# AliaksandrSiarohin/wc-gan

Hardware: AMD Instinct MI355X
Metric: images/sec G+D step, CIFAR-10 ResNet-SN+WC, batch 64 (higher is better)
Workload: dtype f32; 1 GPU; CIFAR-10 ResNet SN uncond + WC (scripts/cifar10_resnet_sn_uncond.sh), batch 64/GPU, training_ratio 5, generator_batch_multiple 2; parallelism=dp1, wc_statistics=per-replica, launch=hipgraph

## Files before the change

include/wc_hip.h:

```cpp
#ifndef WC_HIP_H
#define WC_HIP_H

#include <stddef.h>
#include <stdint.h>

#ifdef __cplusplus
extern "C" {
#endif

#define WC_ABI_VERSION 8

#define WC_OK                 0
#define WC_ERR_NULL          -1
#define WC_ERR_SHAPE         -2
#define WC_ERR_CHANNELS      -3
#define WC_ERR_WORKSPACE     -4
#define WC_ERR_ARG           -5

typedef void* wc_stream_t;

int         wc_abi_version(void);
const char* wc_error_string(int code);

#define WC_CORE_API "wc_stats_f32 wc_factor_f64 wc_color_f32 wc_group_bias_f32 wc_apply_f32 wc_apply_act_f32 " \
                    "wc_bwd_reduce_f32 wc_bwd_factor_f64 wc_bwd_apply_f32 " \
                    "wc_stats_workspace_bytes wc_factor_workspace_bytes wc_color_workspace_bytes wc_apply_workspace_bytes " \
                    "wc_bwd_reduce_workspace_bytes wc_bwd_factor_workspace_bytes wc_bwd_apply_workspace_bytes"

size_t wc_whiten_workspace_bytes(int64_t M, int C, int groups);
size_t wc_factor_error_offset(int C, int groups);
int    wc_factor_route(int C, int groups);
size_t wc_whiten_error_offset(int64_t M, int C, int groups);
int    wc_whiten_f32(const float* x, int64_t M, int C, int groups, double eps, double momentum, int ddof,
                     float* moving_mean , float* moving_cov ,
                     float* mu , float* chan_scale , double* L , double* W ,
                     void* ws, size_t ws_bytes, wc_stream_t stream);

size_t wc_stats_workspace_bytes(int64_t M, int C, int groups);
size_t wc_factor_workspace_bytes(int C, int groups);
size_t wc_color_workspace_bytes(int C, int Kc);
size_t wc_bwd_reduce_workspace_bytes(int64_t N, int64_t HW, int C, int Kc, int has_slot);
size_t wc_bwd_factor_workspace_bytes(int C, int Kc);
size_t wc_apply_workspace_bytes(int64_t N, int64_t HW, int C, int Kc);
size_t wc_apply_plan_bytes(int C, int Kc);
size_t wc_bwd_apply_workspace_bytes(int64_t N, int64_t HW, int C, int Kc);

int wc_stats_f32(const float* x, int64_t M, int C, int groups,
                 double* sum , double* xtx ,
                 void* ws, size_t ws_bytes, wc_stream_t stream);

int wc_factor_f64(const double* sum, const double* xtx, int64_t M , int C, int groups,
                  double eps, double momentum, int ddof, int training,
                  float* moving_mean , float* moving_cov ,
                  float* mu , float* chan_scale ,
                  double* L , double* W ,
                  void* ws, size_t ws_bytes, wc_stream_t stream);

int wc_color_f32(const double* W , const float* gamma ,
                 int Kc, int C, int groups, int per_group,
                 float* A , float* At ,
                 const float* chan_scale , void* plan ,
                 void* ws, size_t ws_bytes, wc_stream_t stream);

int wc_group_bias_f32(const float* mu , const float* A ,
                      const float* beta ,
                      int groups, int Kc, int C, int per_group, float* center , float* bias ,
                      wc_stream_t stream);

int wc_apply_f32(const float* x, const float* mu, const float* A, const float* bias,
                 const int32_t* slot, int64_t N, int64_t HW, int C, int Kc,
                 float* y, const void* plan ,
                 void* ws, size_t ws_bytes, wc_stream_t stream);

int wc_apply_act_f32(const float* x, const float* mu, const float* A, const float* bias,
                     const int32_t* slot, int64_t N, int64_t HW, int C, int Kc, int relu,
                     float* y, const void* plan ,
                     void* ws, size_t ws_bytes, wc_stream_t stream);

size_t wc_split_bytes(int64_t M, int C);
#define WC_SPLIT_FLAG_WORDS (64 + 2 * 1024)
int wc_split_scales_f32(const float* x, int64_t M, int C, float* center , float* scale ,
                        int* flag , wc_stream_t stream);
int wc_split_f32(const float* x, const float* center , const float* scale, int64_t M, int C, int relu,
                 void* xs , int* flag , wc_stream_t stream);
int wc_unsplit_f32(const void* xs, const float* center , const float* scale, int64_t M, int C, float* x ,
                   wc_stream_t stream);

int    wc_stats_split_supported(int64_t M, int C, int groups);
size_t wc_stats_split_workspace_bytes(int64_t M, int C, int groups);
int wc_stats_split_f16x2(const void* xs, const float* xs_center, const float* xs_scale, int64_t M, int C, int groups,
                         double* sum , double* xtx , void* ws, size_t ws_bytes, wc_stream_t stream);

int    wc_split_bias_f32(const float* A , const float* bias, const float* xs_center, const float* mu, int Kc, int C,
                         float* bias_eff , wc_stream_t stream);
int    wc_apply_split_supported(int64_t N, int64_t HW, int C);
size_t wc_apply_split_workspace_bytes(int C, int Kc);
int wc_apply_split_f16x2(const void* xs, const float* xs_center , const float* xs_scale,
                         const float* mu , const float* A, const float* bias ,
                         const int32_t* slot, int64_t N, int64_t HW, int C, int Kc, int relu,
                         float* y, const void* plan , void* ws, size_t ws_bytes, wc_stream_t stream);

int wc_resadd_split_supported(int64_t N, int64_t H, int64_t W, int C);
int wc_resadd_f32(const float* h, const float* s , int64_t N, int64_t H, int64_t W, int C, int up, float* out,
                  wc_stream_t stream);
int wc_resadd_split_f32(const float* h, const float* s , int64_t N, int64_t H, int64_t W, int C, int up,
                        void* xs , float* center , float* scale ,
                        int* flag , float* x32 ,
                        wc_stream_t stream);
int wc_patch_sum_f32(const float* g , int64_t N, int64_t Hs, int64_t Ws, int C, float* out ,
                     wc_stream_t stream);
int    wc_resadd_stats_supported(int64_t N, int64_t H, int64_t W, int C, int up, int groups);
size_t wc_resadd_stats_workspace_bytes(int64_t N, int64_t H, int64_t W, int C, int groups);
int    wc_resadd_stats_split_f32(const float* h, const float* s , int64_t N, int64_t H, int64_t W, int C, int up, int groups,
                                 void* xs , float* center , float* scale , int* flag ,
                                 float* x32 , void* ws , size_t ws_bytes, wc_stream_t stream);
size_t wc_whiten_presummed_error_offset(int64_t M, int C, int groups);
int    wc_whiten_presummed_f16x2(const float* xs_center, int64_t M, int C, int groups, double eps, double momentum, int ddof,
                                 float* moving_mean , float* moving_cov , float* mu ,
                                 double* L , double* W , void* ws ,
                                 size_t ws_bytes, wc_stream_t stream);
int    wc_stats_presummed_f16x2(const float* xs_center, int64_t M, int C, int groups, double* sum ,
                                double* xtx , void* ws , size_t ws_bytes, wc_stream_t stream);
int wc_fold_channel_scale_f32(const float* w, int64_t stride_o, int64_t stride_c, int Cout, int Cin, const float* bias ,
                              const float* scale, const float* center, float* wf , float* bf , wc_stream_t stream);
int wc_unfold_channel_scale_f32(const float* D, const float* db, int64_t stride_o, int64_t stride_c, int Cout, int Cin,
                                const float* scale, const float* center, float* dW , wc_stream_t stream);

size_t wc_whiten_split_workspace_bytes(int64_t M, int C, int groups);
size_t wc_whiten_split_error_offset(int64_t M, int C, int groups);
int    wc_whiten_split_f16x2(const void* xs, const float* xs_center, const float* xs_scale, int64_t M, int C, int groups,
                             double eps, double momentum, int ddof, float* moving_mean , float* moving_cov ,
                             float* mu , double* L , double* W ,
                             void* ws, size_t ws_bytes, wc_stream_t stream);

int wc_color_split_f32(const double* W , const float* gamma , int Kc, int C, float* A ,
                       float* At , const float* xs_scale, const float* xs_center, const float* mu ,
                       const float* beta , void* plan , float* bias_eff ,
                       void* ws, size_t ws_bytes, wc_stream_t stream);
int wc_group_bias_centered_f32(const float* mu , const float* A , const float* beta ,
                               const float* center , int groups, int Kc, int C, int per_group, float* bias ,
                               wc_stream_t stream);

int    wc_factor_mix_supported(int E, int C);
int    wc_factor_mix_f32(const float* dict, const float* alpha, const int32_t* idx , const float* base ,
                         int E, int C, int K, int Kc, float* out , wc_stream_t stream);
size_t wc_factor_mix_bwd_workspace_bytes(int E, int Kc);
int    wc_factor_mix_bwd_f32(const float* dict, const float* alpha, const int32_t* idx , const float* dout ,
                             int E, int C, int K, int Kc, float* ddict , float* dalpha , float* dbase ,
                             void* ws, size_t ws_bytes, wc_stream_t stream);

int wc_apply_split_ex_f16x2(const void* xs, const float* xs_center , const float* xs_scale,
                            const float* mu , const float* A, const float* bias ,
                            const int32_t* slot, int64_t N, int64_t HW, int C, int Kc, int relu,
                            float* y , void* relu_mask , void* planes , float* oscale,
                            const void* plan , void* ws, size_t ws_bytes, wc_stream_t stream);

size_t wc_relu_mask_bytes(int64_t M, int C);
int wc_relu_mask_apply_f32(const float* gy, const void* relu_mask, int64_t M, int C, float* out, wc_stream_t stream);
int wc_apply_mask_f32(const float* x, const float* mu, const float* A, const float* bias,
                      const int32_t* slot, int64_t N, int64_t HW, int C, int Kc,
                      float* y, void* relu_mask , const void* plan ,
                      void* ws, size_t ws_bytes, wc_stream_t stream);

int    wc_apply_planes_supported(int64_t N, int64_t HW, int C);
size_t wc_apply_planes_scale_floats(void);
int    wc_out_scale_f32(const float* gamma , const float* beta , int K, int C,
                        float* oscale, wc_stream_t stream);
int    wc_apply_planes_f32(const float* x, const float* mu, const float* A, const float* bias, const int32_t* slot,
                           int64_t N, int64_t HW, int C, int Kc, int relu, void* planes , float* oscale,
                           void* relu_mask , const void* plan, wc_stream_t stream);

int wc_bwd_reduce_f32(const float* x, const float* mu, const float* gy, const int32_t* slot,
                      int64_t N, int64_t HW, int C, int Kc,
                      double* R , double* gsum ,
                      void* ws, size_t ws_bytes, wc_stream_t stream);

int wc_bwd_reduce_scaled_f32(const float* x, const float* mu, const float* gy, const int32_t* slot,
                             int64_t N, int64_t HW, int C, int Kc,
                             double* R , double* gsum , float* scales_out ,
                             void* ws, size_t ws_bytes, wc_stream_t stream);
int wc_bwd_reduce_relu_f32(const float* x, const float* mu, const float* gy, const float* relu_y , const int32_t* slot,
                           int64_t N, int64_t HW, int C, int Kc,
                           double* R , double* gsum , float* gy_masked ,
                           float* scales_out , void* ws, size_t ws_bytes, wc_stream_t stream);
int wc_bwd_reduce_mask_f32(const float* x, const float* mu, const float* gy, const void* relu_mask, const int32_t* slot,
                           int64_t N, int64_t HW, int C, int Kc,
                           double* R , double* gsum , float* gy_masked ,
                           float* scales_out , void* ws, size_t ws_bytes, wc_stream_t stream);

int wc_bwd_bits_supported(int64_t N, int64_t HW, int C, int has_slot);
int wc_bwd_reduce_bits_f32(const float* x, const float* mu, const float* gy, const void* relu_mask, const int32_t* slot,
                           int64_t N, int64_t HW, int C, int Kc, double* R , double* gsum ,
                           float* scales_out , void* ws, size_t ws_bytes, wc_stream_t stream);
int wc_bwd_apply_bits_f32(const float* gy, const void* relu_mask, const float* x, const float* mu, const float* At, const float* S,
                          const float* gmean, const int32_t* slot, int64_t N, int64_t HW, int C, int Kc,
                          const float* scales , float* dx, void* ws, size_t ws_bytes, wc_stream_t stream);
int wc_bwd_apply_scaled_f32(const float* gy, const float* x, const float* mu, const float* At,
                            const float* S, const float* gmean, const int32_t* slot,
                            int64_t N, int64_t HW, int C, int Kc, const float* scales , float* dx,
                            void* ws, size_t ws_bytes, wc_stream_t stream);

int    wc_bwd_xsplit_supported(int64_t N, int64_t HW, int C, int has_slot);
int    wc_bwd_reduce_xsplit_f32(const void* xs, const float* xs_center, const float* xs_scale, const float* mu, const float* gy,
                                const void* relu_mask , const int32_t* slot, int64_t N, int64_t HW, int C, int Kc,
                                double* R , double* gsum , float* scales_out ,
                                void* ws , size_t ws_bytes, wc_stream_t stream);
size_t wc_bwd_apply_xsplit_workspace_bytes(int C, int Kc);
int    wc_bwd_apply_xsplit_f32(const float* gy, const void* relu_mask , const void* xs, const float* xs_center,
                               const float* xs_scale, const float* mu, const float* At, const float* S, const float* gmean,
                               const int32_t* slot, int64_t N, int64_t HW, int C, int Kc, const float* scales ,
                               float* dx, void* ws, size_t ws_bytes, wc_stream_t stream);

int wc_bwd_factor_f64(const double* R, const double* gsum, const double* W, const double* L,
                      const float* gamma, const float* A, int Kc, int C, int64_t M,
                      double eps, int ddof, int training,
                      float* dgamma , float* dbeta ,
                      float* S , float* gmean ,
                      void* ws, size_t ws_bytes, wc_stream_t stream);

int wc_bwd_apply_f32(const float* gy, const float* x, const float* mu, const float* At,
                     const float* S, const float* gmean, const int32_t* slot,
                     int64_t N, int64_t HW, int C, int Kc, float* dx,
                     void* ws, size_t ws_bytes, wc_stream_t stream);

size_t wc_spectral_norm_workspace_bytes(int rows, int cols);
size_t wc_spectral_norm_amax_offset(int rows, int cols);
size_t wc_spectral_norm_error_offset(int rows, int cols);
int wc_spectral_norm_f32(const float* W, int rows, int cols, float* u, float* v, int iterations, float eps,
                         float* w_sn , float* sigma ,
                         float* u_used , float* v_used ,
                         void* ws, size_t ws_bytes, wc_stream_t stream);

int wc_spectral_norm_bwd_f32(const float* g, const float* w_sn, const float* u, const float* v, const float* sigma,
                             int rows, int cols, int fully_diff, float* dW,
                             void* ws, size_t ws_bytes, wc_stream_t stream);

typedef struct {
    const float* W; float* u; float* v; float* w_sn; float* sigma; float* u_used; float* v_used; void* ws;
    int rows, cols;
} wc_sn_item;
typedef struct {
    const float* g; const float* w_sn; const float* u; const float* v; const float* sigma; float* dW; void* ws;
    int rows, cols;
} wc_sn_bwd_item;
int wc_spectral_norm_batched_f32(const wc_sn_item* items, int count, int iterations, float eps, wc_stream_t stream);
int wc_spectral_norm_bwd_batched_f32(const wc_sn_bwd_item* items, int count, int fully_diff, wc_stream_t stream);

typedef struct {
    int N, H, W;
    int Hin, Win, Cin;
    int Hout, Wout, Cout;
    int in_stride, out_stride;
    int ntaps, nphase;
    signed char dy[4][16], dx[4][16];
    signed char off_y[4], off_x[4];
    signed char nsrc[4][16];
    signed char wr[4][16][4], ws[4][16][4];
    float wcoef;
} wc_conv_geom;

#define WC_CONV_SCRATCH_BYTES 2048

int wc_conv_supported(const wc_conv_geom* g);

int wc_conv_split_f32(const float* x, int64_t n, int relu, void* hi, void* lo, float* scale, void* amax_scratch,
                      wc_stream_t stream);

#define WC_CONV_COLSUM_ROWS 512
int wc_conv_split_colsum_f32(const float* x, int64_t n, int relu, void* hi, void* lo, float* scale, void* amax_scratch,
                             float* colsum_partials, int C, wc_stream_t stream);

#define WC_CONV_HIST_FLOATS (4 * 512 + 16)
#define WC_CONV_HIST_REDO (4 * 512)
int wc_conv_split_hist_f32(const float* x, int64_t n, int relu, void* hi, void* lo, float* scale, float* colsum_partials , int C,
                           float* hist, int bootstrap, wc_stream_t stream);

int wc_conv_split_leaky_f32(const float* x, int64_t n, float negative_slope, void* hi, void* lo, float* scale, void* amax_scratch,
                            float* colsum_partials , int C, wc_stream_t stream);
int wc_conv_split_hist_leaky_f32(const float* x, int64_t n, float negative_slope, void* hi, void* lo, float* scale,
                                 float* colsum_partials , int C, float* hist, int bootstrap, wc_stream_t stream);
int wc_conv_leaky_bwd_f32(float* dx, const float* x, int64_t n, float negative_slope, wc_stream_t stream);

size_t wc_conv_weights_bytes(const wc_conv_geom* g);
int wc_conv_weights_f32(const float* w, int64_t stride_k, int64_t stride_n, int64_t stride_r, int64_t stride_s,
                        int64_t n_elems, const wc_conv_geom* g, void* image, float* scale, void* amax_scratch,
                        const float* known_amax, int known_count, wc_stream_t stream);

int wc_conv_weights_pair_f32(const float* w, int64_t stride_r, int64_t stride_s, int64_t n_elems,
                             int64_t a_stride_k, int64_t a_stride_n, const wc_conv_geom* ga, void* image_a,
                             int64_t b_stride_k, int64_t b_stride_n, const wc_conv_geom* gb, void* image_b,
                             float* scale, void* amax_scratch, const float* known_amax, int known_count,
                             wc_stream_t stream);

size_t wc_conv_workspace_bytes(const wc_conv_geom* g);
int wc_conv_f16x3(const void* xhi, const void* xlo, const float* xscale, const void* wimage, const float* wscale,
                  const float* bias, const void* zero_line, const wc_conv_geom* g, int relu, float* y,
                  void* ws, size_t ws_bytes, wc_stream_t stream);

size_t wc_conv_wrw_workspace_bytes(const wc_conv_geom* g);
int wc_conv_wrw_f16x3(const void* xhi, const void* xlo, const float* xscale, const void* ghi, const void* glo,
                      const float* gscale, const void* zero_line, const wc_conv_geom* g, float* dw, int64_t stride_k,
                      int64_t stride_n, int64_t stride_r, int64_t stride_s, void* ws, size_t ws_bytes,
                      wc_stream_t stream);

int    wc_conv_wrw_narrow_supported(int64_t N, int64_t H, int64_t W, int Cin, int Cout, int ksize);
size_t wc_conv_wrw_narrow_workspace_bytes(int64_t N, int64_t H, int64_t W, int Cin, int Cout, int ksize);
int    wc_conv_wrw_narrow_f32(const float* x, const float* gy, int64_t N, int64_t H, int64_t W, int Cin, int Cout, int ksize,
                              float* dw, int64_t stride_k, int64_t stride_n, int64_t stride_r, int64_t stride_s, float* db ,
                              void* ws, size_t ws_bytes, wc_stream_t stream);

int    wc_conv_narrow64_supported(int64_t N, int64_t H, int64_t W, int Cin, int Cout, int ksize);
size_t wc_conv_wrw_narrow64_workspace_bytes(int64_t N, int64_t H, int64_t W, int Cin, int Cout, int ksize);
int    wc_conv_wrw_narrow64_f32(const float* x, const float* gy, int64_t N, int64_t H, int64_t W, int Cin, int Cout, int ksize,
                                float* dw, int64_t stride_k, int64_t stride_n, int64_t stride_r, int64_t stride_s, float* db ,
                                void* ws, size_t ws_bytes, wc_stream_t stream);

int    wc_conv_fwd_narrow_f32(const float* x, const float* w, int64_t stride_k, int64_t stride_n, int64_t stride_r, int64_t stride_s,
                              const float* bias , int64_t N, int64_t H, int64_t W, int Cin, int Cout, int ksize, int relu,
                              float* y, wc_stream_t stream);

int wc_conv_wrw_bias_f16x3(const void* xhi, const void* xlo, const float* xscale, const void* ghi, const void* glo,
                           const float* gscale, const void* zero_line, const wc_conv_geom* g, float* dw, int64_t stride_k,
                           int64_t stride_n, int64_t stride_r, int64_t stride_s, const float* colsum_partials, float* db,
                           void* ws, size_t ws_bytes, wc_stream_t stream);

int wc_stream_copy_f32(const float* src, float* dst, int64_t n, wc_stream_t stream);


size_t wc_std_stats_workspace_bytes(int64_t M, int C, int groups);
int    wc_std_stats_f32(const float* x, int64_t M, int C, int groups, double* sum , double* sqsum ,
                        void* ws, size_t ws_bytes, wc_stream_t stream);

int    wc_std_factor_f64(const double* sum, const double* sqsum, int64_t M, int C, int groups, double eps, double momentum, int ddof,
                         int training, float* moving_mean , float* moving_variance ,
                         const float* gamma , const float* beta , int Kc,
                         float* mu , float* w , float* a , float* b ,
                         wc_stream_t stream);

int    wc_std_apply_f32(const float* x, const float* a, const float* b, const int32_t* slot , int64_t N, int64_t HW,
                        int C, int Kt, int relu, float* y, wc_stream_t stream);

size_t wc_std_bwd_reduce_workspace_bytes(int64_t N, int64_t HW, int C, int Kc);
int    wc_std_bwd_reduce_f32(const float* x, const float* gy, const float* a, const float* b, const int32_t* slot, int64_t N, int64_t HW,
                             int C, int Kc, int relu, double* gsum , double* gxsum ,
                             void* ws, size_t ws_bytes, wc_stream_t stream);

int    wc_std_bwd_factor_f64(const double* gsum, const double* gxsum, const float* mu , const float* w ,
                             const float* gamma , int64_t M, int C, int Kc, int training,
                             float* dgamma , float* dbeta , float* q , float* r , wc_stream_t stream);

int    wc_std_bwd_apply_f32(const float* x, const float* gy, const float* a, const float* b, const float* q, const float* r,
                            const int32_t* slot, int64_t N, int64_t HW, int C, int Kc, int relu, float* dx, wc_stream_t stream);


int    wc_zca_supported(int C);
size_t wc_zca_workspace_bytes(int C, int groups);
size_t wc_zca_status_offset(int C, int groups);
int    wc_zca_f64(const double* L , int C, int groups, double eps,
                  double* U , double* lam , double* W ,
                  void* ws, size_t ws_bytes, wc_stream_t stream);

size_t wc_bwd_factor_zca_workspace_bytes(int C, int Kc);
int    wc_bwd_factor_zca_f64(const double* R, const double* gsum, const double* W, const double* U, const double* lam,
                             const float* gamma, const float* A, int Kc, int C, int64_t M,
                             double eps, int ddof, int training,
                             float* dgamma , float* dbeta ,
                             float* S , float* gmean ,
                             void* ws, size_t ws_bytes, wc_stream_t stream);


int    wc_renorm_supported(int C);
size_t wc_renorm_workspace_bytes(int C);
int    wc_renorm_f64(const float* moving_cov , const double* L , int C, double eps,
                     double* Wm , double* C0 ,
                     void* ws, size_t ws_bytes, wc_stream_t stream);

size_t wc_bwd_factor_renorm_workspace_bytes(int C, int Kc);
int    wc_bwd_factor_renorm_f64(const double* R, const double* gsum, const double* W, const double* Wm, const double* C0,
                                const float* gamma, const float* A, int Kc, int C, int64_t M,
                                double eps, int ddof, int training,
                                float* dgamma , float* dbeta ,
                                float* S , float* gmean ,
                                void* ws, size_t ws_bytes, wc_stream_t stream);


int wc_conv_split_masked_f32(const float* t, const float* a, int64_t n, float slope, void* hi, void* lo, float* scale, void* amax_scratch,
                             wc_stream_t stream);
int wc_conv_split_hist_masked_f32(const float* t, const float* a, int64_t n, float slope, void* hi, void* lo, float* scale, float* hist,
                                  int bootstrap, wc_stream_t stream);

int wc_gp_interp_f32(const float* real, const float* fake, const float* eps, int64_t N, int64_t L, float* x_hat, wc_stream_t stream);

size_t wc_gp_rows_workspace_bytes(int64_t N);
int wc_gp_rows_f32(const float* g, int64_t N, int64_t L, double lambda, double inv_n, float* norms , float* v ,
                   float* penalty , void* ws, size_t ws_bytes, wc_stream_t stream);

#ifdef __cplusplus
}
#endif
#endif
```

wc_gan_amd/_lib.py:

```python
from __future__ import annotations

import ctypes
import os
from ctypes import c_float, c_char_p, c_double, c_int, c_int64, c_size_t, c_void_p

_HERE = os.path.dirname(os.path.abspath(__file__))
LIB_PATH = os.path.join(_HERE, "libwc_hip.so")

WC_OK = 0
ABI_VERSION = 8
ERRORS = {-1: "WC_ERR_NULL", -2: "WC_ERR_SHAPE", -3: "WC_ERR_CHANNELS", -4: "WC_ERR_WORKSPACE", -5: "WC_ERR_ARG"}

SIGNATURES = {
    "wc_abi_version": (c_int, []),
    "wc_error_string": (c_char_p, [c_int]),
    "wc_stats_workspace_bytes": (c_size_t, [c_int64, c_int, c_int]),
    "wc_factor_workspace_bytes": (c_size_t, [c_int, c_int]),
    "wc_color_workspace_bytes": (c_size_t, [c_int, c_int]),
    "wc_bwd_reduce_workspace_bytes": (c_size_t, [c_int64, c_int64, c_int, c_int, c_int]),
    "wc_bwd_factor_workspace_bytes": (c_size_t, [c_int, c_int]),
    "wc_apply_workspace_bytes": (c_size_t, [c_int64, c_int64, c_int, c_int]),
    "wc_apply_plan_bytes": (c_size_t, [c_int, c_int]),
    "wc_bwd_apply_workspace_bytes": (c_size_t, [c_int64, c_int64, c_int, c_int]),
    "wc_stats_f32": (c_int, [c_void_p, c_int64, c_int, c_int, c_void_p, c_void_p, c_void_p, c_size_t, c_void_p]),
    "wc_group_bias_f32": (c_int, [c_void_p, c_void_p, c_void_p, c_int, c_int, c_int, c_int, c_void_p, c_void_p, c_void_p]),
    "wc_factor_f64": (c_int, [c_void_p, c_void_p, c_int64, c_int, c_int, c_double, c_double, c_int, c_int,
                              c_void_p, c_void_p, c_void_p, c_void_p, c_void_p, c_void_p, c_void_p, c_size_t, c_void_p]),
    "wc_color_f32": (c_int, [c_void_p, c_void_p, c_int, c_int, c_int, c_int, c_void_p, c_void_p, c_void_p, c_void_p,
                             c_void_p, c_size_t, c_void_p]),
    "wc_apply_f32": (c_int, [c_void_p, c_void_p, c_void_p, c_void_p, c_void_p, c_int64, c_int64, c_int, c_int,
                             c_void_p, c_void_p, c_void_p, c_size_t, c_void_p]),
    "wc_apply_act_f32": (c_int, [c_void_p, c_void_p, c_void_p, c_void_p, c_void_p, c_int64, c_int64, c_int, c_int, c_int,
                                 c_void_p, c_void_p, c_void_p, c_size_t, c_void_p]),
    "wc_bwd_reduce_f32": (c_int, [c_void_p, c_void_p, c_void_p, c_void_p, c_int64, c_int64, c_int, c_int,
                                  c_void_p, c_void_p, c_void_p, c_size_t, c_void_p]),
    "wc_bwd_reduce_scaled_f32": (c_int, [c_void_p, c_void_p, c_void_p, c_void_p, c_int64, c_int64, c_int, c_int,
                                         c_void_p, c_void_p, c_void_p, c_void_p, c_size_t, c_void_p]),
    "wc_bwd_reduce_relu_f32": (c_int, [c_void_p, c_void_p, c_void_p, c_void_p, c_void_p, c_int64, c_int64, c_int, c_int,
                                       c_void_p, c_void_p, c_void_p, c_void_p, c_void_p, c_size_t, c_void_p]),
    "wc_relu_mask_bytes": (c_size_t, [c_int64, c_int]),
    "wc_relu_mask_apply_f32": (c_int, [c_void_p, c_void_p, c_int64, c_int, c_void_p, c_void_p]),
    "wc_apply_mask_f32": (c_int, [c_void_p, c_void_p, c_void_p, c_void_p, c_void_p, c_int64, c_int64, c_int, c_int,
                                  c_void_p, c_void_p, c_void_p, c_void_p, c_size_t, c_void_p]),
    "wc_whiten_workspace_bytes": (c_size_t, [c_int64, c_int, c_int]),
    "wc_factor_error_offset": (c_size_t, [c_int, c_int]),
    "wc_factor_route": (c_int, [c_int, c_int]),
    "wc_whiten_error_offset": (c_size_t, [c_int64, c_int, c_int]),
    "wc_whiten_f32": (c_int, [c_void_p, c_int64, c_int, c_int, c_double, c_double, c_int, c_void_p, c_void_p, c_void_p, c_void_p,
                              c_void_p, c_void_p, c_void_p, c_size_t, c_void_p]),
    "wc_apply_planes_supported": (c_int, [c_int64, c_int64, c_int]),
    "wc_apply_planes_scale_floats": (c_size_t, []),
    "wc_out_scale_f32": (c_int, [c_void_p, c_void_p, c_int, c_int, c_void_p, c_void_p]),
    "wc_apply_planes_f32": (c_int, [c_void_p, c_void_p, c_void_p, c_void_p, c_void_p, c_int64, c_int64, c_int, c_int, c_int,
                                    c_void_p, c_void_p, c_void_p, c_void_p, c_void_p]),
    "wc_bwd_reduce_mask_f32": (c_int, [c_void_p, c_void_p, c_void_p, c_void_p, c_void_p, c_int64, c_int64, c_int, c_int,
                                       c_void_p, c_void_p, c_void_p, c_void_p, c_void_p, c_size_t, c_void_p]),
    "wc_bwd_bits_supported": (c_int, [c_int64, c_int64, c_int, c_int]),
    "wc_bwd_reduce_bits_f32": (c_int, [c_void_p, c_void_p, c_void_p, c_void_p, c_void_p, c_int64, c_int64, c_int, c_int,
                                       c_void_p, c_void_p, c_void_p, c_void_p, c_size_t, c_void_p]),
    "wc_bwd_apply_bits_f32": (c_int, [c_void_p, c_void_p, c_void_p, c_void_p, c_void_p, c_void_p, c_void_p, c_void_p,
                                      c_int64, c_int64, c_int, c_int, c_void_p, c_void_p, c_void_p, c_size_t, c_void_p]),
    "wc_bwd_apply_scaled_f32": (c_int, [c_void_p, c_void_p, c_void_p, c_void_p, c_void_p, c_void_p, c_void_p,
                                        c_int64, c_int64, c_int, c_int, c_void_p, c_void_p, c_void_p, c_size_t, c_void_p]),
    "wc_bwd_factor_f64": (c_int, [c_void_p, c_void_p, c_void_p, c_void_p, c_void_p, c_void_p, c_int, c_int, c_int64,
                                  c_double, c_int, c_int, c_void_p, c_void_p, c_void_p, c_void_p,
                                  c_void_p, c_size_t, c_void_p]),
    "wc_bwd_apply_f32": (c_int, [c_void_p, c_void_p, c_void_p, c_void_p, c_void_p, c_void_p, c_void_p,
                                 c_int64, c_int64, c_int, c_int, c_void_p, c_void_p, c_size_t, c_void_p]),
    "wc_split_bytes": (c_size_t, [c_int64, c_int]),
    "wc_split_scales_f32": (c_int, [c_void_p, c_int64, c_int, c_void_p, c_void_p, c_void_p, c_void_p]),
    "wc_split_f32": (c_int, [c_void_p, c_void_p, c_void_p, c_int64, c_int, c_int, c_void_p, c_void_p, c_void_p]),
    "wc_unsplit_f32": (c_int, [c_void_p, c_void_p, c_void_p, c_int64, c_int, c_void_p, c_void_p]),
    "wc_stats_split_supported": (c_int, [c_int64, c_int, c_int]),
    "wc_stats_split_workspace_bytes": (c_size_t, [c_int64, c_int, c_int]),
    "wc_stats_split_f16x2": (c_int, [c_void_p, c_void_p, c_void_p, c_int64, c_int, c_int, c_void_p, c_void_p, c_void_p, c_size_t, c_void_p]),
    "wc_split_bias_f32": (c_int, [c_void_p, c_void_p, c_void_p, c_void_p, c_int, c_int, c_void_p, c_void_p]),
    "wc_apply_split_supported": (c_int, [c_int64, c_int64, c_int]),
    "wc_apply_split_workspace_bytes": (c_size_t, [c_int, c_int]),
    "wc_apply_split_f16x2": (c_int, [c_void_p, c_void_p, c_void_p, c_void_p, c_void_p, c_void_p, c_void_p, c_int64, c_int64,
                                     c_int, c_int, c_int, c_void_p, c_void_p, c_void_p, c_size_t, c_void_p]),
    "wc_apply_split_ex_f16x2": (c_int, [c_void_p, c_void_p, c_void_p, c_void_p, c_void_p, c_void_p, c_void_p, c_int64, c_int64,
                                        c_int, c_int, c_int, c_void_p, c_void_p, c_void_p, c_void_p, c_void_p, c_void_p, c_size_t, c_void_p]),
    "wc_whiten_split_workspace_bytes": (c_size_t, [c_int64, c_int, c_int]),
    "wc_whiten_split_error_offset": (c_size_t, [c_int64, c_int, c_int]),
    "wc_whiten_split_f16x2": (c_int, [c_void_p, c_void_p, c_void_p, c_int64, c_int, c_int, c_double, c_double, c_int, c_void_p, c_void_p,
                                      c_void_p, c_void_p, c_void_p, c_void_p, c_size_t, c_void_p]),
    "wc_resadd_split_supported": (c_int, [c_int64, c_int64, c_int64, c_int]),
    "wc_resadd_f32": (c_int, [c_void_p, c_void_p, c_int64, c_int64, c_int64, c_int, c_int, c_void_p, c_void_p]),
    "wc_resadd_stats_supported": (c_int, [c_int64, c_int64, c_int64, c_int, c_int, c_int]),
    "wc_resadd_stats_workspace_bytes": (c_size_t, [c_int64, c_int64, c_int64, c_int, c_int]),
    "wc_resadd_stats_split_f32": (c_int, [c_void_p, c_void_p, c_int64, c_int64, c_int64, c_int, c_int, c_int, c_void_p, c_void_p, c_void_p, c_void_p,
                                          c_void_p, c_void_p, c_size_t, c_void_p]),
    "wc_whiten_presummed_error_offset": (c_size_t, [c_int64, c_int, c_int]),
    "wc_whiten_presummed_f16x2": (c_int, [c_void_p, c_int64, c_int, c_int, c_double, c_double, c_int, c_void_p, c_void_p, c_void_p, c_void_p,
                                          c_void_p, c_void_p, c_size_t, c_void_p]),
    "wc_stats_presummed_f16x2": (c_int, [c_void_p, c_int64, c_int, c_int, c_void_p, c_void_p, c_void_p, c_size_t, c_void_p]),
    "wc_resadd_split_f32": (c_int, [c_void_p, c_void_p, c_int64, c_int64, c_int64, c_int, c_int, c_void_p, c_void_p, c_void_p, c_void_p,
                                    c_void_p, c_void_p]),
    "wc_patch_sum_f32": (c_int, [c_void_p, c_int64, c_int64, c_int64, c_int, c_void_p, c_void_p]),
    "wc_fold_channel_scale_f32": (c_int, [c_void_p, c_int64, c_int64, c_int, c_int, c_void_p, c_void_p, c_void_p, c_void_p, c_void_p, c_void_p]),
    "wc_unfold_channel_scale_f32": (c_int, [c_void_p, c_void_p, c_int64, c_int64, c_int, c_int, c_void_p, c_void_p, c_void_p, c_void_p]),
    "wc_color_split_f32": (c_int, [c_void_p, c_void_p, c_int, c_int, c_void_p, c_void_p, c_void_p, c_void_p, c_void_p, c_void_p, c_void_p,
                                   c_void_p, c_void_p, c_size_t, c_void_p]),
    "wc_factor_mix_supported": (c_int, [c_int, c_int]),
    "wc_factor_mix_f32": (c_int, [c_void_p, c_void_p, c_void_p, c_void_p, c_int, c_int, c_int, c_int, c_void_p, c_void_p]),
    "wc_factor_mix_bwd_workspace_bytes": (c_size_t, [c_int, c_int]),
    "wc_factor_mix_bwd_f32": (c_int, [c_void_p, c_void_p, c_void_p, c_void_p, c_int, c_int, c_int, c_int, c_void_p, c_void_p, c_void_p,
                                      c_void_p, c_size_t, c_void_p]),
    "wc_group_bias_centered_f32": (c_int, [c_void_p, c_void_p, c_void_p, c_void_p, c_int, c_int, c_int, c_int, c_void_p, c_void_p]),
    "wc_bwd_xsplit_supported": (c_int, [c_int64, c_int64, c_int, c_int]),
    "wc_bwd_reduce_xsplit_f32": (c_int, [c_void_p, c_void_p, c_void_p, c_void_p, c_void_p, c_void_p, c_void_p, c_int64, c_int64, c_int, c_int,
                                         c_void_p, c_void_p, c_void_p, c_void_p, c_size_t, c_void_p]),
    "wc_bwd_apply_xsplit_workspace_bytes": (c_size_t, [c_int, c_int]),
    "wc_bwd_apply_xsplit_f32": (c_int, [c_void_p, c_void_p, c_void_p, c_void_p, c_void_p, c_void_p, c_void_p, c_void_p, c_void_p, c_void_p,
                                        c_int64, c_int64, c_int, c_int, c_void_p, c_void_p, c_void_p, c_size_t, c_void_p]),
    "wc_stream_copy_f32": (c_int, [c_void_p, c_void_p, c_int64, c_void_p]),
    "wc_spectral_norm_workspace_bytes": (c_size_t, [c_int, c_int]),
    "wc_spectral_norm_batched_f32": (c_int, [c_void_p, c_int, c_int, c_float, c_void_p]),
    "wc_spectral_norm_bwd_batched_f32": (c_int, [c_void_p, c_int, c_int, c_void_p]),
    "wc_spectral_norm_f32": (c_int, [c_void_p, c_int, c_int, c_void_p, c_void_p, c_int, c_float, c_void_p, c_void_p,
                                     c_void_p, c_void_p, c_void_p, c_size_t, c_void_p]),
    "wc_spectral_norm_bwd_f32": (c_int, [c_void_p, c_void_p, c_void_p, c_void_p, c_void_p, c_int, c_int, c_int, c_void_p,
                                         c_void_p, c_size_t, c_void_p]),
    "wc_conv_supported": (c_int, [c_void_p]),
    "wc_conv_split_f32": (c_int, [c_void_p, c_int64, c_int, c_void_p, c_void_p, c_void_p, c_void_p, c_void_p]),
    "wc_conv_weights_bytes": (c_size_t, [c_void_p]),
    "wc_conv_weights_f32": (c_int, [c_void_p, c_int64, c_int64, c_int64, c_int64, c_int64, c_void_p, c_void_p, c_void_p,
                                    c_void_p, c_void_p, c_int, c_void_p]),
    "wc_spectral_norm_amax_offset": (c_size_t, [c_int, c_int]),
    "wc_spectral_norm_error_offset": (c_size_t, [c_int, c_int]),
    "wc_conv_split_hist_f32": (c_int, [c_void_p, c_int64, c_int, c_void_p, c_void_p, c_void_p, c_void_p, c_int, c_void_p, c_int, c_void_p]),
    "wc_conv_split_leaky_f32": (c_int, [c_void_p, c_int64, c_float, c_void_p, c_void_p, c_void_p, c_void_p, c_void_p, c_int, c_void_p]),
    "wc_conv_split_hist_leaky_f32": (c_int, [c_void_p, c_int64, c_float, c_void_p, c_void_p, c_void_p, c_void_p, c_int, c_void_p, c_int, c_void_p]),
    "wc_conv_leaky_bwd_f32": (c_int, [c_void_p, c_void_p, c_int64, c_float, c_void_p]),
    "wc_conv_narrow64_supported": (c_int, [c_int64, c_int64, c_int64, c_int, c_int, c_int]),
    "wc_conv_wrw_narrow64_workspace_bytes": (c_size_t, [c_int64, c_int64, c_int64, c_int, c_int, c_int]),
    "wc_conv_wrw_narrow64_f32": (c_int, [c_void_p, c_void_p, c_int64, c_int64, c_int64, c_int, c_int, c_int, c_void_p, c_int64, c_int64, c_int64,
                                         c_int64, c_void_p, c_void_p, c_size_t, c_void_p]),
    "wc_conv_fwd_narrow_f32": (c_int, [c_void_p, c_void_p, c_int64, c_int64, c_int64, c_int64, c_void_p, c_int64, c_int64, c_int64, c_int, c_int, c_int,
                                       c_int, c_void_p, c_void_p]),
    "wc_conv_wrw_narrow_supported": (c_int, [c_int64, c_int64, c_int64, c_int, c_int, c_int]),
    "wc_conv_wrw_narrow_workspace_bytes": (c_size_t, [c_int64, c_int64, c_int64, c_int, c_int, c_int]),
    "wc_conv_wrw_narrow_f32": (c_int, [c_void_p, c_void_p, c_int64, c_int64, c_int64, c_int, c_int, c_int, c_void_p, c_int64, c_int64, c_int64,
                                       c_int64, c_void_p, c_void_p, c_size_t, c_void_p]),
    "wc_conv_split_colsum_f32": (c_int, [c_void_p, c_int64, c_int, c_void_p, c_void_p, c_void_p, c_void_p, c_void_p, c_int, c_void_p]),
    "wc_conv_wrw_bias_f16x3": (c_int, [c_void_p, c_void_p, c_void_p, c_void_p, c_void_p, c_void_p, c_void_p, c_void_p, c_void_p,
                                       c_int64, c_int64, c_int64, c_int64, c_void_p, c_void_p, c_void_p, c_size_t, c_void_p]),
    "wc_conv_weights_pair_f32": (c_int, [c_void_p, c_int64, c_int64, c_int64, c_int64, c_int64, c_void_p, c_void_p,
                                         c_int64, c_int64, c_void_p, c_void_p, c_void_p, c_void_p, c_void_p, c_int, c_void_p]),
    "wc_conv_wrw_workspace_bytes": (c_size_t, [c_void_p]),
    "wc_conv_wrw_f16x3": (c_int, [c_void_p, c_void_p, c_void_p, c_void_p, c_void_p, c_void_p, c_void_p, c_void_p, c_void_p,
                                  c_int64, c_int64, c_int64, c_int64, c_void_p, c_size_t, c_void_p]),
    "wc_conv_workspace_bytes": (c_size_t, [c_void_p]),
    "wc_conv_f16x3": (c_int, [c_void_p, c_void_p, c_void_p, c_void_p, c_void_p, c_void_p, c_void_p, c_void_p, c_int,
                              c_void_p, c_void_p, c_size_t, c_void_p]),
    "wc_std_stats_workspace_bytes": (c_size_t, [c_int64, c_int, c_int]),
    "wc_std_stats_f32": (c_int, [c_void_p, c_int64, c_int, c_int, c_void_p, c_void_p, c_void_p, c_size_t, c_void_p]),
    "wc_std_factor_f64": (c_int, [c_void_p, c_void_p, c_int64, c_int, c_int, c_double, c_double, c_int, c_int, c_void_p, c_void_p,
                                  c_void_p, c_void_p, c_int, c_void_p, c_void_p, c_void_p, c_void_p, c_void_p]),
    "wc_std_apply_f32": (c_int, [c_void_p, c_void_p, c_void_p, c_void_p, c_int64, c_int64, c_int, c_int, c_int, c_void_p, c_void_p]),
    "wc_std_bwd_reduce_workspace_bytes": (c_size_t, [c_int64, c_int64, c_int, c_int]),
    "wc_std_bwd_reduce_f32": (c_int, [c_void_p, c_void_p, c_void_p, c_void_p, c_void_p, c_int64, c_int64, c_int, c_int, c_int,
                                      c_void_p, c_void_p, c_void_p, c_size_t, c_void_p]),
    "wc_std_bwd_factor_f64": (c_int, [c_void_p, c_void_p, c_void_p, c_void_p, c_void_p, c_int64, c_int, c_int, c_int,
                                      c_void_p, c_void_p, c_void_p, c_void_p, c_void_p]),
    "wc_std_bwd_apply_f32": (c_int, [c_void_p, c_void_p, c_void_p, c_void_p, c_void_p, c_void_p, c_void_p, c_int64, c_int64, c_int, c_int,
                                     c_int, c_void_p, c_void_p]),
    "wc_zca_supported": (c_int, [c_int]),
    "wc_zca_workspace_bytes": (c_size_t, [c_int, c_int]),
    "wc_zca_status_offset": (c_size_t, [c_int, c_int]),
    "wc_zca_f64": (c_int, [c_void_p, c_int, c_int, c_double, c_void_p, c_void_p, c_void_p, c_void_p, c_size_t, c_void_p]),
    "wc_bwd_factor_zca_workspace_bytes": (c_size_t, [c_int, c_int]),
    "wc_bwd_factor_zca_f64": (c_int, [c_void_p, c_void_p, c_void_p, c_void_p, c_void_p, c_void_p, c_void_p, c_int, c_int, c_int64,
                                      c_double, c_int, c_int, c_void_p, c_void_p, c_void_p, c_void_p,
                                      c_void_p, c_size_t, c_void_p]),
    "wc_renorm_supported": (c_int, [c_int]),
    "wc_renorm_workspace_bytes": (c_size_t, [c_int]),
    "wc_renorm_f64": (c_int, [c_void_p, c_void_p, c_int, c_double, c_void_p, c_void_p, c_void_p, c_size_t, c_void_p]),
    "wc_bwd_factor_renorm_workspace_bytes": (c_size_t, [c_int, c_int]),
    "wc_bwd_factor_renorm_f64": (c_int, [c_void_p, c_void_p, c_void_p, c_void_p, c_void_p, c_void_p, c_void_p, c_int, c_int, c_int64,
                                         c_double, c_int, c_int, c_void_p, c_void_p, c_void_p, c_void_p,
                                         c_void_p, c_size_t, c_void_p]),
    "wc_conv_split_masked_f32": (c_int, [c_void_p, c_void_p, c_int64, c_float, c_void_p, c_void_p, c_void_p, c_void_p, c_void_p]),
    "wc_conv_split_hist_masked_f32": (c_int, [c_void_p, c_void_p, c_int64, c_float, c_void_p, c_void_p, c_void_p, c_void_p, c_int, c_void_p]),
    "wc_gp_interp_f32": (c_int, [c_void_p, c_void_p, c_void_p, c_int64, c_int64, c_void_p, c_void_p]),
    "wc_gp_rows_workspace_bytes": (c_size_t, [c_int64]),
    "wc_gp_rows_f32": (c_int, [c_void_p, c_int64, c_int64, c_double, c_double, c_void_p, c_void_p, c_void_p, c_void_p, c_size_t, c_void_p]),
}


class SnItem(ctypes.Structure):
    _fields_ = [("W", c_void_p), ("u", c_void_p), ("v", c_void_p), ("w_sn", c_void_p), ("sigma", c_void_p),
                ("u_used", c_void_p), ("v_used", c_void_p), ("ws", c_void_p), ("rows", c_int), ("cols", c_int)]


class SnBwdItem(ctypes.Structure):
    _fields_ = [("g", c_void_p), ("w_sn", c_void_p), ("u", c_void_p), ("v", c_void_p), ("sigma", c_void_p),
                ("dW", c_void_p), ("ws", c_void_p), ("rows", c_int), ("cols", c_int)]


class ConvGeom(ctypes.Structure):
    _fields_ = [("N", c_int), ("H", c_int), ("W", c_int), ("Hin", c_int), ("Win", c_int), ("Cin", c_int),
                ("Hout", c_int), ("Wout", c_int), ("Cout", c_int), ("in_stride", c_int), ("out_stride", c_int),
                ("ntaps", c_int), ("nphase", c_int),
                ("dy", (ctypes.c_byte * 16) * 4), ("dx", (ctypes.c_byte * 16) * 4),
                ("off_y", ctypes.c_byte * 4), ("off_x", ctypes.c_byte * 4),
                ("nsrc", (ctypes.c_byte * 16) * 4),
                ("wr", ((ctypes.c_byte * 4) * 16) * 4), ("ws", ((ctypes.c_byte * 4) * 16) * 4),
                ("wcoef", c_float)]


_lib = None


class WcHipError(RuntimeError):
    pass


def shared_gpu_guard(device_count=None) -> bool:
    if "WC_K2_TWO_LAUNCH" in os.environ:
        if os.environ["WC_K2_TWO_LAUNCH"] == "0":
            del os.environ["WC_K2_TWO_LAUNCH"]
        return False
    try:
        ranks = int(os.environ.get("LOCAL_WORLD_SIZE", "1") or 1)
    except ValueError:
        ranks = 1
    if ranks <= 1:
        return False
    if any(os.environ.get(k) for k in ("HIP_VISIBLE_DEVICES", "CUDA_VISIBLE_DEVICES", "ROCR_VISIBLE_DEVICES")):
        return False
    if device_count is None:
        try:
            import torch
            device_count = torch.cuda.device_count()
        except Exception:
            device_count = 0
    if device_count and ranks > device_count:
        os.environ["WC_K2_TWO_LAUNCH"] = "1"
        return True
    return False


def load() -> ctypes.CDLL:
    global _lib
    if _lib is not None:
        return _lib
    import torch
    shared_gpu_guard()
    if not os.path.exists(LIB_PATH):
        raise WcHipError(
            f"{LIB_PATH} is missing: build it with `python -m wc_gan_amd.build` "
            "(or __graft_entry__.build()); the WC path has no non-HIP fallback")
    lib = ctypes.CDLL(LIB_PATH)
    for name, (res, args) in SIGNATURES.items():
        fn = getattr(lib, name)
        fn.restype = res
        fn.argtypes = args
    if lib.wc_abi_version() != ABI_VERSION:
        raise WcHipError(f"libwc_hip.so ABI version {lib.wc_abi_version()} != {ABI_VERSION}: rebuild it "
                         "(python -m wc_gan_amd.build)")
    _lib = lib
    return lib


def check(code: int, what: str) -> None:
    if code == WC_OK:
        return
    lib = load()
    msg = lib.wc_error_string(code)
    raise WcHipError(f"{what} failed: {ERRORS.get(code, code)} ({msg.decode() if msg else '?'})")
```

wc_gan_amd/conv.py:

```python
from __future__ import annotations

import ctypes
import os

import torch
import torch.nn.functional as F

from . import _lib, _state
from .ops import _ptr, _stream

_zero_lines = {}


def _zero_line(device):
    z = _zero_lines.get(device)
    if z is None:
        z = _zero_lines[device] = torch.zeros(64, dtype=torch.uint8, device=device)
    return z


def _plain(r, s):
    return [(r, s)], 1.0


def _pooled3(r, s):
    return [(r - a, s - b) for a in (0, 1) for b in (0, 1) if 0 <= r - a <= 2 and 0 <= s - b <= 2], 0.25


_UP_ROWS = ((2,), (1, 2), (0, 1), (0,))


def _upsampled3(r, s):
    return [(r3, s3) for r3 in _UP_ROWS[r] for s3 in _UP_ROWS[s]], 1.0


def _set_sources(g, p, t, r, s, source):
    taps, coef = source(r, s)
    g.nsrc[p][t] = len(taps)
    for m, (r3, s3) in enumerate(taps):
        g.wr[p][t][m], g.ws[p][t][m] = r3, s3
    g.wcoef = coef


def _dense_geom(N, Hin, Win, Cin, Cout, k, stride, source=_plain):
    pad = k // 2 if stride == 1 else 1
    g = _lib.ConvGeom()
    g.N, g.Hin, g.Win, g.Cin, g.Cout = N, Hin, Win, Cin, Cout
    g.H, g.W = Hin // stride, Win // stride
    g.Hout, g.Wout = g.H, g.W
    g.in_stride, g.out_stride, g.ntaps, g.nphase = stride, 1, k * k, 1
    for r in range(k):
        for s in range(k):
            t = r * k + s
            g.dy[0][t], g.dx[0][t] = r - pad, s - pad
            _set_sources(g, 0, t, r, s, source)
    return g


def _phase_geom(N, Hin, Win, Cin, Cout, source=_plain):
    g = _lib.ConvGeom()
    g.N, g.Hin, g.Win, g.Cin, g.Cout = N, Hin, Win, Cin, Cout
    g.H, g.W, g.Hout, g.Wout = Hin, Win, 2 * Hin, 2 * Win
    g.in_stride, g.out_stride, g.ntaps, g.nphase = 1, 2, 4, 4
    for py in range(2):
        for px in range(2):
            p = py * 2 + px
            g.off_y[p], g.off_x[p] = py, px
            t = 0
            for dy in ((-1, 0) if py == 0 else (0, 1)):
                for dx in ((-1, 0) if px == 0 else (0, 1)):
                    g.dy[p][t], g.dx[p][t] = dy, dx
                    _set_sources(g, p, t, py + 1 - 2 * dy, px + 1 - 2 * dx, source)
                    t += 1
    return g


def _supported(g):
    return bool(_lib.load().wc_conv_supported(ctypes.addressof(g)))


def supported(x, w, kind):
    handed = getattr(x, '_wc_planes', None) is not None
    if not (x.is_cuda and x.dtype == torch.float32 and x.dim() == 4 and (handed or x.is_contiguous()) and w.dtype == torch.float32):
        return False
    p = _plan(kind, x, w)
    return bool(p) and p.ok


class _Plan:
    __slots__ = ('ok', 'fwd', 'bwd', 'fwd_ws', 'bwd_ws', 'wrw_ws', 'fwd_ptr', 'bwd_ptr')

    def __init__(self, kind, N, H, W, wshape):
        class _W:
            shape = wshape
        lib = _lib.load()
        (gf, kf, nf), (gb, kb, nb) = _geoms(kind, N, H, W, _W)
        self.fwd, self.bwd = (gf, kf, nf), (gb, kb, nb)
        self.fwd_ptr, self.bwd_ptr = ctypes.addressof(gf), ctypes.addressof(gb)
        self.ok = bool(lib.wc_conv_supported(self.fwd_ptr)) and bool(lib.wc_conv_supported(self.bwd_ptr))
        self.fwd_ws = lib.wc_conv_workspace_bytes(self.fwd_ptr) if self.ok else 0
        self.bwd_ws = lib.wc_conv_workspace_bytes(self.bwd_ptr) if self.ok else 0
        self.wrw_ws = lib.wc_conv_wrw_workspace_bytes(self.fwd_ptr) if self.ok else 0


_plans = {}


def _plan(kind, x, w):
    key = (kind, tuple(x.shape), tuple(w.shape))
    p = _plans.get(key)
    if p is None:
        N, H, W, C = x.shape
        good = (kind == 'same' and w.shape[1] == C and w.shape[2] == w.shape[3] and w.shape[2] in (1, 3)) or \
               (kind == 'down' and w.shape[1] == C and tuple(w.shape[2:]) == (4, 4) and H % 2 == 0 and W % 2 == 0) or \
               (kind == 'down3' and w.shape[1] == C and tuple(w.shape[2:]) == (3, 3) and H % 2 == 0 and W % 2 == 0) or \
               (kind == 'up3' and w.shape[1] == C and tuple(w.shape[2:]) == (3, 3)) or \
               (kind == 'up' and w.shape[0] == C and tuple(w.shape[2:]) == (4, 4))
        if kind not in ('same', 'down', 'up', 'down3', 'up3'):
            raise ValueError(kind)
        if good and kind != 'down' and (C % 128 or w.shape[0] % 128 or w.shape[1] % 128):
            good = False
        p = _plans[key] = _Plan(kind, N, H, W, tuple(w.shape)) if good else False
    return p


def _colsum_ok(C):
    return C % 4 == 0 and 256 % (C // 4) == 0


SPLIT_HIST = os.environ.get('WC_SPLIT_HIST', '1') != '0'
HIST_FLOATS = 4 * 512 + 16
HIST_REDO = 4 * 512


_REDO_MODE = os.environ.get('WC_SPLIT_HIST_REDO', '1')


def _guarded(role):
    return _REDO_MODE == '2' or (_REDO_MODE != '0' and role in ('g', 't', 'd'))


def _site_hist(site, role, device):
    if not getattr(site, 'training', True):
        return None
    book = site.__dict__.setdefault('_wc_split_hist', {})
    h = book.get(role)
    if h is not None and h[0].device != device:
        h = None
    if h is None:
        if torch.cuda.is_current_stream_capturing():
            return None
        h = book[role] = [torch.zeros(HIST_FLOATS, dtype=torch.float32, device=device), False]
    return h


def split_planes(x, relu=False, colsum=False, site=None, role='x', leaky=None):
    lib = _lib.load()
    if leaky is not None:
        if relu:
            raise ValueError("relu and leaky are two activations")
        return _split_planes_leaky(lib, x, float(leaky), colsum, site, role)
    both = torch.empty((2,) + tuple(x.shape), dtype=torch.float16, device=x.device)
    hi, lo = both[0], both[1]
    scale = torch.empty(1 + 512, dtype=torch.float32, device=x.device)
    h = _site_hist(site, role, x.device) if (SPLIT_HIST and site is not None) else None
    if h is not None:
        C = x.shape[-1]
        part = torch.empty((512, C), dtype=torch.float32, device=x.device) if colsum else None
        _lib.check(lib.wc_conv_split_hist_f32(_ptr(x), x.numel(), 1 if relu else 0, _ptr(hi), _ptr(lo), _ptr(scale), _ptr(part), C if colsum else 0,
                                              _ptr(h[0]), (0 if h[1] else 1) | (0 if _guarded(role) else 2), _stream()), "wc_conv_split_hist_f32")
        h[1] = True
        return (hi, lo, scale, part) if colsum else (hi, lo, scale)
    if not colsum:
        _lib.check(lib.wc_conv_split_f32(_ptr(x), x.numel(), 1 if relu else 0, _ptr(hi), _ptr(lo), _ptr(scale),
                                         scale.data_ptr() + 4, _stream()), "wc_conv_split_f32")
        return hi, lo, scale
    C = x.shape[-1]
    part = torch.empty((512, C), dtype=torch.float32, device=x.device)
    _lib.check(lib.wc_conv_split_colsum_f32(_ptr(x), x.numel(), 1 if relu else 0, _ptr(hi), _ptr(lo), _ptr(scale),
                                            scale.data_ptr() + 4, _ptr(part), C, _stream()), "wc_conv_split_colsum_f32")
    return hi, lo, scale, part


def _split_planes_leaky(lib, x, slope, colsum, site, role):
    both = torch.empty((2,) + tuple(x.shape), dtype=torch.float16, device=x.device)
    hi, lo = both[0], both[1]
    scale = torch.empty(1 + 512, dtype=torch.float32, device=x.device)
    C = x.shape[-1]
    part = torch.empty((512, C), dtype=torch.float32, device=x.device) if colsum else None
    h = _site_hist(site, role, x.device) if (SPLIT_HIST and site is not None) else None
    if h is not None:
        _lib.check(lib.wc_conv_split_hist_leaky_f32(_ptr(x), x.numel(), slope, _ptr(hi), _ptr(lo), _ptr(scale), _ptr(part), C if colsum else 0,
                                                    _ptr(h[0]), (0 if h[1] else 1) | (0 if _guarded(role) else 2), _stream()),
                   "wc_conv_split_hist_leaky_f32")
        h[1] = True
    else:
        _lib.check(lib.wc_conv_split_leaky_f32(_ptr(x), x.numel(), slope, _ptr(hi), _ptr(lo), _ptr(scale), scale.data_ptr() + 4,
                                               _ptr(part), C if colsum else 0, _stream()), "wc_conv_split_leaky_f32")
    return (hi, lo, scale, part) if colsum else (hi, lo, scale)


def split_planes_masked(t, a, slope=0.0, site=None, role='t'):
    if not (t.is_contiguous() and a.is_contiguous() and t.shape == a.shape and t.dtype == a.dtype == torch.float32):
        raise ValueError("split_planes_masked: dense fp32 tensors of one shape")
    lib = _lib.load()
    both = torch.empty((2,) + tuple(t.shape), dtype=torch.float16, device=t.device)
    hi, lo = both[0], both[1]
    scale = torch.empty(1 + 512, dtype=torch.float32, device=t.device)
    h = _site_hist(site, role, t.device) if (SPLIT_HIST and site is not None) else None
    if h is not None:
        _lib.check(lib.wc_conv_split_hist_masked_f32(_ptr(t), _ptr(a), t.numel(), float(slope), _ptr(hi), _ptr(lo), _ptr(scale), _ptr(h[0]),
                                                     (0 if h[1] else 1) | (0 if _guarded(role) else 2), _stream()),
                   "wc_conv_split_hist_masked_f32")
        h[1] = True
    else:
        _lib.check(lib.wc_conv_split_masked_f32(_ptr(t), _ptr(a), t.numel(), float(slope), _ptr(hi), _ptr(lo), _ptr(scale),
                                                scale.data_ptr() + 4, _stream()), "wc_conv_split_masked_f32")
    return hi, lo, scale


def leaky_backward_(dx, x, slope):
    if not (dx.is_contiguous() and x.is_contiguous() and dx.shape == x.shape and dx.dtype == x.dtype == torch.float32):
        raise ValueError("leaky_backward_: dense fp32 tensors of one shape")
    _lib.check(_lib.load().wc_conv_leaky_bwd_f32(_ptr(dx), _ptr(x), dx.numel(), float(slope), _stream()), "wc_conv_leaky_bwd_f32")
    return dx


def _storage_extent(w):
    return 1 + sum((n - 1) * s for n, s in zip(w.shape, w.stride()))


def weight_image(w, geom, k_axis, n_axis):
    lib = _lib.load()
    nbytes = lib.wc_conv_weights_bytes(ctypes.addressof(geom))
    img = torch.empty(nbytes, dtype=torch.uint8, device=w.device)
    scale = torch.empty(1 + 512, dtype=torch.float32, device=w.device)
    ext = _storage_extent(w)
    if ext != w.numel():
        raise ValueError("weight must be dense")
    known = getattr(w, '_wc_amax', None)
    _lib.check(lib.wc_conv_weights_f32(_ptr(w), w.stride(k_axis), w.stride(n_axis), w.stride(2), w.stride(3), ext,
                                       ctypes.addressof(geom), _ptr(img), _ptr(scale), scale.data_ptr() + 4,
                                       _ptr(known), 0 if known is None else known.numel(), _stream()),
               "wc_conv_weights_f32")
    return img, scale


def weight_image_pair(w, fwd, bwd):
    lib = _lib.load()
    (ga, ka, na), (gb, kb, nb) = fwd, bwd
    img_a = torch.empty(lib.wc_conv_weights_bytes(ctypes.addressof(ga)), dtype=torch.uint8, device=w.device)
    img_b = torch.empty(lib.wc_conv_weights_bytes(ctypes.addressof(gb)), dtype=torch.uint8, device=w.device)
    scale = torch.empty(2 + 512, dtype=torch.float32, device=w.device)
    ext = _storage_extent(w)
    if ext != w.numel():
        raise ValueError("weight must be dense")
    known = getattr(w, '_wc_amax', None)
    _lib.check(lib.wc_conv_weights_pair_f32(_ptr(w), w.stride(2), w.stride(3), ext,
                                            w.stride(ka), w.stride(na), ctypes.addressof(ga), _ptr(img_a),
                                            w.stride(kb), w.stride(nb), ctypes.addressof(gb), _ptr(img_b),
                                            _ptr(scale), scale.data_ptr() + 8, _ptr(known), 0 if known is None else known.numel(),
                                            _stream()), "wc_conv_weights_pair_f32")
    return (img_a, scale[0:1]), (img_b, scale[1:2])


def _cached_image(w, key, geom, k_axis, n_axis):
    return weight_image(w, geom, k_axis, n_axis)


def run(planes, image, geom, bias=None, relu=False, nbytes=None):
    hi, lo, xs = planes
    img, ws = image
    lib = _lib.load()
    y = torch.empty((geom.N, geom.Hout, geom.Wout, geom.Cout), dtype=torch.float32, device=hi.device)
    if nbytes is None:
        nbytes = lib.wc_conv_workspace_bytes(ctypes.addressof(geom))
    work = torch.empty(nbytes, dtype=torch.uint8, device=hi.device) if nbytes else None
    _lib.check(lib.wc_conv_f16x3(_ptr(hi), _ptr(lo), _ptr(xs), _ptr(img), _ptr(ws), _ptr(bias) if bias is not None else None,
                                 _ptr(_zero_line(hi.device)), ctypes.addressof(geom), 1 if relu else 0, _ptr(y),
                                 _ptr(work), nbytes, _stream()), "wc_conv_f16x3")
    return y


def _geoms(kind, N, H, W, w):
    if kind == 'same':
        co, ci, k = w.shape[0], w.shape[1], w.shape[2]
        fwd = _dense_geom(N, H, W, ci, co, k, 1)
        bwd = _dense_geom(N, H, W, co, ci, k, 1)
        for t in range(k * k):
            bwd.dy[0][t], bwd.dx[0][t] = -bwd.dy[0][t], -bwd.dx[0][t]
        return (fwd, 1, 0), (bwd, 0, 1)
    if kind in ('down', 'down3'):
        co, ci = w.shape[0], w.shape[1]
        src = _pooled3 if kind == 'down3' else _plain
        return (_dense_geom(N, H, W, ci, co, 4, 2, src), 1, 0), (_phase_geom(N, H // 2, W // 2, co, ci, src), 0, 1)
    if kind == 'up3':
        co, ci = w.shape[0], w.shape[1]
        return (_phase_geom(N, H, W, ci, co, _upsampled3), 1, 0), (_dense_geom(N, 2 * H, 2 * W, co, ci, 4, 2, _upsampled3), 0, 1)
    ci, co = w.shape[0], w.shape[1]
    return (_phase_geom(N, H, W, ci, co), 0, 1), (_dense_geom(N, 2 * H, 2 * W, co, ci, 4, 2), 1, 0)


def weight_gradient(x_planes, g_planes, geom, w, k_axis, n_axis, nbytes=None, colsum=None):
    lib = _lib.load()
    xh, xl, xs = x_planes
    gh, gl, gs = g_planes[:3]
    dw = torch.empty_like(w)
    if dw.stride() != w.stride():
        raise ValueError("weight must be dense")
    if nbytes is None:
        nbytes = lib.wc_conv_wrw_workspace_bytes(ctypes.addressof(geom))
    ws = torch.empty(nbytes, dtype=torch.uint8, device=w.device)
    if colsum is not None:
        db = torch.empty(geom.Cout, dtype=torch.float32, device=w.device)
        _lib.check(lib.wc_conv_wrw_bias_f16x3(_ptr(xh), _ptr(xl), _ptr(xs), _ptr(gh), _ptr(gl), _ptr(gs), _ptr(_zero_line(w.device)),
                                              ctypes.addressof(geom), _ptr(dw), w.stride(k_axis), w.stride(n_axis), w.stride(2),
                                              w.stride(3), _ptr(colsum), _ptr(db), _ptr(ws), nbytes, _stream()),
                   "wc_conv_wrw_bias_f16x3")
        return dw, db
    _lib.check(lib.wc_conv_wrw_f16x3(_ptr(xh), _ptr(xl), _ptr(xs), _ptr(gh), _ptr(gl), _ptr(gs), _ptr(_zero_line(w.device)),
                                     ctypes.addressof(geom), _ptr(dw), w.stride(k_axis), w.stride(n_axis), w.stride(2),
                                     w.stride(3), _ptr(ws), nbytes, _stream()), "wc_conv_wrw_f16x3")
    return dw


def takes_planes(shape, wshape, kind):
    class _S:
        pass
    xs, ws = _S(), _S()
    xs.shape, ws.shape = tuple(shape), tuple(wshape)
    p = _plan(kind, xs, ws)
    return bool(p) and p.ok


class _FastConv(torch.autograd.Function):
    @staticmethod
    def forward(ctx, x, w, bias, kind, plan, relu_input=False, handed=None, site=None, leaky=None):
        gf, kf, nf = plan.fwd
        planes = handed if handed is not None else split_planes(x, relu=relu_input, site=site, role='x', leaky=leaky)
        ctx.site, ctx.leaky = site, leaky
        if ctx.needs_input_grad[0]:
            img, ctx.bwd_image = weight_image_pair(w, plan.fwd, plan.bwd)
        else:
            img, ctx.bwd_image = weight_image(w, gf, kf, nf), None
        y = run(planes, img, gf, bias, nbytes=plan.fwd_ws)
        ctx.save_for_backward(w, *planes, *((x,) if (relu_input or leaky is not None) else ()))
        ctx.kind, ctx.has_bias, ctx.plan, ctx.relu_input = kind, bias is not None, plan, relu_input
        return y

    @staticmethod
    def backward(ctx, gy):
        w, xh, xl, xs = ctx.saved_tensors[:4]
        kind, plan = ctx.kind, ctx.plan
        gy = gy.contiguous()
        want_db = ctx.has_bias and ctx.needs_input_grad[2]
        fused_db = want_db and ctx.needs_input_grad[1] and _colsum_ok(gy.shape[-1])
        g_planes = split_planes(gy, colsum=fused_db, site=ctx.site, role='g')
        dx = dw = db = None
        if ctx.needs_input_grad[0]:
            gb, kb, nb = plan.bwd
            image = ctx.bwd_image if ctx.bwd_image is not None else weight_image(w, gb, kb, nb)
            dx = run(g_planes[:3], image, gb, nbytes=plan.bwd_ws)
            if ctx.relu_input:
                dx = torch.ops.aten.threshold_backward(dx, ctx.saved_tensors[4], 0)
            elif ctx.leaky is not None:
                dx = leaky_backward_(dx, ctx.saved_tensors[4], ctx.leaky)
        if ctx.needs_input_grad[1]:
            gf, kf, nf = plan.fwd
            if fused_db:
                dw, db = weight_gradient((xh, xl, xs), g_planes, gf, w, kf, nf, nbytes=plan.wrw_ws, colsum=g_planes[3])
            else:
                dw = weight_gradient((xh, xl, xs), g_planes, gf, w, kf, nf, nbytes=plan.wrw_ws)
        if want_db and not fused_db:
            db = gy.sum((0, 1, 2))
        return dx, dw, db, None, None, None, None, None, None


_ones = {}


def _one(device):
    t = _ones.get(device)
    if t is None:
        t = torch.ones(1, dtype=torch.float32, device=device)
        if not torch.cuda.is_current_stream_capturing():
            _ones[device] = t
    return t


class _SplitConv(torch.autograd.Function):

    @staticmethod
    def forward(ctx, x, w, bias, plan, st, site=None):
        from . import ops
        ctx.site = site
        gf, kf, nf = plan.fwd
        wf, bf = ops.fold_channel_scale(w, bias, st.scale, st.center)
        img = weight_image(wf, gf, kf, nf)
        ctx.bwd_image = None
        if ctx.needs_input_grad[0]:
            gb, kb, nb = plan.bwd
            ctx.bwd_image = weight_image(w, gb, kb, nb)
        hi, lo = st.planes[0].view(st.shape), st.planes[1].view(st.shape)
        one = _one(hi.device)
        y = run((hi, lo, one), img, gf, bf, nbytes=plan.fwd_ws)
        ctx.save_for_backward(w, hi, lo, one, st.scale, st.center)
        ctx.plan, ctx.has_bias = plan, bias is not None
        return y

    @staticmethod
    def backward(ctx, gy):
        from . import ops
        w, xh, xl, one, scale, center = ctx.saved_tensors
        plan = ctx.plan
        gy = gy.contiguous()
        need_w = ctx.needs_input_grad[1]
        need_b = ctx.has_bias and ctx.needs_input_grad[2]
        fused_db = need_w and _colsum_ok(gy.shape[-1])
        g_planes = split_planes(gy, colsum=fused_db, site=ctx.site, role='g')
        dx = dw = db = None
        if ctx.needs_input_grad[0]:
            gb, kb, nb = plan.bwd
            image = ctx.bwd_image if ctx.bwd_image is not None else weight_image(w, gb, kb, nb)
            dx = run(g_planes[:3], image, gb, nbytes=plan.bwd_ws)
        if need_w:
            gf, kf, nf = plan.fwd
            if fused_db:
                D, db = weight_gradient((xh, xl, one), g_planes, gf, w, kf, nf, nbytes=plan.wrw_ws, colsum=g_planes[3])
            else:
                D = weight_gradient((xh, xl, one), g_planes, gf, w, kf, nf, nbytes=plan.wrw_ws)
                db = gy.sum((0, 1, 2))
            dw = ops.unfold_channel_scale(D, db, scale, center)
        elif need_b:
            db = gy.sum((0, 1, 2))
        return dx, dw, (db if need_b else None), None, None, None


def split_conv(x, st, w, bias=None, site=None):
    p = _plan('same', x, w)
    if not (p and p.ok and tuple(w.shape[2:]) == (1, 1) and w.dtype == torch.float32):
        raise _lib.WcHipError(f"split_conv: a pre-split handle reached a convolution without a planes path {tuple(x.shape)} x {tuple(w.shape)}")
    return _SplitConv.apply(x, w, bias, p, st, site)


def fast_conv_or_none(x, w, bias=None, kind='same', relu_input=False, site=None, leaky_input=None):
    if leaky_input is not None and relu_input:
        raise ValueError("relu_input and leaky_input are two activations")
    handed = getattr(x, '_wc_planes', None)
    if not supported(x, w, kind):
        if handed is not None:
            raise _lib.WcHipError(f"fast_conv: a K3 handle reached a convolution that cannot take planes {tuple(x.shape)} x {tuple(w.shape)} ({kind})")
        return None
    if handed is not None:
        if relu_input or leaky_input is not None:
            raise ValueError("a K3 handle is already ReLU'd")
        return _FastConv.apply(x, w, bias, kind, _plan(kind, x, w), False, handed, site)
    return _FastConv.apply(x, w, bias, kind, _plan(kind, x, w), relu_input, None, site,
                           None if leaky_input is None else float(leaky_input))


NARROW_WRW = os.environ.get('WC_NARROW_WRW', '1') != '0'


def narrow_wrw_supported(x, w):
    if not (NARROW_WRW and x.is_cuda and x.dtype == torch.float32 and w.dtype == torch.float32 and x.dim() == 4 and w.dim() == 4):
        return False
    k = w.shape[2]
    if w.shape[3] != k or k not in (1, 3) or w.shape[1] != x.shape[3]:
        return False
    N, H, W, C = x.shape
    return bool(_lib.load().wc_conv_narrow64_supported(N, H, W, C, w.shape[0], k))


def narrow_forward(x, w, bias=None, relu=False, mirrored=False):
    lib = _lib.load()
    N, H, W, C = x.shape
    k = w.shape[2]
    if mirrored:
        O = w.shape[1]
        ptr = ctypes.c_void_p(w.data_ptr() + 4 * ((k - 1) * w.stride(2) + (k - 1) * w.stride(3)))
        strides = (w.stride(0), w.stride(1), -w.stride(2), -w.stride(3))
    else:
        O = w.shape[0]
        ptr = _ptr(w)
        strides = (w.stride(1), w.stride(0), w.stride(2), w.stride(3))
    y = torch.empty((N, H, W, O), dtype=torch.float32, device=x.device)
    xc = x if x.is_contiguous() else x.contiguous()
    _lib.check(lib.wc_conv_fwd_narrow_f32(_ptr(xc), ptr, *strides, _ptr(bias), N, H, W, C, O, k, 1 if relu else 0, _ptr(y), _stream()),
               "wc_conv_fwd_narrow_f32")
    return y


class _NarrowInConv(torch.autograd.Function):

    @staticmethod
    def forward(ctx, x, w, bias):
        ctx.save_for_backward(x, w)
        ctx.has_bias = bias is not None
        return narrow_forward(x, w, bias)

    @staticmethod
    def backward(ctx, gy):
        x, w = ctx.saved_tensors
        N, H, W, C = x.shape
        O, k = w.shape[0], w.shape[2]
        lib = _lib.load()
        dx = dw = db = None
        g = gy if gy.is_contiguous() else gy.contiguous()
        if ctx.needs_input_grad[0]:
            dx = torch.ops.aten.convolution_backward(g.permute(0, 3, 1, 2), x.permute(0, 3, 1, 2), w, None, [1, 1], [k // 2, k // 2], [1, 1],
                                                     False, [0, 0], 1, [True, False, False])[0].permute(0, 2, 3, 1)
        if ctx.needs_input_grad[1] or (ctx.has_bias and ctx.needs_input_grad[2]):
            dw = torch.empty_strided(w.shape, w.stride(), dtype=torch.float32, device=w.device)
            if _storage_extent(dw) != dw.numel():
                raise ValueError("weight must be dense")
            db = torch.empty(O, dtype=torch.float32, device=w.device) if ctx.has_bias else None
            nb = lib.wc_conv_wrw_narrow64_workspace_bytes(N, H, W, C, O, k)
            ws = torch.empty(nb, dtype=torch.uint8, device=x.device)
            xc = x if x.is_contiguous() else x.contiguous()
            _lib.check(lib.wc_conv_wrw_narrow64_f32(_ptr(xc), _ptr(g), N, H, W, C, O, k, _ptr(dw), dw.stride(1), dw.stride(0), dw.stride(2),
                                                    dw.stride(3), _ptr(db), _ptr(ws), nb, _stream()), "wc_conv_wrw_narrow64_f32")
        return dx, dw, db


def narrow_weight_gradient(x, gy, w):
    N, H, W, C = x.shape
    O, k = w.shape[0], w.shape[2]
    lib = _lib.load()
    dw = torch.empty_strided(w.shape, w.stride(), dtype=torch.float32, device=w.device)
    if _storage_extent(dw) != dw.numel():
        raise ValueError("weight must be dense")
    nb = lib.wc_conv_wrw_narrow64_workspace_bytes(N, H, W, C, O, k)
    ws = torch.empty(nb, dtype=torch.uint8, device=x.device)
    xc = x if x.is_contiguous() else x.contiguous()
    g = gy if gy.is_contiguous() else gy.contiguous()
    _lib.check(lib.wc_conv_wrw_narrow64_f32(_ptr(xc), _ptr(g), N, H, W, C, O, k, _ptr(dw), dw.stride(1), dw.stride(0), dw.stride(2),
                                            dw.stride(3), None, _ptr(ws), nb, _stream()), "wc_conv_wrw_narrow64_f32")
    return dw


def narrow_in_conv(x, w, bias=None):
    if _storage_extent(w) != w.numel():
        w = w.contiguous()
    return _NarrowInConv.apply(x, w, bias)


def narrow_out_weight_gradient(x, gy, w):
    lib = _lib.load()
    N, H, W, C = x.shape
    O, k = w.shape[0], w.shape[2]
    dw = torch.empty_strided(w.shape, w.stride(), dtype=torch.float32, device=w.device)
    if _storage_extent(dw) != dw.numel():
        raise ValueError("weight must be dense")
    nb = lib.wc_conv_wrw_narrow_workspace_bytes(N, H, W, O, C, k)
    ws = torch.empty(nb, dtype=torch.uint8, device=x.device)
    last = dw.data_ptr() + 4 * ((k - 1) * dw.stride(2) + (k - 1) * dw.stride(3))
    _lib.check(lib.wc_conv_wrw_narrow_f32(_ptr(gy), _ptr(x), N, H, W, O, C, k, ctypes.c_void_p(last), dw.stride(0), dw.stride(1), -dw.stride(2),
                                          -dw.stride(3), None, _ptr(ws), nb, _stream()), "wc_conv_wrw_narrow_f32")
    return dw


def narrow_out_wrw_supported(x, w):
    if not (NARROW_WRW and x.is_cuda and x.dtype == torch.float32 and w.dtype == torch.float32 and x.dim() == 4 and w.dim() == 4):
        return False
    k = w.shape[2]
    if w.shape[3] != k or k not in (1, 3) or w.shape[1] != x.shape[3]:
        return False
    N, H, W, C = x.shape
    return bool(_lib.load().wc_conv_wrw_narrow_supported(N, H, W, w.shape[0], C, k))


def fast_conv(x, w, bias=None, kind='same'):
    if not supported(x, w, kind):
        raise _lib.WcHipError(f"fast_conv: unsupported call {tuple(x.shape)} x {tuple(w.shape)} ({kind})")
    return _FastConv.apply(x, w, bias, kind, _plan(kind, x, w))
```

wc_gan_amd/csrc/wc_conv.hip:

```cpp
#include "wc_common.h"
#include "../../include/wc_hip.h"
#include <stdlib.h>


namespace {

constexpr int kMaxTaps = 16, kMaxPhase = 4;

struct ConvArgs {
    const _Float16* xhi; const _Float16* xlo;
    const _Float16* zero;
    const char* wimg;
    const float* xscale; const float* wscale;
    const float* bias;
    float* y;
    int N, H, W, Hin, Win, Cin, Cout, in_stride, ntaps, nphase, Hout, Wout, out_stride, relu;
    unsigned magHW, shHW, magW, shW;
    int ksplit; float* partial;
    signed char dy[kMaxPhase][kMaxTaps], dx[kMaxPhase][kMaxTaps];
    signed char offy[kMaxPhase], offx[kMaxPhase];
};

__device__ __forceinline__ void lds_dma16(const void* g, unsigned lds)
{
    unsigned keep;
    asm volatile("s_mov_b32 %0, m0\n\ts_mov_b32 m0, %2\n\ts_nop 0\n\tglobal_load_lds_dwordx4 %1, off\n\ts_mov_b32 m0, %0"
                 : "=&s"(keep) : "v"(g), "s"(lds) : "memory");
}

template <int MB, int NB, bool KS>
__global__ __launch_bounds__(256) void conv_f16x3_kernel(ConvArgs a)
{
    extern __shared__ __attribute__((aligned(16))) char smem[];
    constexpr int TM = 64 * MB, TN = 64 * NB;
    constexpr int A_BYTES = 2 * MB * 4 * 1024, B_BYTES = 2 * NB * 4 * 1024, STAGE = A_BYTES + B_BYTES;
    constexpr int AQ = (2 * MB) / 4;
    static_assert(AQ >= 1, "MB >= 2");

    const int tid = threadIdx.x, lane = tid & 63;
    const int wave = __builtin_amdgcn_readfirstlane(tid >> 6);
    const int wm = wave >> 1, wn = wave & 1;
    const int ntn = a.Cout / TN;
    const int phase = blockIdx.y / ntn, nt = blockIdx.y - phase * ntn;
    const unsigned m0 = blockIdx.x * TM;
    const unsigned HW = a.H * a.W;
    const int koff = (lane >> 5) * 8;

    int gy[AQ], gx[AQ];
    unsigned gpix[AQ];
    #pragma unroll
    for (int q = 0; q < AQ; ++q) {
        const unsigned m = m0 + (wave * AQ + q) * 32 + (lane & 31);
        const unsigned n = __umulhi(m, a.magHW) >> a.shHW, rem = m - n * HW;
        const unsigned yy = __umulhi(rem, a.magW) >> a.shW, xx = rem - yy * a.W;
        gy[q] = yy * a.in_stride; gx[q] = xx * a.in_stride; gpix[q] = n * (a.Hin * a.Win);
    }
    const unsigned lds0 = (unsigned)(size_t)((__attribute__((address_space(3))) char*)smem);
    const int nchunk = a.Cin >> 5;
    const int iters = a.ntaps * nchunk;
    const int nblk_all = a.Cout >> 5;

    auto issue = [&](int it, int stage) {
        const int tap = it / nchunk, ch = it - tap * nchunk;
        const int dy = a.dy[phase][tap], dx = a.dx[phase][tap];
        const unsigned sbase = __builtin_amdgcn_readfirstlane(lds0 + stage * STAGE);
        #pragma unroll
        for (int q = 0; q < AQ; ++q) {
            const int iy = gy[q] + dy, ix = gx[q] + dx;
            const bool ok = (unsigned)iy < (unsigned)a.Hin && (unsigned)ix < (unsigned)a.Win;
            const int64_t e = ((int64_t)(gpix[q] + iy * a.Win + ix)) * a.Cin + ch * 32 + koff;
            #pragma unroll
            for (int s = 0; s < 2; ++s) {
                const _Float16* ph = ok ? a.xhi + e + s * 16 : a.zero + koff;
                const _Float16* pl = ok ? a.xlo + e + s * 16 : a.zero + koff;
                const unsigned l = sbase + (((wave * AQ + q) * 2 + s) * 2) * 1024;
                lds_dma16(ph, l);
                lds_dma16(pl, l + 1024);
            }
        }
        const char* wsrc = a.wimg + ((((int64_t)(phase * a.ntaps + tap) * nchunk + ch) * nblk_all + nt * 2 * NB) << 12);
        #pragma unroll
        for (int c = 0; c < 2 * NB; ++c) {
            const int idx = wave * 2 * NB + c;
            lds_dma16(wsrc + idx * 1024 + lane * 16, sbase + A_BYTES + idx * 1024);
        }
    };

    f32x16 acc[MB][NB];
    #pragma unroll
    for (int i = 0; i < MB; ++i)
        #pragma unroll
        for (int j = 0; j < NB; ++j)
            #pragma unroll
            for (int r = 0; r < 16; ++r) acc[i][j][r] = 0.f;

    const int it0 = KS ? (int)blockIdx.z * iters / a.ksplit : 0, it1 = KS ? ((int)blockIdx.z + 1) * iters / a.ksplit : iters;
    constexpr int NA = AQ * 4, ND = NA + 2 * NB, HALF = ND / 2, PER = 3 * MB * NB, GAP = PER / HALF;
    static_assert(PER % HALF == 0, "DMAs spread evenly");
    int tabv = 0;
    if (lane < a.ntaps) tabv = (a.dy[phase][lane] & 0xff) | ((a.dx[phase][lane] & 0xff) << 8);
    const char* pa[AQ][2];
    int pstep[AQ];
    const char* pw;
    unsigned sb_next = 0;
    auto prep = [&](int it, int stage) {
        const int tap = it / nchunk, ch = it - tap * nchunk;
        const int p = __builtin_amdgcn_readlane(tabv, tap);
        const int dy = (signed char)(p & 0xff), dx = (signed char)((p >> 8) & 0xff);
        #pragma unroll
        for (int q = 0; q < AQ; ++q) {
            const int iy = gy[q] + dy, ix = gx[q] + dx;
            const bool ok = (unsigned)iy < (unsigned)a.Hin && (unsigned)ix < (unsigned)a.Win;
            const int64_t e = ((int64_t)(gpix[q] + iy * a.Win + ix)) * a.Cin + ch * 32 + koff;
            pa[q][0] = reinterpret_cast<const char*>(ok ? a.xhi + e : a.zero + koff);
            pa[q][1] = reinterpret_cast<const char*>(ok ? a.xlo + e : a.zero + koff);
            pstep[q] = ok ? 32 : 0;
        }
        pw = a.wimg + ((((int64_t)(phase * a.ntaps + tap) * nchunk + ch) * nblk_all + nt * 2 * NB) << 12) + wave * (2 * NB * 1024) + lane * 16;
        sb_next = __builtin_amdgcn_readfirstlane(lds0 + stage * STAGE);
    };
    auto dma = [&](int d) {
        if (d < NA) {
            const int q = d >> 2, ks = (d >> 1) & 1, pl = d & 1;
            lds_dma16(pa[q][pl] + ks * pstep[q], sb_next + (((wave * AQ + q) * 2 + ks) * 2 + pl) * 1024);
        } else {
            const int c = d - NA;
            lds_dma16(pw + c * 1024, sb_next + A_BYTES + (wave * 2 * NB + c) * 1024);
        }
    };
    f16x8 fa[2][MB][2], fb[2][NB][2];
    auto frags = [&](int stage, int ks) {
        const char* sa = smem + stage * STAGE;
        const char* sb = sa + A_BYTES;
        #pragma unroll
        for (int i = 0; i < MB; ++i) {
            const char* p = sa + (((wm * MB + i) * 2 + ks) * 2) * 1024 + lane * 16;
            fa[ks][i][0] = *reinterpret_cast<const f16x8*>(p);
            fa[ks][i][1] = *reinterpret_cast<const f16x8*>(p + 1024);
        }
        #pragma unroll
        for (int j = 0; j < NB; ++j) {
            const char* p = sb + (((wn * NB + j) * 2 + ks) * 2) * 1024 + lane * 16;
            fb[ks][j][0] = *reinterpret_cast<const f16x8*>(p);
            fb[ks][j][1] = *reinterpret_cast<const f16x8*>(p + 1024);
        }
    };
    prep(it0, 0);
    #pragma unroll
    for (int d = 0; d < ND; ++d) dma(d);
    for (int it = it0; it < it1; ++it) {
        const int stage = (it - it0) & 1;
        __builtin_amdgcn_s_waitcnt(0x0F70);
        __syncthreads();
        frags(stage, 0);
        prep(it + 1 < it1 ? it + 1 : it, stage ^ 1);
        __builtin_amdgcn_sched_barrier(0);
        #pragma unroll
        for (int ks = 0; ks < 2; ++ks) {
            #pragma unroll
            for (int g = 0; g < PER; ++g) {
                const int prod = g / (MB * NB), i = (g / NB) % MB, j = g % NB;
                acc[i][j] = __builtin_amdgcn_mfma_f32_32x32x16_f16(fa[ks][i][prod == 0 ? 1 : 0], fb[ks][j][prod == 1 ? 1 : 0], acc[i][j], 0, 0, 0);
                if ((g + 1) % GAP == 0) {
                    dma(ks * HALF + g / GAP);
                    __builtin_amdgcn_sched_barrier(0);
                }
                if (ks == 0 && g == PER / 2) {
                    frags(stage, 1);
                    __builtin_amdgcn_sched_barrier(0);
                }
            }
        }
    }
    __builtin_amdgcn_s_waitcnt(0x0F70);
    const float inv = 1.0f / (a.xscale[0] * a.wscale[0]);
    const int oy0 = a.offy[phase], ox0 = a.offx[phase];
    float bj[NB];
    #pragma unroll
    for (int j = 0; j < NB; ++j) bj[j] = a.bias ? a.bias[nt * TN + (wn * NB + j) * 32 + (lane & 31)] : 0.f;
    #pragma unroll
    for (int i = 0; i < MB; ++i) {
        #pragma unroll
        for (int r = 0; r < 16; ++r) {
            const unsigned row = (r & 3) + 8 * (r >> 2) + 4 * (lane >> 5);
            const unsigned m = m0 + (wm * MB + i) * 32 + row;
            const unsigned n = __umulhi(m, a.magHW) >> a.shHW, rem = m - n * HW;
            const unsigned yy = __umulhi(rem, a.magW) >> a.shW, xx = rem - yy * a.W;
            const int64_t opix = ((int64_t)n * a.Hout + (yy * a.out_stride + oy0)) * a.Wout + (xx * a.out_stride + ox0);
            const int64_t oe = opix * a.Cout + nt * TN + wn * NB * 32 + (lane & 31);
            if (KS) {
                float* o = a.partial + (int64_t)blockIdx.z * ((int64_t)a.N * a.Hout * a.Wout * a.Cout) + oe;
                #pragma unroll
                for (int j = 0; j < NB; ++j) o[j * 32] = acc[i][j][r];
            } else {
                float* o = a.y + oe;
                #pragma unroll
                for (int j = 0; j < NB; ++j) {
                    float v = acc[i][j][r] * inv + bj[j];
                    if (a.relu) v = fmaxf(v, 0.f);
                    o[j * 32] = v;
                }
            }
        }
    }
}

__global__ __launch_bounds__(256) void conv_ksplit_reduce_kernel(const float* __restrict__ partial, int ksplit, int64_t n4, int cout,
                                                                 const float* __restrict__ xscale, const float* __restrict__ wscale,
                                                                 const float* __restrict__ bias, int relu, float* __restrict__ y)
{
    const float inv = 1.0f / (xscale[0] * wscale[0]);
    for (int64_t i = (int64_t)blockIdx.x * 256 + threadIdx.x; i < n4; i += (int64_t)gridDim.x * 256) {
        f32x4 v = *reinterpret_cast<const f32x4*>(partial + 4 * i);
        int z = 1;
        for (; z + 3 < ksplit; z += 4) {
            f32x4 t[4];
            #pragma unroll
            for (int u = 0; u < 4; ++u) t[u] = *reinterpret_cast<const f32x4*>(partial + 4 * ((z + u) * n4 + i));
            #pragma unroll
            for (int u = 0; u < 4; ++u) v += t[u];
        }
        for (; z < ksplit; ++z) v += *reinterpret_cast<const f32x4*>(partial + 4 * (z * n4 + i));
        v = v * inv;
        if (bias) v += *reinterpret_cast<const f32x4*>(bias + (4 * i) % cout);
        if (relu) { v[0] = fmaxf(v[0], 0.f); v[1] = fmaxf(v[1], 0.f); v[2] = fmaxf(v[2], 0.f); v[3] = fmaxf(v[3], 0.f); }
        *reinterpret_cast<f32x4*>(y + 4 * i) = v;
    }
}

__device__ __forceinline__ f32x4 split_act(f32x4 v, int relu, float slope)
{
    if (relu == 1) { v[0] = fmaxf(v[0], 0.f); v[1] = fmaxf(v[1], 0.f); v[2] = fmaxf(v[2], 0.f); v[3] = fmaxf(v[3], 0.f); }
    else if (relu == 2) {
        #pragma unroll
        for (int j = 0; j < 4; ++j) v[j] = v[j] > 0.f ? v[j] : slope * v[j];
    }
    return v;
}

constexpr int kAmaxBlocks = 512;

__global__ __launch_bounds__(256) void conv_absmax_kernel(const float* __restrict__ x, int64_t n4, int64_t n, float* __restrict__ partial,
                                                          float* __restrict__ colsum = nullptr, int c4n = 0, float leaky = -1.f)
{
    __shared__ float red[4];
    __shared__ f32x4 red4[256];
    float m = 0.f;
    f32x4 cs = {0.f, 0.f, 0.f, 0.f};
    for (int64_t i = blockIdx.x * 256 + threadIdx.x; i < n4; i += (int64_t)gridDim.x * 256) {
        const f32x4 v = *reinterpret_cast<const f32x4*>(x + 4 * i);
        const f32x4 u = leaky >= 0.f ? split_act(v, 2, leaky) : v;
        m = fmaxf(fmaxf(m, fabsf(u[0])), fmaxf(fabsf(u[1]), fmaxf(fabsf(u[2]), fabsf(u[3]))));
        cs += v;
    }
    if (blockIdx.x == 0 && threadIdx.x == 0) for (int64_t i = 4 * n4; i < n; ++i) m = fmaxf(m, fabsf(x[i]));
    #pragma unroll
    for (int o = 32; o > 0; o >>= 1) m = fmaxf(m, __shfl_xor(m, o));
    if ((threadIdx.x & 63) == 0) red[threadIdx.x >> 6] = m;
    if (colsum) red4[threadIdx.x] = cs;
    __syncthreads();
    if (threadIdx.x == 0) partial[blockIdx.x] = fmaxf(fmaxf(red[0], red[1]), fmaxf(red[2], red[3]));
    if (colsum && (int)threadIdx.x < c4n) {
        f32x4 t = red4[threadIdx.x];
        for (int p = threadIdx.x + c4n; p < 256; p += c4n) t += red4[p];
        *reinterpret_cast<f32x4*>(colsum + (int64_t)blockIdx.x * 4 * c4n + 4 * threadIdx.x) = t;
    }
}

__device__ __forceinline__ float scale_of(const float* __restrict__ partial, float mul = 1.0f, int count = kAmaxBlocks)
{
    float amax = 0.f;
    for (int i = threadIdx.x & 63; i < count; i += 64) amax = fmaxf(amax, partial[i]);
    #pragma unroll
    for (int o = 32; o > 0; o >>= 1) amax = fmaxf(amax, __shfl_xor(amax, o));
    amax *= mul;
    if (!(amax > 0.f) || !(amax < 3.0e38f)) return 1.0f;
    int e;
    (void)frexpf(amax, &e);
    return ldexpf(1.0f, 14 - e);
}

__global__ __launch_bounds__(256) void conv_leaky_bwd_kernel(float* __restrict__ dx, const float* __restrict__ x, int64_t n4, float slope)
{
    for (int64_t i = blockIdx.x * 256 + threadIdx.x; i < n4; i += (int64_t)gridDim.x * 256) {
        f32x4 g = *reinterpret_cast<const f32x4*>(dx + 4 * i);
        const f32x4 v = *reinterpret_cast<const f32x4*>(x + 4 * i);
        #pragma unroll
        for (int j = 0; j < 4; ++j) g[j] = v[j] > 0.f ? g[j] : slope * g[j];
        *reinterpret_cast<f32x4*>(dx + 4 * i) = g;
    }
}

__global__ __launch_bounds__(256) void conv_split_kernel(const float* __restrict__ x, int64_t n4, const float* __restrict__ amax,
                                                         int relu, _Float16* __restrict__ hi, _Float16* __restrict__ lo,
                                                         float* __restrict__ scale_out, float slope = 0.f)
{
    const float s = scale_of(amax);
    if (blockIdx.x == 0 && threadIdx.x == 0) scale_out[0] = s;
    for (int64_t i = blockIdx.x * 256 + threadIdx.x; i < n4; i += (int64_t)gridDim.x * 256) {
        f32x4 v = *reinterpret_cast<const f32x4*>(x + 4 * i);
        v = split_act(v, relu, slope);
        v = v * s;
        f16x4 h, l;
        #pragma unroll
        for (int j = 0; j < 4; ++j) { h[j] = (_Float16)v[j]; l[j] = (_Float16)(v[j] - (float)h[j]); }
        *reinterpret_cast<f16x4*>(hi + 4 * i) = h;
        *reinterpret_cast<f16x4*>(lo + 4 * i) = l;
    }
}

constexpr float kHistMargin = 64.0f;
constexpr int kHistArray = 2 * kAmaxBlocks;

__device__ __forceinline__ float scale_for(float amax)
{
    if (!(amax > 0.f) || !(amax < 3.0e38f)) return 1.0f;
    int e;
    (void)frexpf(amax, &e);
    return ldexpf(1.0f, 14 - e);
}

__global__ __launch_bounds__(kAmaxBlocks) void conv_hist_seed_kernel(float* __restrict__ hist)
{
    const float m = hist[threadIdx.x];
    __syncthreads();
    typedef float f32x2h __attribute__((ext_vector_type(2)));
    f32x2h a = {m, __builtin_bit_cast(float, 1u)}, b = {0.f, __builtin_bit_cast(float, 0u)};
    *reinterpret_cast<f32x2h*>(hist + 2 * threadIdx.x) = a;
    *reinterpret_cast<f32x2h*>(hist + kHistArray + 2 * threadIdx.x) = b;
    __shared__ float red[kAmaxBlocks / 64];
    float mm = m;
    #pragma unroll
    for (int o = 32; o > 0; o >>= 1) mm = fmaxf(mm, __shfl_xor(mm, o));
    if ((threadIdx.x & 63) == 0) red[threadIdx.x >> 6] = mm;
    __syncthreads();
    if (threadIdx.x == 0) {
        float t = 0.f;
        for (int i = 0; i < kAmaxBlocks / 64; ++i) t = fmaxf(t, red[i]);
        hist[2 * kHistArray + 2] = t; hist[2 * kHistArray + 3] = t;
    }
}

__global__ __launch_bounds__(256) void conv_split_hist_kernel(const float* __restrict__ x, int64_t n4, int relu, _Float16* __restrict__ hi,
                                                              _Float16* __restrict__ lo, float* __restrict__ scale_out,
                                                              float* __restrict__ hist, float* __restrict__ colsum, int c4n,
                                                              float slope = 0.f)
{
    __shared__ float red[4];
    __shared__ f32x4 red4[256];
    typedef float f32x2h __attribute__((ext_vector_type(2)));
    typedef int i32x2h __attribute__((ext_vector_type(2)));
    float mx[2] = {0.f, 0.f};
    int tlo[2] = {0x7fffffff, 0x7fffffff}, thi[2] = {0, 0};
    #pragma unroll
    for (int arr = 0; arr < 2; ++arr)
        #pragma unroll
        for (int i = 0; i < kAmaxBlocks / 64; ++i) {
            const i32x2h p = *reinterpret_cast<const i32x2h*>(hist + arr * kHistArray + 2 * ((threadIdx.x & 63) + 64 * i));
            mx[arr] = fmaxf(mx[arr], __builtin_bit_cast(float, p[0]));
            tlo[arr] = min(tlo[arr], p[1]);
            thi[arr] = max(thi[arr], p[1]);
        }
    #pragma unroll
    for (int o = 32; o > 0; o >>= 1)
        #pragma unroll
        for (int arr = 0; arr < 2; ++arr) {
            mx[arr] = fmaxf(mx[arr], __shfl_xor(mx[arr], o));
            tlo[arr] = min(tlo[arr], __shfl_xor(tlo[arr], o));
            thi[arr] = max(thi[arr], __shfl_xor(thi[arr], o));
        }
    const bool ok0 = tlo[0] == thi[0], ok1 = tlo[1] == thi[1];
    const int src = (ok1 && (!ok0 || thi[1] > thi[0])) ? 1 : 0;
    const int tag = (src ? thi[1] : thi[0]) + 1;
    const float prev = src ? mx[1] : mx[0];
    const float assumed = prev > 0.f ? prev : hist[2 * kHistArray + 2 + src];
    const float s = scale_for(assumed * kHistMargin);
    if (blockIdx.x == 0 && threadIdx.x == 0) { scale_out[0] = s; hist[2 * kHistArray + 2 + (1 - src)] = assumed; }
    float m = 0.f;
    f32x4 cs = {0.f, 0.f, 0.f, 0.f};
    for (int64_t i = blockIdx.x * 256 + threadIdx.x; i < n4; i += (int64_t)gridDim.x * 256) {
        f32x4 v = *reinterpret_cast<const f32x4*>(x + 4 * i);
        cs += v;
        v = split_act(v, relu, slope);
        m = fmaxf(fmaxf(m, fabsf(v[0])), fmaxf(fabsf(v[1]), fmaxf(fabsf(v[2]), fabsf(v[3]))));
        v = v * s;
        f16x4 h, l;
        #pragma unroll
        for (int j = 0; j < 4; ++j) { h[j] = (_Float16)v[j]; l[j] = (_Float16)(v[j] - (float)h[j]); }
        *reinterpret_cast<f16x4*>(hi + 4 * i) = h;
        *reinterpret_cast<f16x4*>(lo + 4 * i) = l;
    }
    #pragma unroll
    for (int o = 32; o > 0; o >>= 1) m = fmaxf(m, __shfl_xor(m, o));
    if ((threadIdx.x & 63) == 0) red[threadIdx.x >> 6] = m;
    if (colsum) red4[threadIdx.x] = cs;
    __syncthreads();
    if (threadIdx.x == 0) {
        const f32x2h p = {fmaxf(fmaxf(red[0], red[1]), fmaxf(red[2], red[3])), __builtin_bit_cast(float, tag)};
        *reinterpret_cast<f32x2h*>(hist + (1 - src) * kHistArray + 2 * blockIdx.x) = p;
    }
    if (colsum && (int)threadIdx.x < c4n) {
        f32x4 t = red4[threadIdx.x];
        for (int p = threadIdx.x + c4n; p < 256; p += c4n) t += red4[p];
        *reinterpret_cast<f32x4*>(colsum + (int64_t)blockIdx.x * 4 * c4n + 4 * threadIdx.x) = t;
    }
}

constexpr int kHistRedoWord = 2 * kHistArray;
__global__ __launch_bounds__(256) void conv_split_redo_kernel(const float* __restrict__ x, int64_t n4, int relu, _Float16* __restrict__ hi,
                                                              _Float16* __restrict__ lo, float* __restrict__ scale_out,
                                                              float* __restrict__ hist, float slope = 0.f)
{
    typedef int i32x2h __attribute__((ext_vector_type(2)));
    float mx[2] = {0.f, 0.f};
    int tg[2] = {0, 0};
    #pragma unroll
    for (int arr = 0; arr < 2; ++arr)
        #pragma unroll
        for (int i = 0; i < kAmaxBlocks / 64; ++i) {
            const i32x2h p = *reinterpret_cast<const i32x2h*>(hist + arr * kHistArray + 2 * ((threadIdx.x & 63) + 64 * i));
            mx[arr] = fmaxf(mx[arr], __builtin_bit_cast(float, p[0]));
            tg[arr] = max(tg[arr], p[1]);
        }
    #pragma unroll
    for (int o = 32; o > 0; o >>= 1)
        #pragma unroll
        for (int arr = 0; arr < 2; ++arr) {
            mx[arr] = fmaxf(mx[arr], __shfl_xor(mx[arr], o));
            tg[arr] = max(tg[arr], __shfl_xor(tg[arr], o));
        }
    const int now = tg[1] > tg[0] ? 1 : 0;
    const float own = mx[now], assumed = hist[2 * kHistArray + 2 + now];
    const float s_used = scale_for(assumed * kHistMargin);
    const float top = own * s_used;
    const bool fine = !(own > 0.f) || !(own < 3.0e38f) || (top >= 0.03125f && top < 65504.0f);
    if (fine) return;
    const float s = scale_for(own);
    if (blockIdx.x == 0 && threadIdx.x == 0) {
        scale_out[0] = s;
        reinterpret_cast<unsigned*>(hist)[kHistRedoWord] += 1u;
    }
    for (int64_t i = blockIdx.x * 256 + threadIdx.x; i < n4; i += (int64_t)gridDim.x * 256) {
        f32x4 v = *reinterpret_cast<const f32x4*>(x + 4 * i);
        v = split_act(v, relu, slope);
        v = v * s;
        f16x4 h, l;
        #pragma unroll
        for (int j = 0; j < 4; ++j) { h[j] = (_Float16)v[j]; l[j] = (_Float16)(v[j] - (float)h[j]); }
        *reinterpret_cast<f16x4*>(hi + 4 * i) = h;
        *reinterpret_cast<f16x4*>(lo + 4 * i) = l;
    }
}

struct WeightArgs {
    const float* w; int64_t sk, sn, sr, ss;
    const float* amax; float* scale_out; char* img;
    int K, Nn, ntaps, nphase;
    int64_t n4;
    float coef, bound_mul;
    int amax_count;
    signed char nsrc[kMaxPhase][kMaxTaps];
    signed char r[kMaxPhase][kMaxTaps][4], s[kMaxPhase][kMaxTaps][4];
};

__device__ __forceinline__ void conv_weights_body(const WeightArgs& a, const int bid, const int nblocks)
{
    float sc;
    if (a.amax) sc = scale_of(a.amax, a.bound_mul, a.amax_count);
    else {
        __shared__ float red[4];
        float m = 0.f;
        for (int64_t i = threadIdx.x; i < a.n4; i += 256) {
            const f32x4 v = *reinterpret_cast<const f32x4*>(a.w + 4 * i);
            m = fmaxf(fmaxf(m, fabsf(v[0])), fmaxf(fabsf(v[1]), fmaxf(fabsf(v[2]), fabsf(v[3]))));
        }
        #pragma unroll
        for (int o = 32; o > 0; o >>= 1) m = fmaxf(m, __shfl_xor(m, o));
        if ((threadIdx.x & 63) == 0) red[threadIdx.x >> 6] = m;
        __syncthreads();
        m = fmaxf(fmaxf(red[0], red[1]), fmaxf(red[2], red[3])) * a.bound_mul;
        sc = 1.0f;
        if (m > 0.f && m < 3.0e38f) { int e; (void)frexpf(m, &e); sc = ldexpf(1.0f, 14 - e); }
    }
    if (bid == 0 && threadIdx.x == 0) a.scale_out[0] = sc;
    const int nchunk = a.K >> 5, nblk = a.Nn >> 5;
    const int64_t groups = (int64_t)a.nphase * a.ntaps * nchunk * nblk * 2 * 64;
    for (int64_t g = (int64_t)bid * 256 + threadIdx.x; g < groups; g += (int64_t)nblocks * 256) {
        const int lane = g & 63;
        int64_t t = g >> 6;
        const int ks = t & 1; t >>= 1;
        const int nb = t % nblk; t /= nblk;
        const int ch = t % nchunk; t /= nchunk;
        const int tap = t % a.ntaps; const int ph = t / a.ntaps;
        const int n = nb * 32 + (lane & 31);
        const int k0 = ch * 32 + ks * 16 + (lane >> 5) * 8;
        const float* base = a.w + n * a.sn;
        const int ns = a.nsrc[ph][tap];
        float acc8[8] = {0.f, 0.f, 0.f, 0.f, 0.f, 0.f, 0.f, 0.f};
        for (int m = 0; m < ns; ++m) {
            const float* src = base + a.r[ph][tap][m] * a.sr + a.s[ph][tap][m] * a.ss;
            #pragma unroll
            for (int j = 0; j < 8; ++j) acc8[j] += src[(k0 + j) * a.sk];
        }
        const float cs = a.coef * sc;
        f16x8 h, l;
        #pragma unroll
        for (int j = 0; j < 8; ++j) {
            const float v = acc8[j] * cs;
            h[j] = (_Float16)v; l[j] = (_Float16)(v - (float)h[j]);
        }
        char* dst = a.img + (((((int64_t)(ph * a.ntaps + tap) * nchunk + ch) * nblk + nb) * 2 + ks) * 2) * 1024 + lane * 16;
        *reinterpret_cast<f16x8*>(dst) = h;
        *reinterpret_cast<f16x8*>(dst + 1024) = l;
    }
}

__global__ __launch_bounds__(256) void conv_weights_kernel(WeightArgs a) { conv_weights_body(a, blockIdx.x, gridDim.x); }

__global__ __launch_bounds__(256) void conv_weights_pair_kernel(WeightArgs a, WeightArgs b, int blocks_a)
{
    if ((int)blockIdx.x < blocks_a) conv_weights_body(a, blockIdx.x, blocks_a);
    else conv_weights_body(b, blockIdx.x - blocks_a, gridDim.x - blocks_a);
}

struct WrwOperand {
    const _Float16* hi; const _Float16* lo;
    int Hp, Wp, C, stride;
    signed char dy[kMaxPhase][kMaxTaps], dx[kMaxPhase][kMaxTaps];
};

struct WrwArgs {
    WrwOperand A, B;
    const _Float16* zero;
    float* partial;
    int N, H, W, ntaps, nphase;
    unsigned magHW, shHW, magW, shW;
    int nchunks, cps;
};

typedef short s16x4v __attribute__((__vector_size__(4 * sizeof(short))));

__device__ __forceinline__ f16x8 tr_read8(const char* block, int lane_off)
{
    auto p = (__attribute__((address_space(3))) s16x4v*)((__attribute__((address_space(3))) char*)(block + lane_off));
    auto q = (__attribute__((address_space(3))) s16x4v*)((__attribute__((address_space(3))) char*)(block + lane_off + 256));
    const s16x4v a = __builtin_amdgcn_ds_read_tr16_b64_v4i16(p);
    const s16x4v b = __builtin_amdgcn_ds_read_tr16_b64_v4i16(q);
    typedef short s16x8v __attribute__((__vector_size__(8 * sizeof(short))));
    const s16x8v ab = __builtin_shufflevector(a, b, 0, 1, 2, 3, 4, 5, 6, 7);
    return __builtin_bit_cast(f16x8, ab);
}

template <int MB, int NB>
__global__ __launch_bounds__(256) void conv_wrw_kernel(WrwArgs a)
{
    extern __shared__ __attribute__((aligned(16))) char smem[];
    constexpr int TA = 64 * MB, TB = 64 * NB;
    constexpr int A_BYTES = 2 * MB * 4 * 1024, B_BYTES = 2 * NB * 4 * 1024, STAGE = A_BYTES + B_BYTES;
    constexpr int AQ = (2 * MB) / 4, BQ = (2 * NB) / 4;
    constexpr bool ONE = MB == 1 && NB == 1;
    static_assert(ONE || (MB >= 2 && NB >= 2), "a wave stages whole blocks of both operands, or one block of one");

    const int tid = threadIdx.x, lane = tid & 63;
    const int wave = __builtin_amdgcn_readfirstlane(tid >> 6);
    const int wm = wave >> 1, wn = wave & 1;
    const int nta = a.A.C / TA, ntb = a.B.C / TB;
    int idx = blockIdx.y;
    const int tb = idx % ntb; idx /= ntb;
    const int ta = idx % nta; idx /= nta;
    const int tap = idx % a.ntaps, phase = idx / a.ntaps;
    const int c0 = blockIdx.x * a.cps, c1 = min(c0 + a.cps, a.nchunks);
    const int dya = a.A.dy[phase][tap], dxa = a.A.dx[phase][tap], dyb = a.B.dy[phase][tap], dxb = a.B.dx[phase][tap];
    const unsigned HW = a.H * a.W;
    const unsigned lds0 = (unsigned)(size_t)((__attribute__((address_space(3))) char*)smem);
    const int c8 = (lane & 3) * 8;

    auto issue = [&](int c, int stage) {
        const unsigned sbase = __builtin_amdgcn_readfirstlane(lds0 + stage * STAGE);
        #pragma unroll
        for (int s = 0; s < 2; ++s) {
            const unsigned m = c * 32 + s * 16 + (lane >> 2);
            const unsigned n = __umulhi(m, a.magHW) >> a.shHW, rem = m - n * HW;
            const unsigned yy = __umulhi(rem, a.magW) >> a.shW, xx = rem - yy * a.W;
            const int ay = yy * a.A.stride + dya, ax = xx * a.A.stride + dxa;
            const int by = yy * a.B.stride + dyb, bx = xx * a.B.stride + dxb;
            const bool oka = (unsigned)ay < (unsigned)a.A.Hp && (unsigned)ax < (unsigned)a.A.Wp;
            const bool okb = (unsigned)by < (unsigned)a.B.Hp && (unsigned)bx < (unsigned)a.B.Wp;
            const int64_t ea = ((int64_t)((n * a.A.Hp + ay) * a.A.Wp + ax)) * a.A.C + ta * TA + c8;
            const int64_t eb = ((int64_t)((n * a.B.Hp + by) * a.B.Wp + bx)) * a.B.C + tb * TB + c8;
            #pragma unroll
            for (int q = 0; q < AQ; ++q) {
                const int b = wave * AQ + q;
                const _Float16* ph = oka ? a.A.hi + ea + b * 32 : a.zero + c8;
                const _Float16* pl = oka ? a.A.lo + ea + b * 32 : a.zero + c8;
                const unsigned l = sbase + ((b * 2 + s) * 2) * 1024;
                lds_dma16(ph, l);
                lds_dma16(pl, l + 1024);
            }
            #pragma unroll
            for (int q = 0; q < BQ; ++q) {
                const int b = wave * BQ + q;
                const _Float16* ph = okb ? a.B.hi + eb + b * 32 : a.zero + c8;
                const _Float16* pl = okb ? a.B.lo + eb + b * 32 : a.zero + c8;
                const unsigned l = sbase + A_BYTES + ((b * 2 + s) * 2) * 1024;
                lds_dma16(ph, l);
                lds_dma16(pl, l + 1024);
            }
        }
    };

    f32x16 acc[MB][NB];
    #pragma unroll
    for (int i = 0; i < MB; ++i)
        #pragma unroll
        for (int j = 0; j < NB; ++j)
            #pragma unroll
            for (int r = 0; r < 16; ++r) acc[i][j][r] = 0.f;

    const int tr_off = ((lane >> 5) * 8 + ((lane & 15) >> 2)) * 64 + (((lane >> 4) & 1) * 16 + (lane & 3) * 4) * 2;

    constexpr int NA = ONE ? 4 : AQ * 4, ND = ONE ? 4 : NA + BQ * 4, HALF = ND / 2, PER = 3 * MB * NB, GAP = ONE ? 1 : PER / HALF;
    static_assert(ONE || PER % HALF == 0, "DMAs spread evenly");
    const char* pA[2][2]; const char* pB[2][2];
    int stA[2], stB[2];
    unsigned sb_next = 0;
    auto prep = [&](int c, int stage) {
        #pragma unroll
        for (int s = 0; s < 2; ++s) {
            const unsigned m = c * 32 + s * 16 + (lane >> 2);
            const unsigned n = __umulhi(m, a.magHW) >> a.shHW, rem = m - n * HW;
            const unsigned yy = __umulhi(rem, a.magW) >> a.shW, xx = rem - yy * a.W;
            if constexpr (ONE) {
                const bool isb = wave >= 2;
                const int py = isb ? yy * a.B.stride + dyb : yy * a.A.stride + dya, px = isb ? xx * a.B.stride + dxb : xx * a.A.stride + dxa;
                const int Hp = isb ? a.B.Hp : a.A.Hp, Wp = isb ? a.B.Wp : a.A.Wp, Cc = isb ? a.B.C : a.A.C;
                const bool okp = (unsigned)py < (unsigned)Hp && (unsigned)px < (unsigned)Wp;
                const int64_t ep = ((int64_t)((n * Hp + py) * Wp + px)) * Cc + (isb ? tb * TB : ta * TA) + (wave & 1) * 32 + c8;
                pA[s][0] = reinterpret_cast<const char*>(okp ? (isb ? a.B.hi : a.A.hi) + ep : a.zero + c8);
                pA[s][1] = reinterpret_cast<const char*>(okp ? (isb ? a.B.lo : a.A.lo) + ep : a.zero + c8);
                continue;
            }
            const int ay = yy * a.A.stride + dya, ax = xx * a.A.stride + dxa;
            const int by = yy * a.B.stride + dyb, bx = xx * a.B.stride + dxb;
            const bool oka = (unsigned)ay < (unsigned)a.A.Hp && (unsigned)ax < (unsigned)a.A.Wp;
            const bool okb = (unsigned)by < (unsigned)a.B.Hp && (unsigned)bx < (unsigned)a.B.Wp;
            const int64_t ea = ((int64_t)((n * a.A.Hp + ay) * a.A.Wp + ax)) * a.A.C + ta * TA + wave * (AQ * 32) + c8;
            const int64_t eb = ((int64_t)((n * a.B.Hp + by) * a.B.Wp + bx)) * a.B.C + tb * TB + wave * (BQ * 32) + c8;
            pA[s][0] = reinterpret_cast<const char*>(oka ? a.A.hi + ea : a.zero + c8);
            pA[s][1] = reinterpret_cast<const char*>(oka ? a.A.lo + ea : a.zero + c8);
            pB[s][0] = reinterpret_cast<const char*>(okb ? a.B.hi + eb : a.zero + c8);
            pB[s][1] = reinterpret_cast<const char*>(okb ? a.B.lo + eb : a.zero + c8);
            stA[s] = oka ? 64 : 0; stB[s] = okb ? 64 : 0;
        }
        sb_next = __builtin_amdgcn_readfirstlane(lds0 + stage * STAGE);
    };
    auto dma = [&](int d) {
        if constexpr (ONE) {
            lds_dma16(pA[d >> 1][d & 1], sb_next + (((wave * 2) + (d >> 1)) * 2 + (d & 1)) * 1024);
        } else if (d < NA) {
            const int s = d / (AQ * 2), q = (d >> 1) % AQ, pl = d & 1;
            lds_dma16(pA[s][pl] + q * stA[s], sb_next + (((wave * AQ + q) * 2 + s) * 2 + pl) * 1024);
        } else {
            const int e = d - NA;
            const int s = e / (BQ * 2), q = (e >> 1) % BQ, pl = e & 1;
            lds_dma16(pB[s][pl] + q * stB[s], sb_next + A_BYTES + (((wave * BQ + q) * 2 + s) * 2 + pl) * 1024);
        }
    };
    f16x8 fa[2][MB][2], fb[2][NB][2];
    auto frags = [&](int stage, int ks) {
        const char* sa = smem + stage * STAGE;
        const char* sb = sa + A_BYTES;
        #pragma unroll
        for (int i = 0; i < MB; ++i) {
            const char* p = sa + (((wm * MB + i) * 2 + ks) * 2) * 1024;
            fa[ks][i][0] = tr_read8(p, tr_off);
            fa[ks][i][1] = tr_read8(p + 1024, tr_off);
        }
        #pragma unroll
        for (int j = 0; j < NB; ++j) {
            const char* p = sb + (((wn * NB + j) * 2 + ks) * 2) * 1024;
            fb[ks][j][0] = tr_read8(p, tr_off);
            fb[ks][j][1] = tr_read8(p + 1024, tr_off);
        }
    };
    if (c0 < c1) {
        prep(c0, 0);
        #pragma unroll
        for (int d = 0; d < ND; ++d) dma(d);
    }
    for (int c = c0; c < c1; ++c) {
        const int stage = (c - c0) & 1;
        __builtin_amdgcn_s_waitcnt(0x0F70);
        __syncthreads();
        frags(stage, 0);
        prep(c + 1 < c1 ? c + 1 : c, stage ^ 1);
        __builtin_amdgcn_sched_barrier(0);
        #pragma unroll
        for (int ks = 0; ks < 2; ++ks) {
            #pragma unroll
            for (int g = 0; g < PER; ++g) {
                const int prod = g / (MB * NB), i = (g / NB) % MB, j = g % NB;
                acc[i][j] = __builtin_amdgcn_mfma_f32_32x32x16_f16(fa[ks][i][prod == 0 ? 1 : 0], fb[ks][j][prod == 1 ? 1 : 0], acc[i][j], 0, 0, 0);
                if ((g + 1) % GAP == 0 && g / GAP < HALF) {
                    dma(ks * HALF + g / GAP);
                    __builtin_amdgcn_sched_barrier(0);
                }
                if (ks == 0 && g == PER / 2) {
                    frags(stage, 1);
                    __builtin_amdgcn_sched_barrier(0);
                }
            }
        }
    }
    __builtin_amdgcn_s_waitcnt(0x0F70);

    const int slice = phase * a.ntaps + tap, nslice = a.nphase * a.ntaps;
    float* out = a.partial + ((int64_t)blockIdx.x * nslice + slice) * a.A.C * a.B.C;
    #pragma unroll
    for (int i = 0; i < MB; ++i)
        #pragma unroll
        for (int r = 0; r < 16; ++r) {
            const int ci = ta * TA + (wm * MB + i) * 32 + (r & 3) + 8 * (r >> 2) + 4 * (lane >> 5);
            float* o = out + (int64_t)ci * a.B.C + tb * TB + wn * NB * 32 + (lane & 31);
            #pragma unroll
            for (int j = 0; j < NB; ++j) o[j * 32] = acc[i][j][r];
        }
}

struct WrwReduceArgs {
    const float* partial; int splits, nslice, Ca, Cb;
    const float* xscale; const float* gscale;
    float* dw; int64_t sa, sb, sr, ss;
    float coef;
    const float* colsum; float* db; int c4n, main_blocks;
    int nout;
    signed char r[kMaxTaps], s[kMaxTaps], cnt[kMaxTaps], slice[kMaxTaps][4];
};

__global__ __launch_bounds__(256) void conv_wrw_reduce_kernel(WrwReduceArgs a)
{
    if ((int)blockIdx.x >= a.main_blocks) {
        const int u = ((int)blockIdx.x - a.main_blocks) * 256 + threadIdx.x, cg = u >> 6, lane = u & 63;
        if (cg >= a.c4n) return;
        f32x4 v = {0.f, 0.f, 0.f, 0.f};
        for (int b = lane; b < kAmaxBlocks; b += 64) v += *reinterpret_cast<const f32x4*>(a.colsum + (int64_t)b * 4 * a.c4n + 4 * cg);
        #pragma unroll
        for (int j = 0; j < 4; ++j)
            #pragma unroll
            for (int o = 1; o < 64; o <<= 1) v[j] += __shfl_xor(v[j], o);
        if (lane == 0) *reinterpret_cast<f32x4*>(a.db + 4 * cg) = v;
        return;
    }
    const int64_t plane = (int64_t)a.Ca * a.Cb, per = (int64_t)a.nslice * plane, total4 = (int64_t)a.nout * plane >> 2;
    const float inv = a.coef / (a.xscale[0] * a.gscale[0]);
    const int part = threadIdx.x & 3;
    for (int64_t e4 = ((int64_t)blockIdx.x * 256 + threadIdx.x) >> 2; e4 < total4; e4 += (int64_t)a.main_blocks * 64) {
        const int64_t e = e4 * 4;
        const int o = e / plane; const int64_t w = e - o * plane;
        f32x4 v = {0.f, 0.f, 0.f, 0.f};
        for (int i = 0; i < a.cnt[o]; ++i) {
            const float* src = a.partial + a.slice[o][i] * plane + w;
            int sp = part;
            for (; sp + 28 < a.splits; sp += 32) {
                f32x4 t[8];
                #pragma unroll
                for (int u = 0; u < 8; ++u) t[u] = *reinterpret_cast<const f32x4*>(src + (int64_t)(sp + 4 * u) * per);
                #pragma unroll
                for (int u = 0; u < 8; ++u) v += t[u];
            }
            for (; sp < a.splits; sp += 4) v += *reinterpret_cast<const f32x4*>(src + sp * per);
        }
        #pragma unroll
        for (int j = 0; j < 4; ++j) { v[j] += __shfl_xor(v[j], 1); v[j] += __shfl_xor(v[j], 2); }
        if (part != 0) continue;
        v = v * inv;
        const int cb = w % a.Cb, ca = w / a.Cb;
        float* out = a.dw + ca * a.sa + cb * a.sb + a.r[o] * a.sr + a.s[o] * a.ss;
        if (a.sb == 1 && ((uintptr_t)out & 15) == 0) *reinterpret_cast<f32x4*>(out) = v;
        else { out[0] = v[0]; out[a.sb] = v[1]; out[2 * a.sb] = v[2]; out[3 * a.sb] = v[3]; }
    }
}

struct NarrowWrwArgs {
    const float* x; const float* gy; float* partial;
    int N, H, W, Cin, Cout, ks, nrow;
    unsigned magHW, shHW, magW, shW;
    int64_t M; int64_t pix_per_wave;
};

__global__ __launch_bounds__(512, 1) void conv_wrw_narrow_kernel(NarrowWrwArgs a)
{
    extern __shared__ __attribute__((aligned(16))) float nw_part[];
    const int tid = threadIdx.x, lane = tid & 63;
    const int wave = __builtin_amdgcn_readfirstlane(tid >> 6);
    const int i = lane & 31, k = lane >> 5;
    const int grp = blockIdx.y;
    const bool is_tap = i < a.nrow, is_one = i == a.nrow;
    int dy = 0, dx = 0, c = 0;
    if (is_tap) {
        const int tap = i / a.Cin;
        c = i - tap * a.Cin;
        dy = tap / a.ks - a.ks / 2; dx = tap % a.ks - a.ks / 2;
    }
    const unsigned HW = (unsigned)(a.H * a.W);
    f32x16 acc[4];
#pragma unroll
    for (int q = 0; q < 4; ++q)
#pragma unroll
        for (int r = 0; r < 16; ++r) acc[q][r] = 0.f;
    const int64_t p0 = ((int64_t)blockIdx.x * 8 + wave) * a.pix_per_wave;
    int64_t p1 = p0 + a.pix_per_wave;
    if (p1 > a.M) p1 = a.M;
    const float* gyc = a.gy + grp * 128 + (grp * 128 + 4 * i < a.Cout ? 4 * i : 0);
    constexpr int U = 8;
    for (int64_t p = p0; p < p1; p += 2 * U) {
        float av[U]; f32x4 bv[U];
#pragma unroll
        for (int u = 0; u < U; ++u) {
            const int64_t pp = p + 2 * u + k;
            const bool ok = pp < p1;
            const unsigned pc = (unsigned)(ok ? pp : a.M - 1);
            const unsigned n = __umulhi(pc, a.magHW) >> a.shHW, rem = pc - n * HW;
            const unsigned yy = __umulhi(rem, a.magW) >> a.shW, xx = rem - yy * a.W;
            const int iy = (int)yy + dy, ix = (int)xx + dx;
            const bool inb = ok && is_tap && (unsigned)iy < (unsigned)a.H && (unsigned)ix < (unsigned)a.W;
            const float xv = a.x[inb ? ((int64_t)(n * a.H + iy) * a.W + ix) * a.Cin + c : 0];
            av[u] = inb ? xv : ((ok && is_one) ? 1.f : 0.f);
            bv[u] = *reinterpret_cast<const f32x4*>(gyc + (int64_t)pc * a.Cout);
        }
#pragma unroll
        for (int u = 0; u < U; ++u)
#pragma unroll
            for (int q = 0; q < 4; ++q) acc[q] = __builtin_amdgcn_mfma_f32_32x32x2f32(av[u], bv[u][q], acc[q], 0, 0, 0);
    }
#pragma unroll
    for (int q = 0; q < 4; ++q)
#pragma unroll
        for (int r = 0; r < 16; ++r) nw_part[((wave * 4 + q) * 16 + r) * 64 + lane] = acc[q][r];
    __syncthreads();
    float* out = a.partial + ((int64_t)blockIdx.y * gridDim.x + blockIdx.x) * 4096;
#pragma unroll
    for (int m = 0; m < 8; ++m) {
        const int e = tid + 512 * m;
        float sum = nw_part[e];
#pragma unroll
        for (int w = 1; w < 8; ++w) sum += nw_part[w * 4096 + e];
        out[e] = sum;
    }
}

__global__ __launch_bounds__(256) void conv_wrw_narrow_reduce_kernel(const float* __restrict__ partial, int nparts, int Cin, int ks, int nrow,
                                                                     float* __restrict__ dw, int64_t sk, int64_t sn, int64_t sr, int64_t ss,
                                                                     float* __restrict__ db, int Cout)
{
    __shared__ float red[8][32];
    const int el = threadIdx.x & 31, pg = threadIdx.x >> 5;
    const int e = blockIdx.x * 32 + el;
    const float* p = partial + (int64_t)blockIdx.y * nparts * 4096 + e;
    float sum = 0.f;
    int z = pg;
    for (; z + 8 * 15 < nparts; z += 8 * 16) {
        float v[16];
#pragma unroll
        for (int u = 0; u < 16; ++u) v[u] = p[(int64_t)(z + 8 * u) * 4096];
#pragma unroll
        for (int u = 0; u < 16; ++u) sum += v[u];
    }
    for (; z < nparts; z += 8) sum += p[(int64_t)z * 4096];
    red[pg][el] = sum;
    __syncthreads();
    if (pg != 0) return;
#pragma unroll
    for (int g = 1; g < 8; ++g) sum += red[g][el];
    const int q = e >> 10, r = (e >> 6) & 15, ln = e & 63;
    const int row = (r & 3) + 8 * (r >> 2) + 4 * (ln >> 5);
    const int o = blockIdx.y * 128 + 4 * (ln & 31) + q;
    if (o >= Cout) return;
    if (row < nrow) {
        const int tap = row / Cin, c = row - tap * Cin;
        dw[c * sk + o * sn + (tap / ks) * sr + (tap % ks) * ss] = sum;
    } else if (row == nrow && db) db[o] = sum;
}

struct NarrowFwdArgs {
    const float* x; const float* w; const float* bias; float* y;
    int N, H, W, Cin, Cout, ks, nrow, relu;
    int64_t sk, sn, sr, ss;
    unsigned magHW, shHW, magW, shW;
    int64_t M; int ntiles, tiles_per_wave;
    signed char tdy[32], tdx[32], tch[32], tr[32], ts[32];
};

constexpr int kNarrowLd = 32 * 2 + 4;
constexpr int kNarrowNQ = 2;
template <int KS>
__global__ __launch_bounds__(256, 2) void conv_fwd_narrow_kernel(NarrowFwdArgs a)
{
    __shared__ __attribute__((aligned(16))) float nf_tile[4 * 32 * kNarrowLd];
    const int tid = threadIdx.x, lane = tid & 63;
    const int wave = __builtin_amdgcn_readfirstlane(tid >> 6);
    const int i = lane & 31, k = lane >> 5;
    const int grp = blockIdx.y;
    __shared__ float nf_w[32][32 * kNarrowNQ];
    __shared__ int nf_tab[32][2];
#pragma unroll
    for (int j = 0; j < 8; ++j) {
        const int m = wave + 4 * j;
        const int kind = m < a.nrow ? 0 : (m == a.nrow ? 1 : 2);
        const int o = grp * (32 * kNarrowNQ) + lane;
        float v = 0.f;
        if (kind == 0) v = a.w[a.tch[m] * a.sk + o * a.sn + a.tr[m] * a.sr + a.ts[m] * a.ss];
        else if (kind == 1) v = a.bias ? a.bias[o] : 0.f;
        nf_w[m][lane] = v;
        if (lane == 0) {
            const int dy = a.tdy[m], dx = a.tdx[m];
            nf_tab[m][0] = (dy & 0xff) | ((dx & 0xff) << 8) | (kind << 16);
            nf_tab[m][1] = (dy * a.W + dx) * a.Cin + a.tch[m];
        }
    }
    __syncthreads();
    int dyx[KS], off[KS]; float bw[KS][kNarrowNQ];
#pragma unroll
    for (int s = 0; s < KS; ++s) {
        const int m = 2 * s + k;
        dyx[s] = nf_tab[m][0];
        off[s] = nf_tab[m][1];
#pragma unroll
        for (int q = 0; q < kNarrowNQ; ++q) bw[s][q] = nf_w[m][q * 32 + i];
    }
    const unsigned HW = (unsigned)(a.H * a.W);
    const int t0 = (blockIdx.x * 4 + wave) * a.tiles_per_wave;
    int t1 = t0 + a.tiles_per_wave;
    if (t1 > a.ntiles) t1 = a.ntiles;
    auto gather = [&](int t, float (&av)[KS]) __attribute__((always_inline)) {
        const int64_t p = (int64_t)t * 32 + i;
        const unsigned pc = (unsigned)(p < a.M ? p : a.M - 1);
        const unsigned n = __umulhi(pc, a.magHW) >> a.shHW, rem = pc - n * HW;
        const unsigned yy = __umulhi(rem, a.magW) >> a.shW, xx = rem - yy * a.W;
        const int pb = (int)pc * a.Cin;
#pragma unroll
        for (int s = 0; s < KS; ++s) {
            const int dy = (signed char)(dyx[s] & 0xff), dx = (signed char)((dyx[s] >> 8) & 0xff), kind = dyx[s] >> 16;
            const bool inb = kind == 0 && (unsigned)((int)yy + dy) < (unsigned)a.H && (unsigned)((int)xx + dx) < (unsigned)a.W;
            const float xv = a.x[inb ? pb + off[s] : 0];
            av[s] = inb ? xv : (kind == 1 ? 1.f : 0.f);
        }
    };
    float av[KS], an[KS];
    if (t0 < t1) gather(t0, av);
    for (int t = t0; t < t1; ++t) {
        if (t + 1 < t1) gather(t + 1, an);
        f32x16 acc[kNarrowNQ];
#pragma unroll
        for (int q = 0; q < kNarrowNQ; ++q)
#pragma unroll
            for (int r = 0; r < 16; ++r) acc[q][r] = 0.f;
#pragma unroll
        for (int s = 0; s < KS; ++s)
#pragma unroll
            for (int q = 0; q < kNarrowNQ; ++q) acc[q] = __builtin_amdgcn_mfma_f32_32x32x2f32(av[s], bw[s][q], acc[q], 0, 0, 0);
        float* tl = nf_tile + wave * (32 * kNarrowLd);
#pragma unroll
        for (int r = 0; r < 16; ++r) {
            const int row = (r & 3) + 8 * (r >> 2) + 4 * k;
#pragma unroll
            for (int q = 0; q < kNarrowNQ; ++q) {
                float v = acc[q][r];
                if (a.relu) v = fmaxf(v, 0.f);
                tl[row * kNarrowLd + q * 32 + i] = v;
            }
        }
        __builtin_amdgcn_s_waitcnt(0xc07f);
#pragma unroll
        for (int j = 0; j < 8; ++j) {
            const int row = 4 * j + (lane >> 4);
            const int64_t pr = (int64_t)t * 32 + row;
            const f32x4 v = *reinterpret_cast<const f32x4*>(tl + row * kNarrowLd + 4 * (lane & 15));
            if (pr < a.M) *reinterpret_cast<f32x4*>(a.y + pr * a.Cout + grp * (32 * kNarrowNQ) + 4 * (lane & 15)) = v;
        }
#pragma unroll
        for (int s = 0; s < KS; ++s) av[s] = an[s];
    }
}

void magic_u31(unsigned d, unsigned* mag, unsigned* sh)
{
    unsigned s = 0;
    while ((1u << s) < d) ++s;
    const unsigned long long num = 1ull << (31 + s);
    *mag = (unsigned)((num + d - 1) / d);
    *sh = s - 1;
}

int grid_for(int64_t work_items)
{
    int64_t g = (work_items + 255) / 256;
    return (int)(g < 1 ? 1 : (g > 2048 ? 2048 : g));
}

template <int MB, int NB, bool KS = false>
hipError_t launch_conv(const ConvArgs& a, hipStream_t st)
{
    constexpr int LDS = 2 * (2 * MB * 4 * 1024 + 2 * NB * 4 * 1024);
    hipError_t e = wc_set_max_lds(reinterpret_cast<const void*>(conv_f16x3_kernel<MB, NB, KS>), LDS);
    if (e != hipSuccess) return e;
    const int64_t M = (int64_t)a.N * a.H * a.W;
    dim3 grid((unsigned)(M / (64 * MB)), (unsigned)(a.nphase * (a.Cout / (64 * NB))), (unsigned)a.ksplit);
    hipLaunchKernelGGL((conv_f16x3_kernel<MB, NB, KS>), grid, dim3(256), LDS, st, a);
    return hipGetLastError();
}

}

extern "C" {

static int split_measured(const float* x, int64_t n, int relu, float slope, void* hi, void* lo, float* scale, void* amax_scratch,
                          float* colsum_partials, int C, hipStream_t st)
{
    if (!x || !hi || !lo || !scale || !amax_scratch || n <= 0 || (n & 3)) return WC_ERR_ARG;
    if (colsum_partials && (C <= 0 || (C & 3) || 256 % (C >> 2) != 0 || n % C != 0)) return WC_ERR_SHAPE;
    hipLaunchKernelGGL(conv_absmax_kernel, dim3(kAmaxBlocks), dim3(256), 0, st, x, n / 4, n, (float*)amax_scratch,
                       colsum_partials, colsum_partials ? C >> 2 : 0, relu == 2 ? slope : -1.f);
    hipLaunchKernelGGL(conv_split_kernel, dim3(grid_for(n / 4)), dim3(256), 0, st, x, n / 4, (const float*)amax_scratch, relu,
                       (_Float16*)hi, (_Float16*)lo, scale, slope);
    return (int)hipGetLastError();
}

static int split_hist(const float* x, int64_t n, int relu, float slope, void* hi, void* lo, float* scale, float* colsum_partials, int C,
                      float* hist, int bootstrap, hipStream_t st)
{
    if (!x || !hi || !lo || !scale || !hist || n <= 0 || (n & 3)) return WC_ERR_ARG;
    if (colsum_partials && (C <= 0 || (C & 3) || 256 % (C >> 2) != 0 || n % C != 0)) return WC_ERR_SHAPE;
    if (bootstrap & 1) {
        hipLaunchKernelGGL(conv_absmax_kernel, dim3(kAmaxBlocks), dim3(256), 0, st, x, n / 4, n, hist, colsum_partials, colsum_partials ? C >> 2 : 0,
                           relu == 2 ? slope : -1.f);
        hipLaunchKernelGGL(conv_split_kernel, dim3(grid_for(n / 4)), dim3(256), 0, st, x, n / 4, (const float*)hist, relu, (_Float16*)hi,
                           (_Float16*)lo, scale, slope);
        hipLaunchKernelGGL(conv_hist_seed_kernel, dim3(1), dim3(kAmaxBlocks), 0, st, hist);
        return (int)hipGetLastError();
    }
    hipLaunchKernelGGL(conv_split_hist_kernel, dim3(kAmaxBlocks), dim3(256), 0, st, x, n / 4, relu, (_Float16*)hi, (_Float16*)lo, scale,
                       hist, colsum_partials, colsum_partials ? C >> 2 : 0, slope);
    if (!(bootstrap & 2)) {
        const unsigned g2 = grid_for(n / 4) < 64u ? grid_for(n / 4) : 64u;
        hipLaunchKernelGGL(conv_split_redo_kernel, dim3(g2), dim3(256), 0, st, x, n / 4, relu, (_Float16*)hi, (_Float16*)lo, scale, hist, slope);
    }
    return (int)hipGetLastError();
}

int wc_conv_split_f32(const float* x, int64_t n, int relu, void* hi, void* lo, float* scale, void* amax_scratch, wc_stream_t stream)
{
    return wc_conv_split_colsum_f32(x, n, relu, hi, lo, scale, amax_scratch, nullptr, 0, stream);
}

int wc_conv_split_colsum_f32(const float* x, int64_t n, int relu, void* hi, void* lo, float* scale, void* amax_scratch,
                             float* colsum_partials, int C, wc_stream_t stream)
{
    return split_measured(x, n, relu ? 1 : 0, 0.f, hi, lo, scale, amax_scratch, colsum_partials, C, (hipStream_t)stream);
}

int wc_conv_split_hist_f32(const float* x, int64_t n, int relu, void* hi, void* lo, float* scale, float* colsum_partials, int C,
                           float* hist, int bootstrap, wc_stream_t stream)
{
    return split_hist(x, n, relu ? 1 : 0, 0.f, hi, lo, scale, colsum_partials, C, hist, bootstrap, (hipStream_t)stream);
}

int wc_conv_split_leaky_f32(const float* x, int64_t n, float negative_slope, void* hi, void* lo, float* scale, void* amax_scratch,
                            float* colsum_partials, int C, wc_stream_t stream)
{
    if (!(negative_slope >= 0.f && negative_slope <= 1.f)) return WC_ERR_ARG;
    return split_measured(x, n, negative_slope == 0.f ? 1 : 2, negative_slope, hi, lo, scale, amax_scratch, colsum_partials, C, (hipStream_t)stream);
}

int wc_conv_split_hist_leaky_f32(const float* x, int64_t n, float negative_slope, void* hi, void* lo, float* scale, float* colsum_partials, int C,
                                 float* hist, int bootstrap, wc_stream_t stream)
{
    if (!(negative_slope >= 0.f && negative_slope <= 1.f)) return WC_ERR_ARG;
    return split_hist(x, n, negative_slope == 0.f ? 1 : 2, negative_slope, hi, lo, scale, colsum_partials, C, hist, bootstrap, (hipStream_t)stream);
}

int wc_conv_leaky_bwd_f32(float* dx, const float* x, int64_t n, float negative_slope, wc_stream_t stream)
{
    if (!dx || !x || n <= 0 || (n & 3)) return WC_ERR_ARG;
    hipLaunchKernelGGL(conv_leaky_bwd_kernel, dim3(grid_for(n / 4)), dim3(256), 0, (hipStream_t)stream, dx, x, n / 4, negative_slope);
    return (int)hipGetLastError();
}

size_t wc_conv_weights_bytes(const wc_conv_geom* g)
{
    if (!g) return 0;
    return (size_t)g->nphase * g->ntaps * g->Cin * g->Cout * 4;
}

static int fill_weight_args(WeightArgs& a, const float* w, int64_t stride_k, int64_t stride_n, int64_t stride_r, int64_t stride_s,
                            int64_t n_elems, const wc_conv_geom* g, void* image, float* scale, const float* amax, int amax_count)
{
    if (g->ntaps < 1 || g->ntaps > kMaxTaps || g->nphase < 1 || g->nphase > kMaxPhase || (g->Cin & 31) || (g->Cout & 31)) return WC_ERR_ARG;
    a.w = w; a.sk = stride_k; a.sn = stride_n; a.sr = stride_r; a.ss = stride_s;
    a.amax = amax; a.amax_count = amax_count; a.scale_out = scale; a.img = (char*)image;
    a.n4 = n_elems / 4;
    a.K = g->Cin; a.Nn = g->Cout; a.ntaps = g->ntaps; a.nphase = g->nphase;
    int most = 1;
    for (int p = 0; p < kMaxPhase; ++p)
        for (int t = 0; t < kMaxTaps; ++t) {
            a.nsrc[p][t] = g->nsrc[p][t];
            if (p < g->nphase && t < g->ntaps) {
                if (g->nsrc[p][t] < 1 || g->nsrc[p][t] > 4) return WC_ERR_ARG;
                if (g->nsrc[p][t] > most) most = g->nsrc[p][t];
            }
            for (int m = 0; m < 4; ++m) { a.r[p][t][m] = g->wr[p][t][m]; a.s[p][t][m] = g->ws[p][t][m]; }
        }
    a.coef = g->wcoef; a.bound_mul = fabsf(g->wcoef) * most;
    return WC_OK;
}

int wc_conv_weights_f32(const float* w, int64_t stride_k, int64_t stride_n, int64_t stride_r, int64_t stride_s, int64_t n_elems,
                        const wc_conv_geom* g, void* image, float* scale, void* amax_scratch,
                        const float* known_amax, int known_count, wc_stream_t stream)
{
    hipStream_t st = (hipStream_t)stream;
    if (!w || !g || !image || !scale || (!amax_scratch && !known_amax) || n_elems <= 0) return WC_ERR_ARG;
    if (known_amax && (known_count < 1 || known_count > 4096)) return WC_ERR_ARG;
    const bool inline_max = !known_amax && n_elems <= 32768 && (n_elems & 3) == 0 && ((uintptr_t)w & 15) == 0;
    if (!inline_max && !known_amax) hipLaunchKernelGGL(conv_absmax_kernel, dim3(kAmaxBlocks), dim3(256), 0, st, w, n_elems / 4, n_elems, (float*)amax_scratch);
    WeightArgs a;
    const int rc = fill_weight_args(a, w, stride_k, stride_n, stride_r, stride_s, n_elems, g, image, scale,
                                    inline_max ? nullptr : (known_amax ? known_amax : (const float*)amax_scratch), known_amax ? known_count : kAmaxBlocks);
    if (rc != WC_OK) return rc;
    const int64_t groups = (int64_t)g->nphase * g->ntaps * (g->Cin >> 5) * (g->Cout >> 5) * 128;
    hipLaunchKernelGGL(conv_weights_kernel, dim3(grid_for(groups)), dim3(256), 0, st, a);
    return (int)hipGetLastError();
}

int wc_conv_weights_pair_f32(const float* w, int64_t stride_r, int64_t stride_s, int64_t n_elems,
                             int64_t a_stride_k, int64_t a_stride_n, const wc_conv_geom* ga, void* image_a,
                             int64_t b_stride_k, int64_t b_stride_n, const wc_conv_geom* gb, void* image_b,
                             float* scale, void* amax_scratch, const float* known_amax, int known_count, wc_stream_t stream)
{
    hipStream_t st = (hipStream_t)stream;
    if (!w || !ga || !gb || !image_a || !image_b || !scale || (!amax_scratch && !known_amax) || n_elems <= 0) return WC_ERR_ARG;
    if (known_amax && (known_count < 1 || known_count > 4096)) return WC_ERR_ARG;
    if (!known_amax) hipLaunchKernelGGL(conv_absmax_kernel, dim3(kAmaxBlocks), dim3(256), 0, st, w, n_elems / 4, n_elems, (float*)amax_scratch);
    const float* amax = known_amax ? known_amax : (const float*)amax_scratch;
    const int cnt = known_amax ? known_count : kAmaxBlocks;
    WeightArgs a, b;
    int rc = fill_weight_args(a, w, a_stride_k, a_stride_n, stride_r, stride_s, n_elems, ga, image_a, scale, amax, cnt);
    if (rc != WC_OK) return rc;
    rc = fill_weight_args(b, w, b_stride_k, b_stride_n, stride_r, stride_s, n_elems, gb, image_b, scale + 1, amax, cnt);
    if (rc != WC_OK) return rc;
    if (a.bound_mul != b.bound_mul) return WC_ERR_ARG;
    const int blocks_a = grid_for((int64_t)ga->nphase * ga->ntaps * (ga->Cin >> 5) * (ga->Cout >> 5) * 128);
    const int blocks_b = grid_for((int64_t)gb->nphase * gb->ntaps * (gb->Cin >> 5) * (gb->Cout >> 5) * 128);
    hipLaunchKernelGGL(conv_weights_pair_kernel, dim3(blocks_a + blocks_b), dim3(256), 0, st, a, b, blocks_a);
    return (int)hipGetLastError();
}

int wc_conv_supported(const wc_conv_geom* g)
{
    if (!g) return 0;
    if (g->ntaps < 1 || g->ntaps > kMaxTaps || g->nphase < 1 || g->nphase > kMaxPhase) return 0;
    if ((g->Cin & 31) || (g->Cout & 63)) return 0;
    const int64_t M = (int64_t)g->N * g->H * g->W;
    if (M <= 0 || (M & 127) || M > (int64_t)1 << 31) return 0;
    if ((int64_t)g->N * g->Hin * g->Win > (int64_t)1 << 31) return 0;
    if (g->W < 2 || g->H < 1) return 0;
    return 1;
}

constexpr int kKsplitMaxWgs = 96;
constexpr int kKsplitTargetWgs = 256;
constexpr int kWrwTargetWgs = 512;

static int conv_ksplit(const wc_conv_geom* g)
{
    const int64_t M = (int64_t)g->N * g->H * g->W;
    const bool wide = (g->Cout % 256) == 0;
    const int64_t wgs = (M / 128) * g->nphase * (g->Cout / (wide ? 256 : (g->Cout % 128) ? 64 : 128));
    const int iters = g->ntaps * (g->Cin / 32);
    if (wgs > kKsplitMaxWgs || iters < 8) return 1;
    int k = (int)((kKsplitTargetWgs + wgs - 1) / wgs);
    if (k > iters / 4) k = iters / 4;
    return k < 1 ? 1 : (k > 8 ? 8 : k);
}

size_t wc_conv_workspace_bytes(const wc_conv_geom* g)
{
    if (!g) return 0;
    const int k = conv_ksplit(g);
    return k > 1 ? (size_t)k * g->N * g->Hout * g->Wout * g->Cout * 4 : 0;
}

int wc_conv_f16x3(const void* xhi, const void* xlo, const float* xscale, const void* wimage, const float* wscale,
                  const float* bias, const void* zero_line, const wc_conv_geom* g, int relu, float* y,
                  void* ws, size_t ws_bytes, wc_stream_t stream)
{
    hipStream_t st = (hipStream_t)stream;
    if (!xhi || !xlo || !xscale || !wimage || !wscale || !zero_line || !g || !y) return WC_ERR_ARG;
    if (!wc_conv_supported(g)) return WC_ERR_SHAPE;
    ConvArgs a;
    a.xhi = (const _Float16*)xhi; a.xlo = (const _Float16*)xlo; a.zero = (const _Float16*)zero_line;
    a.wimg = (const char*)wimage; a.xscale = xscale; a.wscale = wscale; a.bias = bias; a.y = y;
    a.N = g->N; a.H = g->H; a.W = g->W; a.Hin = g->Hin; a.Win = g->Win; a.Cin = g->Cin; a.Cout = g->Cout;
    a.in_stride = g->in_stride; a.ntaps = g->ntaps; a.nphase = g->nphase; a.Hout = g->Hout; a.Wout = g->Wout;
    a.out_stride = g->out_stride; a.relu = relu;
    a.ksplit = conv_ksplit(g); a.partial = (float*)ws;
    magic_u31((unsigned)(g->H * g->W), &a.magHW, &a.shHW);
    magic_u31((unsigned)g->W, &a.magW, &a.shW);
    if (a.ksplit > 1 && (!ws || ws_bytes < wc_conv_workspace_bytes(g))) return WC_ERR_WORKSPACE;
    for (int p = 0; p < kMaxPhase; ++p) {
        a.offy[p] = g->off_y[p]; a.offx[p] = g->off_x[p];
        for (int t = 0; t < kMaxTaps; ++t) { a.dy[p][t] = g->dy[p][t]; a.dx[p][t] = g->dx[p][t]; }
    }
    const int64_t M = (int64_t)g->N * g->H * g->W;
    const bool wide = (g->Cout % 256) == 0;
    const int64_t wgs_big = (M / 256) * g->nphase * (g->Cout / (wide ? 256 : 128));
    hipError_t e;
    if (g->Cout % 128)                                      e = a.ksplit > 1 ? launch_conv<2, 1, true>(a, st) : launch_conv<2, 1>(a, st);
    else if (a.ksplit == 1 && (M % 256) == 0 && wgs_big >= 256) e = wide ? launch_conv<4, 4>(a, st) : launch_conv<4, 2>(a, st);
    else if (a.ksplit > 1)                                  e = wide ? launch_conv<2, 4, true>(a, st) : launch_conv<2, 2, true>(a, st);
    else                                                    e = wide ? launch_conv<2, 4>(a, st) : launch_conv<2, 2>(a, st);
    if (e != hipSuccess) return (int)e;
    if (a.ksplit > 1) {
        const int64_t n4 = (int64_t)g->N * g->Hout * g->Wout * g->Cout / 4;
        hipLaunchKernelGGL(conv_ksplit_reduce_kernel, dim3(grid_for(n4)), dim3(256), 0, st, (const float*)ws, a.ksplit, n4, g->Cout,
                           xscale, wscale, bias, relu, y);
    }
    return (int)hipGetLastError();
}

static int wrw_splits(const wc_conv_geom* g, int* tile)
{
    const bool wide = (g->Cin % 256 == 0) && (g->Cout % 256 == 0) && g->nphase * g->ntaps * (g->Cin / 256) * (g->Cout / 256) >= 4;
    *tile = wide ? 256 : ((g->Cin % 128) || (g->Cout % 128)) ? 64 : 128;
    const int tiles = g->nphase * g->ntaps * (g->Cin / *tile) * (g->Cout / *tile);
    const int64_t nchunks = (int64_t)g->N * g->H * g->W / 32;
    int splits = kWrwTargetWgs / tiles / 8 * 8;
    if (splits < 8) splits = 8;
    if (splits > 64) splits = 64;
    if (splits > nchunks) splits = (int)nchunks;
    return splits < 1 ? 1 : splits;
}

int wc_conv_wrw_narrow_supported(int64_t N, int64_t H, int64_t W, int Cin, int Cout, int ksize);
int wc_conv_narrow64_supported(int64_t N, int64_t H, int64_t W, int Cin, int Cout, int ksize);

int wc_conv_fwd_narrow_f32(const float* x, const float* w, int64_t stride_k, int64_t stride_n, int64_t stride_r, int64_t stride_s,
                           const float* bias, int64_t N, int64_t H, int64_t W, int Cin, int Cout, int ksize, int relu, float* y, wc_stream_t stream)
{
    if (!x || !w || !y) return WC_ERR_ARG;
    if (!wc_conv_narrow64_supported(N, H, W, Cin, Cout, ksize) || N * H * W * Cin >= ((int64_t)1 << 31)) return WC_ERR_SHAPE;
    hipStream_t st = (hipStream_t)stream;
    NarrowFwdArgs a = {};
    a.x = x; a.w = w; a.bias = bias; a.y = y;
    a.N = (int)N; a.H = (int)H; a.W = (int)W; a.Cin = Cin; a.Cout = Cout; a.ks = ksize; a.nrow = ksize * ksize * Cin; a.relu = relu;
    a.sk = stride_k; a.sn = stride_n; a.sr = stride_r; a.ss = stride_s;
    magic_u31((unsigned)(H * W), &a.magHW, &a.shHW);
    magic_u31((unsigned)W, &a.magW, &a.shW);
    for (int m = 0; m < 32; ++m) {
        const int tap = m < a.nrow ? m / Cin : 0, c = m < a.nrow ? m % Cin : 0;
        a.tr[m] = (signed char)(tap / ksize); a.ts[m] = (signed char)(tap % ksize); a.tch[m] = (signed char)c;
        a.tdy[m] = (signed char)(tap / ksize - ksize / 2); a.tdx[m] = (signed char)(tap % ksize - ksize / 2);
    }
    a.M = N * H * W;
    a.ntiles = (int)((a.M + 31) / 32);
    a.tiles_per_wave = (a.ntiles + 1023) / 1024;
    if (a.tiles_per_wave < 1) a.tiles_per_wave = 1;
    const int nwg = (a.ntiles + 4 * a.tiles_per_wave - 1) / (4 * a.tiles_per_wave);
    const int ks2 = (a.nrow + 2) / 2;
    dim3 grid(nwg, Cout / (32 * kNarrowNQ));
    if (ks2 <= 2) hipLaunchKernelGGL(conv_fwd_narrow_kernel<2>, grid, dim3(256), 0, st, a);
    else if (ks2 <= 5) hipLaunchKernelGGL(conv_fwd_narrow_kernel<5>, grid, dim3(256), 0, st, a);
    else if (ks2 <= 10) hipLaunchKernelGGL(conv_fwd_narrow_kernel<10>, grid, dim3(256), 0, st, a);
    else if (ks2 <= 14) hipLaunchKernelGGL(conv_fwd_narrow_kernel<14>, grid, dim3(256), 0, st, a);
    else hipLaunchKernelGGL(conv_fwd_narrow_kernel<16>, grid, dim3(256), 0, st, a);
    return (int)hipGetLastError();
}

static int64_t narrow_wrw_parts(int64_t M, int64_t* pix_per_wave)
{
    int64_t ppw = (M + 256 * 8 - 1) / (256 * 8);
    if (ppw < 16) ppw = 16;
    ppw = (ppw + 1) & ~(int64_t)1;
    *pix_per_wave = ppw;
    return (M + 8 * ppw - 1) / (8 * ppw);
}

int wc_conv_narrow64_supported(int64_t N, int64_t H, int64_t W, int Cin, int Cout, int ksize)
{
    if (N <= 0 || H <= 0 || W <= 0 || Cin <= 0 || Cout <= 0 || (ksize != 1 && ksize != 3)) return 0;
    if (ksize * ksize * Cin >= 32 || (Cout & 63)) return 0;
    return N * H * W < ((int64_t)1 << 31) ? 1 : 0;
}

int wc_conv_wrw_narrow_supported(int64_t N, int64_t H, int64_t W, int Cin, int Cout, int ksize)
{
    return ((Cout & 127) == 0 && wc_conv_narrow64_supported(N, H, W, Cin, Cout, ksize)) ? 1 : 0;
}

size_t wc_conv_wrw_narrow64_workspace_bytes(int64_t N, int64_t H, int64_t W, int Cin, int Cout, int ksize)
{
    if (!wc_conv_narrow64_supported(N, H, W, Cin, Cout, ksize)) return 0;
    int64_t ppw;
    return (size_t)narrow_wrw_parts(N * H * W, &ppw) * ((Cout + 127) / 128) * 4096 * sizeof(float);
}

size_t wc_conv_wrw_narrow_workspace_bytes(int64_t N, int64_t H, int64_t W, int Cin, int Cout, int ksize)
{
    return wc_conv_wrw_narrow_supported(N, H, W, Cin, Cout, ksize) ? wc_conv_wrw_narrow64_workspace_bytes(N, H, W, Cin, Cout, ksize) : 0;
}

int wc_conv_wrw_narrow64_f32(const float* x, const float* gy, int64_t N, int64_t H, int64_t W, int Cin, int Cout, int ksize,
                             float* dw, int64_t stride_k, int64_t stride_n, int64_t stride_r, int64_t stride_s, float* db,
                             void* ws, size_t ws_bytes, wc_stream_t stream)
{
    if (!x || !gy || !dw || !ws) return WC_ERR_ARG;
    if (!wc_conv_narrow64_supported(N, H, W, Cin, Cout, ksize)) return WC_ERR_SHAPE;
    if (ws_bytes < wc_conv_wrw_narrow64_workspace_bytes(N, H, W, Cin, Cout, ksize)) return WC_ERR_WORKSPACE;
    hipStream_t st = (hipStream_t)stream;
    NarrowWrwArgs a = {};
    a.x = x; a.gy = gy; a.partial = (float*)ws;
    a.N = (int)N; a.H = (int)H; a.W = (int)W; a.Cin = Cin; a.Cout = Cout; a.ks = ksize; a.nrow = ksize * ksize * Cin;
    magic_u31((unsigned)(H * W), &a.magHW, &a.shHW);
    magic_u31((unsigned)W, &a.magW, &a.shW);
    a.M = N * H * W;
    const int nparts = (int)narrow_wrw_parts(a.M, &a.pix_per_wave);
    const int ngrp = (Cout + 127) / 128;
    constexpr int lds = 8 * 4096 * 4;
    hipError_t e = wc_set_max_lds(reinterpret_cast<const void*>(conv_wrw_narrow_kernel), lds);
    if (e != hipSuccess) return (int)e;
    hipLaunchKernelGGL(conv_wrw_narrow_kernel, dim3(nparts, ngrp), dim3(512), lds, st, a);
    hipLaunchKernelGGL(conv_wrw_narrow_reduce_kernel, dim3(128, ngrp), dim3(256), 0, st, (const float*)ws, nparts, Cin, ksize, a.nrow,
                       dw, stride_k, stride_n, stride_r, stride_s, db, Cout);
    return (int)hipGetLastError();
}

int wc_conv_wrw_narrow_f32(const float* x, const float* gy, int64_t N, int64_t H, int64_t W, int Cin, int Cout, int ksize,
                           float* dw, int64_t stride_k, int64_t stride_n, int64_t stride_r, int64_t stride_s, float* db,
                           void* ws, size_t ws_bytes, wc_stream_t stream)
{
    if (!x || !gy || !dw || !ws) return WC_ERR_ARG;
    if (!wc_conv_wrw_narrow_supported(N, H, W, Cin, Cout, ksize)) return WC_ERR_SHAPE;
    return wc_conv_wrw_narrow64_f32(x, gy, N, H, W, Cin, Cout, ksize, dw, stride_k, stride_n, stride_r, stride_s, db, ws, ws_bytes, stream);
}

size_t wc_conv_wrw_workspace_bytes(const wc_conv_geom* g)
{
    if (!g) return 0;
    int tile;
    return (size_t)wrw_splits(g, &tile) * g->nphase * g->ntaps * g->Cin * g->Cout * 4;
}

int wc_conv_wrw_f16x3(const void* xhi, const void* xlo, const float* xscale, const void* ghi, const void* glo, const float* gscale,
                      const void* zero_line, const wc_conv_geom* g, float* dw, int64_t stride_k, int64_t stride_n,
                      int64_t stride_r, int64_t stride_s, void* ws, size_t ws_bytes, wc_stream_t stream)
{
    return wc_conv_wrw_bias_f16x3(xhi, xlo, xscale, ghi, glo, gscale, zero_line, g, dw, stride_k, stride_n, stride_r, stride_s,
                                  nullptr, nullptr, ws, ws_bytes, stream);
}

int wc_conv_wrw_bias_f16x3(const void* xhi, const void* xlo, const float* xscale, const void* ghi, const void* glo, const float* gscale,
                           const void* zero_line, const wc_conv_geom* g, float* dw, int64_t stride_k, int64_t stride_n,
                           int64_t stride_r, int64_t stride_s, const float* colsum_partials, float* db,
                           void* ws, size_t ws_bytes, wc_stream_t stream)
{
    hipStream_t st = (hipStream_t)stream;
    if (!xhi || !xlo || !xscale || !ghi || !glo || !gscale || !zero_line || !g || !dw || !ws) return WC_ERR_NULL;
    if (!wc_conv_supported(g) || (g->Cin & 63) || g->W < 2 || g->H * g->W < 2) return WC_ERR_SHAPE;
    if (ws_bytes < wc_conv_wrw_workspace_bytes(g)) return WC_ERR_WORKSPACE;
    int T;
    int splits = wrw_splits(g, &T);
    const int64_t M = (int64_t)g->N * g->H * g->W;
    const int nslice = g->nphase * g->ntaps;
    const int tiles = nslice * (g->Cin / T) * (g->Cout / T);
    const int nchunks = (int)(M / 32);
    WrwOperand X, G;
    X.hi = (const _Float16*)xhi; X.lo = (const _Float16*)xlo; X.Hp = g->Hin; X.Wp = g->Win; X.C = g->Cin; X.stride = g->in_stride;
    G.hi = (const _Float16*)ghi; G.lo = (const _Float16*)glo; G.Hp = g->Hout; G.Wp = g->Wout; G.C = g->Cout; G.stride = g->out_stride;
    WrwReduceArgs r;
    r.nout = 0; r.coef = g->wcoef;
    for (int p = 0; p < kMaxPhase; ++p)
        for (int t = 0; t < kMaxTaps; ++t) {
            X.dy[p][t] = g->dy[p][t]; X.dx[p][t] = g->dx[p][t];
            G.dy[p][t] = g->off_y[p]; G.dx[p][t] = g->off_x[p];
            if (p >= g->nphase || t >= g->ntaps) continue;
            if (g->nsrc[p][t] < 1 || g->nsrc[p][t] > 4) return WC_ERR_ARG;
            for (int m = 0; m < g->nsrc[p][t]; ++m) {
                int o = 0;
                while (o < r.nout && (r.r[o] != g->wr[p][t][m] || r.s[o] != g->ws[p][t][m])) ++o;
                if (o == r.nout) {
                    if (r.nout == kMaxTaps) return WC_ERR_ARG;
                    r.r[o] = g->wr[p][t][m]; r.s[o] = g->ws[p][t][m]; r.cnt[o] = 0; ++r.nout;
                }
                if (r.cnt[o] == 4) return WC_ERR_ARG;
                r.slice[o][r.cnt[o]++] = (signed char)(p * g->ntaps + t);
            }
        }
    const bool x_cols = stride_k == 1;
    WrwArgs a;
    a.A = x_cols ? G : X; a.B = x_cols ? X : G;
    a.zero = (const _Float16*)zero_line; a.partial = (float*)ws;
    a.N = g->N; a.H = g->H; a.W = g->W; a.ntaps = g->ntaps; a.nphase = g->nphase;
    magic_u31((unsigned)(g->H * g->W), &a.magHW, &a.shHW);
    magic_u31((unsigned)g->W, &a.magW, &a.shW);
    a.nchunks = nchunks; a.cps = (nchunks + splits - 1) / splits;
    splits = (nchunks + a.cps - 1) / a.cps;
    dim3 grid((unsigned)splits, (unsigned)tiles);
    hipError_t e = hipSuccess;
    if (T == 256) {
        constexpr int LDS = 2 * (2 * 4 * 4 * 1024 + 2 * 4 * 4 * 1024);
        e = wc_set_max_lds(reinterpret_cast<const void*>(conv_wrw_kernel<4, 4>), LDS);
        if (e != hipSuccess) return (int)e;
        hipLaunchKernelGGL((conv_wrw_kernel<4, 4>), grid, dim3(256), LDS, st, a);
    } else if (T == 64) {
        constexpr int LDS = 2 * (2 * 1 * 4 * 1024 + 2 * 1 * 4 * 1024);
        e = wc_set_max_lds(reinterpret_cast<const void*>(conv_wrw_kernel<1, 1>), LDS);
        if (e != hipSuccess) return (int)e;
        hipLaunchKernelGGL((conv_wrw_kernel<1, 1>), grid, dim3(256), LDS, st, a);
    } else {
        constexpr int LDS = 2 * (2 * 2 * 4 * 1024 + 2 * 2 * 4 * 1024);
        e = wc_set_max_lds(reinterpret_cast<const void*>(conv_wrw_kernel<2, 2>), LDS);
        if (e != hipSuccess) return (int)e;
        hipLaunchKernelGGL((conv_wrw_kernel<2, 2>), grid, dim3(256), LDS, st, a);
    }
    r.partial = (const float*)ws; r.splits = splits; r.nslice = nslice; r.Ca = a.A.C; r.Cb = a.B.C;
    r.xscale = xscale; r.gscale = gscale; r.dw = dw;
    r.sa = x_cols ? stride_n : stride_k; r.sb = x_cols ? stride_k : stride_n; r.sr = stride_r; r.ss = stride_s;
    if ((colsum_partials == nullptr) != (db == nullptr)) return WC_ERR_NULL;
    if (db && ((g->Cout & 3) || 256 % (g->Cout >> 2) != 0)) return WC_ERR_SHAPE;
    r.colsum = colsum_partials; r.db = db; r.c4n = db ? g->Cout >> 2 : 0;
    r.main_blocks = grid_for((int64_t)r.nout * g->Cin * g->Cout);
    const int extra = db ? (r.c4n * 64 + 255) / 256 : 0;
    hipLaunchKernelGGL(conv_wrw_reduce_kernel, dim3(r.main_blocks + extra), dim3(256), 0, st, r);
    return (int)hipGetLastError();
}

}
```

Baseline: 3607 images/sec.

## Fuse conv data-grad and weight-grad into one paired backward launch

```diff
diff --git a/include/wc_hip.h b/include/wc_hip.h
--- a/include/wc_hip.h
+++ b/include/wc_hip.h
@@ -324,6 +324,14 @@
                            int64_t stride_n, int64_t stride_r, int64_t stride_s, const float* colsum_partials, float* db,
                            void* ws, size_t ws_bytes, wc_stream_t stream);
 
+int    wc_conv_bwd_pair_supported(const wc_conv_geom* gd, const wc_conv_geom* gf);
+size_t wc_conv_bwd_pair_workspace_bytes(const wc_conv_geom* gd, const wc_conv_geom* gf);
+int    wc_conv_bwd_pair_f16x3(const void* ghi, const void* glo, const float* gscale, const void* wimage, const float* wscale,
+                              const void* zero_line, const wc_conv_geom* gd, float* dx, void* ws_dx, size_t ws_dx_bytes,
+                              const void* xhi, const void* xlo, const float* xscale, const wc_conv_geom* gf, float* dw,
+                              int64_t stride_k, int64_t stride_n, int64_t stride_r, int64_t stride_s,
+                              const float* colsum_partials, float* db, void* ws_dw, size_t ws_dw_bytes, wc_stream_t stream);
+
 int wc_stream_copy_f32(const float* src, float* dst, int64_t n, wc_stream_t stream);
 
 
diff --git a/wc_gan_amd/_lib.py b/wc_gan_amd/_lib.py
--- a/wc_gan_amd/_lib.py
+++ b/wc_gan_amd/_lib.py
@@ -154,6 +154,11 @@
     "wc_conv_workspace_bytes": (c_size_t, [c_void_p]),
     "wc_conv_f16x3": (c_int, [c_void_p, c_void_p, c_void_p, c_void_p, c_void_p, c_void_p, c_void_p, c_void_p, c_int,
                               c_void_p, c_void_p, c_size_t, c_void_p]),
+    "wc_conv_bwd_pair_supported": (c_int, [c_void_p, c_void_p]),
+    "wc_conv_bwd_pair_workspace_bytes": (c_size_t, [c_void_p, c_void_p]),
+    "wc_conv_bwd_pair_f16x3": (c_int, [c_void_p, c_void_p, c_void_p, c_void_p, c_void_p, c_void_p, c_void_p, c_void_p, c_void_p, c_size_t,
+                                       c_void_p, c_void_p, c_void_p, c_void_p, c_void_p, c_int64, c_int64, c_int64, c_int64,
+                                       c_void_p, c_void_p, c_void_p, c_size_t, c_void_p]),
     "wc_std_stats_workspace_bytes": (c_size_t, [c_int64, c_int, c_int]),
     "wc_std_stats_f32": (c_int, [c_void_p, c_int64, c_int, c_int, c_void_p, c_void_p, c_void_p, c_size_t, c_void_p]),
     "wc_std_factor_f64": (c_int, [c_void_p, c_void_p, c_int64, c_int, c_int, c_double, c_double, c_int, c_int, c_void_p, c_void_p,
diff --git a/wc_gan_amd/conv.py b/wc_gan_amd/conv.py
--- a/wc_gan_amd/conv.py
+++ b/wc_gan_amd/conv.py
@@ -88,7 +88,7 @@
 
 
 class _Plan:
-    __slots__ = ('ok', 'fwd', 'bwd', 'fwd_ws', 'bwd_ws', 'wrw_ws', 'fwd_ptr', 'bwd_ptr')
+    __slots__ = ('ok', 'fwd', 'bwd', 'fwd_ws', 'bwd_ws', 'wrw_ws', 'fwd_ptr', 'bwd_ptr', 'pair')
 
     def __init__(self, kind, N, H, W, wshape):
         class _W:
@@ -101,6 +101,7 @@
         self.fwd_ws = lib.wc_conv_workspace_bytes(self.fwd_ptr) if self.ok else 0
         self.bwd_ws = lib.wc_conv_workspace_bytes(self.bwd_ptr) if self.ok else 0
         self.wrw_ws = lib.wc_conv_wrw_workspace_bytes(self.fwd_ptr) if self.ok else 0
+        self.pair = self.ok and bool(lib.wc_conv_bwd_pair_supported(self.bwd_ptr, self.fwd_ptr))
 
 
 _plans = {}
@@ -324,6 +325,29 @@
     return dw
 
 
+def backward_pair(g_planes, image, x_planes, plan, w, colsum=None):
+    lib = _lib.load()
+    gh, gl, gs = g_planes[:3]
+    xh, xl, xs = x_planes
+    img, ws = image
+    gf, kf, nf = plan.fwd
+    gb = plan.bwd[0]
+    dx = torch.empty((gb.N, gb.Hout, gb.Wout, gb.Cout), dtype=torch.float32, device=gh.device)
+    dw = torch.empty_like(w)
+    if dw.stride() != w.stride():
+        raise ValueError("weight must be dense")
+    work_dx = torch.empty(plan.bwd_ws, dtype=torch.uint8, device=gh.device) if plan.bwd_ws else None
+    work_dw = torch.empty(plan.wrw_ws, dtype=torch.uint8, device=gh.device)
+    db = torch.empty(gf.Cout, dtype=torch.float32, device=w.device) if colsum is not None else None
+    zero = _zero_line(gh.device)
+    _lib.check(lib.wc_conv_bwd_pair_f16x3(_ptr(gh), _ptr(gl), _ptr(gs), _ptr(img), _ptr(ws), _ptr(zero), plan.bwd_ptr, _ptr(dx),
+                                          _ptr(work_dx), plan.bwd_ws,
+                                          _ptr(xh), _ptr(xl), _ptr(xs), plan.fwd_ptr, _ptr(dw), w.stride(kf), w.stride(nf), w.stride(2),
+                                          w.stride(3), _ptr(colsum), _ptr(db), _ptr(work_dw), plan.wrw_ws, _stream()),
+               "wc_conv_bwd_pair_f16x3")
+    return dx, dw, db
+
+
 def takes_planes(shape, wshape, kind):
     class _S:
         pass
@@ -357,15 +381,21 @@
         fused_db = want_db and ctx.needs_input_grad[1] and _colsum_ok(gy.shape[-1])
         g_planes = split_planes(gy, colsum=fused_db, site=ctx.site, role='g')
         dx = dw = db = None
+        paired = ctx.needs_input_grad[0] and ctx.needs_input_grad[1] and ctx.bwd_image is not None and plan.pair
+        if paired:
+            dx, dw, pdb = backward_pair(g_planes, ctx.bwd_image, (xh, xl, xs), plan, w, colsum=g_planes[3] if fused_db else None)
+            if fused_db:
+                db = pdb
         if ctx.needs_input_grad[0]:
-            gb, kb, nb = plan.bwd
-            image = ctx.bwd_image if ctx.bwd_image is not None else weight_image(w, gb, kb, nb)
-            dx = run(g_planes[:3], image, gb, nbytes=plan.bwd_ws)
+            if not paired:
+                gb, kb, nb = plan.bwd
+                image = ctx.bwd_image if ctx.bwd_image is not None else weight_image(w, gb, kb, nb)
+                dx = run(g_planes[:3], image, gb, nbytes=plan.bwd_ws)
             if ctx.relu_input:
                 dx = torch.ops.aten.threshold_backward(dx, ctx.saved_tensors[4], 0)
             elif ctx.leaky is not None:
                 dx = leaky_backward_(dx, ctx.saved_tensors[4], ctx.leaky)
-        if ctx.needs_input_grad[1]:
+        if ctx.needs_input_grad[1] and not paired:
             gf, kf, nf = plan.fwd
             if fused_db:
                 dw, db = weight_gradient((xh, xl, xs), g_planes, gf, w, kf, nf, nbytes=plan.wrw_ws, colsum=g_planes[3])
@@ -419,18 +449,25 @@
         fused_db = need_w and _colsum_ok(gy.shape[-1])
         g_planes = split_planes(gy, colsum=fused_db, site=ctx.site, role='g')
         dx = dw = db = None
-        if ctx.needs_input_grad[0]:
+        paired = ctx.needs_input_grad[0] and need_w and ctx.bwd_image is not None and plan.pair
+        if paired:
+            dx, D, db = backward_pair(g_planes, ctx.bwd_image, (xh, xl, one), plan, w, colsum=g_planes[3] if fused_db else None)
+            if not fused_db:
+                db = gy.sum((0, 1, 2))
+            dw = ops.unfold_channel_scale(D, db, scale, center)
+        elif ctx.needs_input_grad[0]:
             gb, kb, nb = plan.bwd
             image = ctx.bwd_image if ctx.bwd_image is not None else weight_image(w, gb, kb, nb)
             dx = run(g_planes[:3], image, gb, nbytes=plan.bwd_ws)
         if need_w:
-            gf, kf, nf = plan.fwd
-            if fused_db:
-                D, db = weight_gradient((xh, xl, one), g_planes, gf, w, kf, nf, nbytes=plan.wrw_ws, colsum=g_planes[3])
-            else:
-                D = weight_gradient((xh, xl, one), g_planes, gf, w, kf, nf, nbytes=plan.wrw_ws)
-                db = gy.sum((0, 1, 2))
-            dw = ops.unfold_channel_scale(D, db, scale, center)
+            if not paired:
+                gf, kf, nf = plan.fwd
+                if fused_db:
+                    D, db = weight_gradient((xh, xl, one), g_planes, gf, w, kf, nf, nbytes=plan.wrw_ws, colsum=g_planes[3])
+                else:
+                    D = weight_gradient((xh, xl, one), g_planes, gf, w, kf, nf, nbytes=plan.wrw_ws)
+                    db = gy.sum((0, 1, 2))
+                dw = ops.unfold_channel_scale(D, db, scale, center)
         elif need_b:
             db = gy.sum((0, 1, 2))
         return dx, dw, (db if need_b else None), None, None, None
diff --git a/wc_gan_amd/csrc/wc_conv.hip b/wc_gan_amd/csrc/wc_conv.hip
--- a/wc_gan_amd/csrc/wc_conv.hip
+++ b/wc_gan_amd/csrc/wc_conv.hip
@@ -29,7 +29,7 @@
 }
 
 template <int MB, int NB, bool KS>
-__global__ __launch_bounds__(256) void conv_f16x3_kernel(ConvArgs a)
+__device__ __forceinline__ void conv_f16x3_body(const ConvArgs& a, const unsigned bx, const unsigned by, const unsigned bz)
 {
     extern __shared__ __attribute__((aligned(16))) char smem[];
     constexpr int TM = 64 * MB, TN = 64 * NB;
@@ -41,8 +41,8 @@
     const int wave = __builtin_amdgcn_readfirstlane(tid >> 6);
     const int wm = wave >> 1, wn = wave & 1;
     const int ntn = a.Cout / TN;
-    const int phase = blockIdx.y / ntn, nt = blockIdx.y - phase * ntn;
-    const unsigned m0 = blockIdx.x * TM;
+    const int phase = by / ntn, nt = by - phase * ntn;
+    const unsigned m0 = bx * TM;
     const unsigned HW = a.H * a.W;
     const int koff = (lane >> 5) * 8;
 
@@ -94,7 +94,7 @@
             #pragma unroll
             for (int r = 0; r < 16; ++r) acc[i][j][r] = 0.f;
 
-    const int it0 = KS ? (int)blockIdx.z * iters / a.ksplit : 0, it1 = KS ? ((int)blockIdx.z + 1) * iters / a.ksplit : iters;
+    const int it0 = KS ? (int)bz * iters / a.ksplit : 0, it1 = KS ? ((int)bz + 1) * iters / a.ksplit : iters;
     constexpr int NA = AQ * 4, ND = NA + 2 * NB, HALF = ND / 2, PER = 3 * MB * NB, GAP = PER / HALF;
     static_assert(PER % HALF == 0, "DMAs spread evenly");
     int tabv = 0;
@@ -189,7 +189,7 @@
             const int64_t opix = ((int64_t)n * a.Hout + (yy * a.out_stride + oy0)) * a.Wout + (xx * a.out_stride + ox0);
             const int64_t oe = opix * a.Cout + nt * TN + wn * NB * 32 + (lane & 31);
             if (KS) {
-                float* o = a.partial + (int64_t)blockIdx.z * ((int64_t)a.N * a.Hout * a.Wout * a.Cout) + oe;
+                float* o = a.partial + (int64_t)bz * ((int64_t)a.N * a.Hout * a.Wout * a.Cout) + oe;
                 #pragma unroll
                 for (int j = 0; j < NB; ++j) o[j * 32] = acc[i][j][r];
             } else {
@@ -205,12 +205,21 @@
     }
 }
 
-__global__ __launch_bounds__(256) void conv_ksplit_reduce_kernel(const float* __restrict__ partial, int ksplit, int64_t n4, int cout,
-                                                                 const float* __restrict__ xscale, const float* __restrict__ wscale,
-                                                                 const float* __restrict__ bias, int relu, float* __restrict__ y)
+template <int MB, int NB, bool KS>
+__global__ __launch_bounds__(256) void conv_f16x3_kernel(ConvArgs a) { conv_f16x3_body<MB, NB, KS>(a, blockIdx.x, blockIdx.y, blockIdx.z); }
+
+struct KsplitReduceArgs {
+    const float* partial; int ksplit; int64_t n4; int cout;
+    const float* xscale; const float* wscale; const float* bias; int relu; float* y;
+};
+
+__device__ __forceinline__ void conv_ksplit_reduce_body(const float* __restrict__ partial, int ksplit, int64_t n4, int cout,
+                                                        const float* __restrict__ xscale, const float* __restrict__ wscale,
+                                                        const float* __restrict__ bias, int relu, float* __restrict__ y,
+                                                        const unsigned bid, const unsigned nblocks)
 {
     const float inv = 1.0f / (xscale[0] * wscale[0]);
-    for (int64_t i = (int64_t)blockIdx.x * 256 + threadIdx.x; i < n4; i += (int64_t)gridDim.x * 256) {
+    for (int64_t i = (int64_t)bid * 256 + threadIdx.x; i < n4; i += (int64_t)nblocks * 256) {
         f32x4 v = *reinterpret_cast<const f32x4*>(partial + 4 * i);
         int z = 1;
         for (; z + 3 < ksplit; z += 4) {
@@ -226,6 +235,13 @@
         if (relu) { v[0] = fmaxf(v[0], 0.f); v[1] = fmaxf(v[1], 0.f); v[2] = fmaxf(v[2], 0.f); v[3] = fmaxf(v[3], 0.f); }
         *reinterpret_cast<f32x4*>(y + 4 * i) = v;
     }
+}
+
+__global__ __launch_bounds__(256) void conv_ksplit_reduce_kernel(const float* __restrict__ partial, int ksplit, int64_t n4, int cout,
+                                                                 const float* __restrict__ xscale, const float* __restrict__ wscale,
+                                                                 const float* __restrict__ bias, int relu, float* __restrict__ y)
+{
+    conv_ksplit_reduce_body(partial, ksplit, n4, cout, xscale, wscale, bias, relu, y, blockIdx.x, gridDim.x);
 }
 
 __device__ __forceinline__ f32x4 split_act(f32x4 v, int relu, float slope)
@@ -552,7 +568,7 @@
 }
 
 template <int MB, int NB>
-__global__ __launch_bounds__(256) void conv_wrw_kernel(WrwArgs a)
+__device__ __forceinline__ void conv_wrw_body(const WrwArgs& a, const unsigned bx, const unsigned by)
 {
     extern __shared__ __attribute__((aligned(16))) char smem[];
     constexpr int TA = 64 * MB, TB = 64 * NB;
@@ -565,11 +581,11 @@
     const int wave = __builtin_amdgcn_readfirstlane(tid >> 6);
     const int wm = wave >> 1, wn = wave & 1;
     const int nta = a.A.C / TA, ntb = a.B.C / TB;
-    int idx = blockIdx.y;
+    int idx = by;
     const int tb = idx % ntb; idx /= ntb;
     const int ta = idx % nta; idx /= nta;
     const int tap = idx % a.ntaps, phase = idx / a.ntaps;
-    const int c0 = blockIdx.x * a.cps, c1 = min(c0 + a.cps, a.nchunks);
+    const int c0 = bx * a.cps, c1 = min(c0 + a.cps, a.nchunks);
     const int dya = a.A.dy[phase][tap], dxa = a.A.dx[phase][tap], dyb = a.B.dy[phase][tap], dxb = a.B.dx[phase][tap];
     const unsigned HW = a.H * a.W;
     const unsigned lds0 = (unsigned)(size_t)((__attribute__((address_space(3))) char*)smem);
@@ -715,7 +731,7 @@
     __builtin_amdgcn_s_waitcnt(0x0F70);
 
     const int slice = phase * a.ntaps + tap, nslice = a.nphase * a.ntaps;
-    float* out = a.partial + ((int64_t)blockIdx.x * nslice + slice) * a.A.C * a.B.C;
+    float* out = a.partial + ((int64_t)bx * nslice + slice) * a.A.C * a.B.C;
     #pragma unroll
     for (int i = 0; i < MB; ++i)
         #pragma unroll
@@ -726,6 +742,9 @@
             for (int j = 0; j < NB; ++j) o[j * 32] = acc[i][j][r];
         }
 }
+
+template <int MB, int NB>
+__global__ __launch_bounds__(256) void conv_wrw_kernel(WrwArgs a) { conv_wrw_body<MB, NB>(a, blockIdx.x, blockIdx.y); }
 
 struct WrwReduceArgs {
     const float* partial; int splits, nslice, Ca, Cb;
@@ -737,10 +756,10 @@
     signed char r[kMaxTaps], s[kMaxTaps], cnt[kMaxTaps], slice[kMaxTaps][4];
 };
 
-__global__ __launch_bounds__(256) void conv_wrw_reduce_kernel(WrwReduceArgs a)
-{
-    if ((int)blockIdx.x >= a.main_blocks) {
-        const int u = ((int)blockIdx.x - a.main_blocks) * 256 + threadIdx.x, cg = u >> 6, lane = u & 63;
+__device__ __forceinline__ void conv_wrw_reduce_body(const WrwReduceArgs& a, const unsigned bid)
+{
+    if ((int)bid >= a.main_blocks) {
+        const int u = ((int)bid - a.main_blocks) * 256 + threadIdx.x, cg = u >> 6, lane = u & 63;
         if (cg >= a.c4n) return;
         f32x4 v = {0.f, 0.f, 0.f, 0.f};
         for (int b = lane; b < kAmaxBlocks; b += 64) v += *reinterpret_cast<const f32x4*>(a.colsum + (int64_t)b * 4 * a.c4n + 4 * cg);
@@ -754,7 +773,7 @@
     const int64_t plane = (int64_t)a.Ca * a.Cb, per = (int64_t)a.nslice * plane, total4 = (int64_t)a.nout * plane >> 2;
     const float inv = a.coef / (a.xscale[0] * a.gscale[0]);
     const int part = threadIdx.x & 3;
-    for (int64_t e4 = ((int64_t)blockIdx.x * 256 + threadIdx.x) >> 2; e4 < total4; e4 += (int64_t)a.main_blocks * 64) {
+    for (int64_t e4 = ((int64_t)bid * 256 + threadIdx.x) >> 2; e4 < total4; e4 += (int64_t)a.main_blocks * 64) {
         const int64_t e = e4 * 4;
         const int o = e / plane; const int64_t w = e - o * plane;
         f32x4 v = {0.f, 0.f, 0.f, 0.f};
@@ -779,6 +798,28 @@
         if (a.sb == 1 && ((uintptr_t)out & 15) == 0) *reinterpret_cast<f32x4*>(out) = v;
         else { out[0] = v[0]; out[a.sb] = v[1]; out[2 * a.sb] = v[2]; out[3 * a.sb] = v[3]; }
     }
+}
+
+__global__ __launch_bounds__(256) void conv_wrw_reduce_kernel(WrwReduceArgs a) { conv_wrw_reduce_body(a, blockIdx.x); }
+
+template <bool KS>
+__global__ __launch_bounds__(256) void conv_bwd_pair_kernel(ConvArgs d, WrwArgs w, int conv_blocks, int wrw_off, int wrw_splits, int gx, int gy)
+{
+    const int b = blockIdx.x;
+    if (b < conv_blocks) {
+        const int t = b / gx, z = t / gy;
+        conv_f16x3_body<2, 2, KS>(d, (unsigned)(b - t * gx), (unsigned)(t - z * gy), (unsigned)z);
+    } else if (b >= wrw_off) {
+        const int e = b - wrw_off, tile = e / wrw_splits;
+        conv_wrw_body<2, 2>(w, (unsigned)(e - tile * wrw_splits), (unsigned)tile);
+    }
+}
+
+__global__ __launch_bounds__(256) void conv_pair_reduce_kernel(WrwReduceArgs r, KsplitReduceArgs k, int wrw_blocks)
+{
+    if ((int)blockIdx.x < wrw_blocks) conv_wrw_reduce_body(r, blockIdx.x);
+    else conv_ksplit_reduce_body(k.partial, k.ksplit, k.n4, k.cout, k.xscale, k.wscale, k.bias, k.relu, k.y,
+                                 blockIdx.x - wrw_blocks, gridDim.x - wrw_blocks);
 }
 
 struct NarrowWrwArgs {
@@ -1190,14 +1231,19 @@
     return k > 1 ? (size_t)k * g->N * g->Hout * g->Wout * g->Cout * 4 : 0;
 }
 
-int wc_conv_f16x3(const void* xhi, const void* xlo, const float* xscale, const void* wimage, const float* wscale,
-                  const float* bias, const void* zero_line, const wc_conv_geom* g, int relu, float* y,
-                  void* ws, size_t ws_bytes, wc_stream_t stream)
-{
-    hipStream_t st = (hipStream_t)stream;
+static bool conv_big_tile(const wc_conv_geom* g, int ksplit)
+{
+    const int64_t M = (int64_t)g->N * g->H * g->W;
+    const bool wide = (g->Cout % 256) == 0;
+    const int64_t wgs_big = (M / 256) * g->nphase * (g->Cout / (wide ? 256 : 128));
+    return ksplit == 1 && (M % 256) == 0 && wgs_big >= 256;
+}
+
+static int conv_prepare(ConvArgs& a, const void* xhi, const void* xlo, const float* xscale, const void* wimage, const float* wscale,
+                        const float* bias, const void* zero_line, const wc_conv_geom* g, int relu, float* y, void* ws, size_t ws_bytes)
+{
     if (!xhi || !xlo || !xscale || !wimage || !wscale || !zero_line || !g || !y) return WC_ERR_ARG;
     if (!wc_conv_supported(g)) return WC_ERR_SHAPE;
-    ConvArgs a;
     a.xhi = (const _Float16*)xhi; a.xlo = (const _Float16*)xlo; a.zero = (const _Float16*)zero_line;
     a.wimg = (const char*)wimage; a.xscale = xscale; a.wscale = wscale; a.bias = bias; a.y = y;
     a.N = g->N; a.H = g->H; a.W = g->W; a.Hin = g->Hin; a.Win = g->Win; a.Cin = g->Cin; a.Cout = g->Cout;
@@ -1211,12 +1257,21 @@
         a.offy[p] = g->off_y[p]; a.offx[p] = g->off_x[p];
         for (int t = 0; t < kMaxTaps; ++t) { a.dy[p][t] = g->dy[p][t]; a.dx[p][t] = g->dx[p][t]; }
     }
-    const int64_t M = (int64_t)g->N * g->H * g->W;
+    return WC_OK;
+}
+
+int wc_conv_f16x3(const void* xhi, const void* xlo, const float* xscale, const void* wimage, const float* wscale,
+                  const float* bias, const void* zero_line, const wc_conv_geom* g, int relu, float* y,
+                  void* ws, size_t ws_bytes, wc_stream_t stream)
+{
+    hipStream_t st = (hipStream_t)stream;
+    ConvArgs a;
+    const int rc = conv_prepare(a, xhi, xlo, xscale, wimage, wscale, bias, zero_line, g, relu, y, ws, ws_bytes);
+    if (rc != WC_OK) return rc;
     const bool wide = (g->Cout % 256) == 0;
-    const int64_t wgs_big = (M / 256) * g->nphase * (g->Cout / (wide ? 256 : 128));
     hipError_t e;
     if (g->Cout % 128)                                      e = a.ksplit > 1 ? launch_conv<2, 1, true>(a, st) : launch_conv<2, 1>(a, st);
-    else if (a.ksplit == 1 && (M % 256) == 0 && wgs_big >= 256) e = wide ? launch_conv<4, 4>(a, st) : launch_conv<4, 2>(a, st);
+    else if (conv_big_tile(g, a.ksplit))                    e = wide ? launch_conv<4, 4>(a, st) : launch_conv<4, 2>(a, st);
     else if (a.ksplit > 1)                                  e = wide ? launch_conv<2, 4, true>(a, st) : launch_conv<2, 2, true>(a, st);
     else                                                    e = wide ? launch_conv<2, 4>(a, st) : launch_conv<2, 2>(a, st);
     if (e != hipSuccess) return (int)e;
@@ -1358,15 +1413,19 @@
                                   nullptr, nullptr, ws, ws_bytes, stream);
 }
 
-int wc_conv_wrw_bias_f16x3(const void* xhi, const void* xlo, const float* xscale, const void* ghi, const void* glo, const float* gscale,
-                           const void* zero_line, const wc_conv_geom* g, float* dw, int64_t stride_k, int64_t stride_n,
-                           int64_t stride_r, int64_t stride_s, const float* colsum_partials, float* db,
-                           void* ws, size_t ws_bytes, wc_stream_t stream)
-{
-    hipStream_t st = (hipStream_t)stream;
+struct WrwPlan { WrwArgs a; WrwReduceArgs r; int T, splits, tiles, extra; };
+
+static int wrw_prepare(WrwPlan& p, const void* xhi, const void* xlo, const float* xscale, const void* ghi, const void* glo, const float* gscale,
+                       const void* zero_line, const wc_conv_geom* g, float* dw, int64_t stride_k, int64_t stride_n,
+                       int64_t stride_r, int64_t stride_s, const float* colsum_partials, float* db, void* ws, size_t ws_bytes)
+{
     if (!xhi || !xlo || !xscale || !ghi || !glo || !gscale || !zero_line || !g || !dw || !ws) return WC_ERR_NULL;
     if (!wc_conv_supported(g) || (g->Cin & 63) || g->W < 2 || g->H * g->W < 2) return WC_ERR_SHAPE;
     if (ws_bytes < wc_conv_wrw_workspace_bytes(g)) return WC_ERR_WORKSPACE;
+    if ((colsum_partials == nullptr) != (db == nullptr)) return WC_ERR_NULL;
+    if (db && ((g->Cout & 3) || 256 % (g->Cout >> 2) != 0)) return WC_ERR_SHAPE;
+    WrwArgs& a = p.a;
+    WrwReduceArgs& r = p.r;
     int T;
     int splits = wrw_splits(g, &T);
     const int64_t M = (int64_t)g->N * g->H * g->W;
@@ -1376,27 +1435,25 @@
     WrwOperand X, G;
     X.hi = (const _Float16*)xhi; X.lo = (const _Float16*)xlo; X.Hp = g->Hin; X.Wp = g->Win; X.C = g->Cin; X.stride = g->in_stride;
     G.hi = (const _Float16*)ghi; G.lo = (const _Float16*)glo; G.Hp = g->Hout; G.Wp = g->Wout; G.C = g->Cout; G.stride = g->out_stride;
-    WrwReduceArgs r;
     r.nout = 0; r.coef = g->wcoef;
-    for (int p = 0; p < kMaxPhase; ++p)
+    for (int ph = 0; ph < kMaxPhase; ++ph)
         for (int t = 0; t < kMaxTaps; ++t) {
-            X.dy[p][t] = g->dy[p][t]; X.dx[p][t] = g->dx[p][t];
-            G.dy[p][t] = g->off_y[p]; G.dx[p][t] = g->off_x[p];
-            if (p >= g->nphase || t >= g->ntaps) continue;
-            if (g->nsrc[p][t] < 1 || g->nsrc[p][t] > 4) return WC_ERR_ARG;
-            for (int m = 0; m < g->nsrc[p][t]; ++m) {
+            X.dy[ph][t] = g->dy[ph][t]; X.dx[ph][t] = g->dx[ph][t];
+            G.dy[ph][t] = g->off_y[ph]; G.dx[ph][t] = g->off_x[ph];
+            if (ph >= g->nphase || t >= g->ntaps) continue;
+            if (g->nsrc[ph][t] < 1 || g->nsrc[ph][t] > 4) return WC_ERR_ARG;
+            for (int m = 0; m < g->nsrc[ph][t]; ++m) {
                 int o = 0;
-                while (o < r.nout && (r.r[o] != g->wr[p][t][m] || r.s[o] != g->ws[p][t][m])) ++o;
+                while (o < r.nout && (r.r[o] != g->wr[ph][t][m] || r.s[o] != g->ws[ph][t][m])) ++o;
                 if (o == r.nout) {
                     if (r.nout == kMaxTaps) return WC_ERR_ARG;
-                    r.r[o] = g->wr[p][t][m]; r.s[o] = g->ws[p][t][m]; r.cnt[o] = 0; ++r.nout;
+                    r.r[o] = g->wr[ph][t][m]; r.s[o] = g->ws[ph][t][m]; r.cnt[o] = 0; ++r.nout;
                 }
                 if (r.cnt[o] == 4) return WC_ERR_ARG;
-                r.slice[o][r.cnt[o]++] = (signed char)(p * g->ntaps + t);
+                r.slice[o][r.cnt[o]++] = (signed char)(ph * g->ntaps + t);
             }
         }
     const bool x_cols = stride_k == 1;
-    WrwArgs a;
     a.A = x_cols ? G : X; a.B = x_cols ? X : G;
     a.zero = (const _Float16*)zero_line; a.partial = (float*)ws;
     a.N = g->N; a.H = g->H; a.W = g->W; a.ntaps = g->ntaps; a.nphase = g->nphase;
@@ -1404,7 +1461,29 @@
     magic_u31((unsigned)g->W, &a.magW, &a.shW);
     a.nchunks = nchunks; a.cps = (nchunks + splits - 1) / splits;
     splits = (nchunks + a.cps - 1) / a.cps;
-    dim3 grid((unsigned)splits, (unsigned)tiles);
+    r.partial = (const float*)ws; r.splits = splits; r.nslice = nslice; r.Ca = a.A.C; r.Cb = a.B.C;
+    r.xscale = xscale; r.gscale = gscale; r.dw = dw;
+    r.sa = x_cols ? stride_n : stride_k; r.sb = x_cols ? stride_k : stride_n; r.sr = stride_r; r.ss = stride_s;
+    r.colsum = colsum_partials; r.db = db; r.c4n = db ? g->Cout >> 2 : 0;
+    r.main_blocks = grid_for((int64_t)r.nout * g->Cin * g->Cout);
+    p.T = T; p.splits = splits; p.tiles = tiles; p.extra = db ? (r.c4n * 64 + 255) / 256 : 0;
+    return WC_OK;
+}
+
+int wc_conv_wrw_bias_f16x3(const void* xhi, const void* xlo, const float* xscale, const void* ghi, const void* glo, const float* gscale,
+                           const void* zero_line, const wc_conv_geom* g, float* dw, int64_t stride_k, int64_t stride_n,
+                           int64_t stride_r, int64_t stride_s, const float* colsum_partials, float* db,
+                           void* ws, size_t ws_bytes, wc_stream_t stream)
+{
+    hipStream_t st = (hipStream_t)stream;
+    WrwPlan p;
+    const int rc = wrw_prepare(p, xhi, xlo, xscale, ghi, glo, gscale, zero_line, g, dw, stride_k, stride_n, stride_r, stride_s,
+                               colsum_partials, db, ws, ws_bytes);
+    if (rc != WC_OK) return rc;
+    const WrwArgs& a = p.a;
+    const WrwReduceArgs& r = p.r;
+    const int T = p.T;
+    dim3 grid((unsigned)p.splits, (unsigned)p.tiles);
     hipError_t e = hipSuccess;
     if (T == 256) {
         constexpr int LDS = 2 * (2 * 4 * 4 * 1024 + 2 * 4 * 4 * 1024);
@@ -1422,16 +1501,74 @@
         if (e != hipSuccess) return (int)e;
         hipLaunchKernelGGL((conv_wrw_kernel<2, 2>), grid, dim3(256), LDS, st, a);
     }
-    r.partial = (const float*)ws; r.splits = splits; r.nslice = nslice; r.Ca = a.A.C; r.Cb = a.B.C;
-    r.xscale = xscale; r.gscale = gscale; r.dw = dw;
-    r.sa = x_cols ? stride_n : stride_k; r.sb = x_cols ? stride_k : stride_n; r.sr = stride_r; r.ss = stride_s;
-    if ((colsum_partials == nullptr) != (db == nullptr)) return WC_ERR_NULL;
-    if (db && ((g->Cout & 3) || 256 % (g->Cout >> 2) != 0)) return WC_ERR_SHAPE;
-    r.colsum = colsum_partials; r.db = db; r.c4n = db ? g->Cout >> 2 : 0;
-    r.main_blocks = grid_for((int64_t)r.nout * g->Cin * g->Cout);
-    const int extra = db ? (r.c4n * 64 + 255) / 256 : 0;
-    hipLaunchKernelGGL(conv_wrw_reduce_kernel, dim3(r.main_blocks + extra), dim3(256), 0, st, r);
+    hipLaunchKernelGGL(conv_wrw_reduce_kernel, dim3(r.main_blocks + p.extra), dim3(256), 0, st, r);
     return (int)hipGetLastError();
 }
 
-}
+int wc_conv_bwd_pair_supported(const wc_conv_geom* gd, const wc_conv_geom* gf)
+{
+    if (!gd || !gf || !wc_conv_supported(gd) || !wc_conv_supported(gf) || (gf->Cin & 63) || gf->H * gf->W < 2) return 0;
+    if (gd->N != gf->N || gd->Cin != gf->Cout || gd->Cout != gf->Cin) return 0;
+    if (gd->Hin != gf->Hout || gd->Win != gf->Wout || gd->Hout != gf->Hin || gd->Wout != gf->Win) return 0;
+    if (gf->nphase != 1 || gd->in_stride != 1) return 0;
+    if ((gd->Cout % 128) != 0 || (gd->Cout % 256) == 0 || conv_big_tile(gd, conv_ksplit(gd))) return 0;
+    int tile;
+    (void)wrw_splits(gf, &tile);
+    return tile == 128 ? 1 : 0;
+}
+
+size_t wc_conv_bwd_pair_workspace_bytes(const wc_conv_geom* gd, const wc_conv_geom* gf)
+{
+    if (!gd || !gf) return 0;
+    return wc_conv_workspace_bytes(gd) + wc_conv_wrw_workspace_bytes(gf);
+}
+
+int wc_conv_bwd_pair_f16x3(const void* ghi, const void* glo, const float* gscale, const void* wimage, const float* wscale,
+                           const void* zero_line, const wc_conv_geom* gd, float* dx, void* ws_dx, size_t ws_dx_bytes,
+                           const void* xhi, const void* xlo, const float* xscale, const wc_conv_geom* gf, float* dw,
+                           int64_t stride_k, int64_t stride_n, int64_t stride_r, int64_t stride_s,
+                           const float* colsum_partials, float* db, void* ws_dw, size_t ws_dw_bytes, wc_stream_t stream)
+{
+    hipStream_t st = (hipStream_t)stream;
+    ConvArgs d;
+    int rc = conv_prepare(d, ghi, glo, gscale, wimage, wscale, nullptr, zero_line, gd, 0, dx, ws_dx, ws_dx_bytes);
+    if (rc != WC_OK) return rc;
+    WrwPlan p;
+    rc = wrw_prepare(p, xhi, xlo, xscale, ghi, glo, gscale, zero_line, gf, dw, stride_k, stride_n, stride_r, stride_s,
+                     colsum_partials, db, ws_dw, ws_dw_bytes);
+    if (rc != WC_OK) return rc;
+    if (!wc_conv_bwd_pair_supported(gd, gf) || p.T != 128) return WC_ERR_SHAPE;
+    constexpr int LDS = 2 * (2 * 2 * 4 * 1024 + 2 * 2 * 4 * 1024);
+    const int64_t M = (int64_t)gd->N * gd->H * gd->W;
+    const int gx = (int)(M / 128), gy = gd->nphase * (gd->Cout / 128);
+    const int64_t conv_blocks = (int64_t)gx * gy * d.ksplit, wrw_off = (conv_blocks + 7) & ~(int64_t)7;
+    const int64_t blocks = wrw_off + (int64_t)p.splits * p.tiles;
+    if (blocks > 0x7fffffff) return WC_ERR_SHAPE;
+    hipError_t e;
+    if (d.ksplit > 1) {
+        e = wc_set_max_lds(reinterpret_cast<const void*>(conv_bwd_pair_kernel<true>), LDS);
+        if (e != hipSuccess) return (int)e;
+        hipLaunchKernelGGL((conv_bwd_pair_kernel<true>), dim3((unsigned)blocks), dim3(256), LDS, st, d, p.a,
+                           (int)conv_blocks, (int)wrw_off, p.splits, gx, gy);
+    } else {
+        e = wc_set_max_lds(reinterpret_cast<const void*>(conv_bwd_pair_kernel<false>), LDS);
+        if (e != hipSuccess) return (int)e;
+        hipLaunchKernelGGL((conv_bwd_pair_kernel<false>), dim3((unsigned)blocks), dim3(256), LDS, st, d, p.a,
+                           (int)conv_blocks, (int)wrw_off, p.splits, gx, gy);
+    }
+    e = hipGetLastError();
+    if (e != hipSuccess) return (int)e;
+    const int reduce_blocks = p.r.main_blocks + p.extra;
+    if (d.ksplit > 1) {
+        KsplitReduceArgs k;
+        k.n4 = (int64_t)gd->N * gd->Hout * gd->Wout * gd->Cout / 4;
+        k.partial = (const float*)ws_dx; k.ksplit = d.ksplit; k.cout = gd->Cout;
+        k.xscale = gscale; k.wscale = wscale; k.bias = nullptr; k.relu = 0; k.y = dx;
+        hipLaunchKernelGGL(conv_pair_reduce_kernel, dim3(reduce_blocks + grid_for(k.n4)), dim3(256), 0, st, p.r, k, reduce_blocks);
+    } else {
+        hipLaunchKernelGGL(conv_wrw_reduce_kernel, dim3(reduce_blocks), dim3(256), 0, st, p.r);
+    }
+    return (int)hipGetLastError();
+}
+
+}
```

Result: faster. 3692 images/sec (median of 6 runs) (+2.4%).
